# thisparticle/scl_slam

Measured on AMD Instinct MI355X. Metric: loop-closure candidates/sec: (scan, keyframe) pairs taken through full-database ARG-MIN detection per second (every pair aligned exactly and bounded by the f16 matrix-core screening; only the survivors get the f64 distance), batches of 16 scans, 10k-keyframe DB per GPU, higher is better.
Workload: dtype f64 results; f16-operand / f32-accumulate MFMA screening + f64 exact pass on the survivors

## Files before the change

### include/scl_engine.h

```cpp
#ifndef SCL_ENGINE_H
#define SCL_ENGINE_H

#include <stddef.h>
#include <stdint.h>

#ifdef __cplusplus
extern "C" {
#endif

typedef struct scl_engine scl_engine;

typedef enum scl_status {
    SCL_OK               =  0,
    SCL_ERR_INVALID_ARG  = -1,
    SCL_ERR_NO_DEVICE    = -2,
    SCL_ERR_HIP          = -3,
    SCL_ERR_OUT_OF_RANGE = -4,
    SCL_ERR_NOMEM        = -5,
    SCL_ERR_UNSUPPORTED  = -6
} scl_status;

typedef struct scl_config {
    int    num_ring;
    int    num_sector;
// ... 149 lines not shown
                             const scl_icp_params *p, int min_src_points, int min_tgt_points,
                             float T[16], float *fitness, int *converged, int *iterations, int *n_src, int *n_tgt);
int  scl_loop_icp_batch_from_store(scl_engine *e, int robot, int key_cur, const float *pose_cur,
                                   int n_candidates, const int *keys_pre, int search_num, const float *poses_pre, float leaf,
                                   const scl_icp_params *p, int min_src_points, int min_tgt_points,
                                   float *T, float *fitness, int *converged, int *iterations, int *n_src, int *n_tgts);

int  scl_geometric_verification_from_store(scl_engine *e, const void *src, int n_src, int stride_bytes, float src_leaf,
                                           int robot, int key_pre, int search_num, const float *poses_pre, float leaf,
                                           int min_src_points, int min_tgt_points,
                                           int ransac_iterations, double inlier_threshold, double inlier_ratio, uint64_t seed,
                                           float T[16], int *success, int *n_src_filtered, int *n_tgt,
                                           int *n_correspondences, int *n_inliers);

int  scl_geometric_verification_batch(scl_engine *e, const void *src, int n_src,
                                      const void *const *tgts, const int *n_tgts, int n_targets, int stride_bytes,
                                      int ransac_iterations, double inlier_threshold, double inlier_ratio, uint64_t seed,
                                      float *T, int *success, int *n_correspondences, int *n_inliers);
int  scl_geometric_verification_batch_from_store(scl_engine *e, const void *src, int n_src, int stride_bytes, float src_leaf,
                                                 int robot, int n_candidates, const int *keys_pre, int search_num, const float *poses_pre, float leaf,
                                                 int min_src_points, int min_tgt_points,
                                                 int ransac_iterations, double inlier_threshold, double inlier_ratio, uint64_t seed,
                                                 float *T, int *success, int *n_src_filtered, int *n_tgts,
                                                 int *n_correspondences, int *n_inliers);

int  scl_geometric_verification_batch_guess(scl_engine *e, const void *src, int n_src,
                                            const void *const *tgts, const int *n_tgts, int n_targets, int stride_bytes,
                                            const float *guesses,
                                            int ransac_iterations, double inlier_threshold, double inlier_ratio, uint64_t seed,
                                            float *T, float *T_fit, int *success, int *n_correspondences, int *n_inliers);
int  scl_geometric_verification_batch_from_store_guess(scl_engine *e, const void *src, int n_src, int stride_bytes, float src_leaf,
                                                       int robot, int n_candidates, const int *keys_pre, int search_num, const float *poses_pre, float leaf,
                                                       const float *guesses,
                                                       int min_src_points, int min_tgt_points,
                                                       int ransac_iterations, double inlier_threshold, double inlier_ratio, uint64_t seed,
                                                       float *T, float *T_fit, int *success, int *n_src_filtered, int *n_tgts,
                                                       int *n_correspondences, int *n_inliers);

int  scl_icp_align_batch_guess(scl_engine *e, const void *src, int n_src, const void *const *tgts, const int *n_tgts,
                               int n_targets, int stride_bytes, const float *guesses, const scl_icp_params *p,
                               float *T, float *T_icp, float *fitness, int *converged, int *iterations);
int  scl_loop_icp_batch_from_store_guess(scl_engine *e, int robot, int key_cur, const float *pose_cur,
                                         int n_candidates, const int *keys_pre, int search_num, const float *poses_pre, float leaf,
                                         const float *guesses, const scl_icp_params *p, int min_src_points, int min_tgt_points,
                                         float *T, float *T_icp, float *fitness, int *converged, int *iterations, int *n_src, int *n_tgts);
int  scl_icp_align_batch_from_store_guess(scl_engine *e, const void *src, int n_src, int stride_bytes, float src_leaf,
                                          int robot, int n_candidates, const int *keys_pre, int search_num, const float *poses_pre, float leaf,
                                          const float *guesses, const scl_icp_params *p, int min_src_points, int min_tgt_points,
                                          float *T, float *T_icp, float *fitness, int *converged, int *iterations,
                                          int *n_src_filtered, int *n_tgts);

int  scl_registration_eval_batch(scl_engine *e, const void *src, int n_src, const void *const *tgts, const int *n_tgts,
                                 int n_targets, int stride_bytes, const float *transforms, double max_dist,
                                 int *n_valid, int *n_inliers, double *moments);
int  scl_registration_eval_batch_from_store(scl_engine *e, const void *src, int n_src, int stride_bytes, float src_leaf,
                                            int robot, int n_candidates, const int *keys_pre, int search_num, const float *poses_pre, float leaf,
                                            const float *transforms, int min_src_points, int min_tgt_points, double max_dist,
                                            int *n_valid, int *n_inliers, double *moments, int *n_src_filtered, int *n_tgts);
int  scl_loop_eval_batch_from_store(scl_engine *e, int robot, int key_cur, const float *pose_cur,
                                    int n_candidates, const int *keys_pre, int search_num, const float *poses_pre, float leaf,
                                    const float *transforms, int min_src_points, int min_tgt_points, double max_dist,
                                    int *n_valid, int *n_inliers, double *moments, int *n_src, int *n_tgts);
int  scl_registration_information(int n_inliers, const double moments[10], double info[36]);

int  scl_target_normals(scl_engine *e, const void *tgt, int n_tgt, int stride_bytes, double radius, float *normals);
int  scl_registration_eval_plane_batch(scl_engine *e, const void *src, int n_src, const void *const *tgts, const int *n_tgts,
                                       int n_targets, int stride_bytes, const float *transforms, double max_dist, double normal_radius,
                                       int *n_valid, int *n_inliers, int *n_planar, double *sums);
int  scl_registration_eval_plane_batch_from_store(scl_engine *e, const void *src, int n_src, int stride_bytes, float src_leaf,
                                                  int robot, int n_candidates, const int *keys_pre, int search_num, const float *poses_pre, float leaf,
                                                  const float *transforms, int min_src_points, int min_tgt_points, double max_dist, double normal_radius,
                                                  int *n_valid, int *n_inliers, int *n_planar, double *sums, int *n_src_filtered, int *n_tgts);
int  scl_loop_eval_plane_batch_from_store(scl_engine *e, int robot, int key_cur, const float *pose_cur,
                                          int n_candidates, const int *keys_pre, int search_num, const float *poses_pre, float leaf,
                                          const float *transforms, int min_src_points, int min_tgt_points, double max_dist, double normal_radius,
                                          int *n_valid, int *n_inliers, int *n_planar, double *sums, int *n_src, int *n_tgts);
int  scl_registration_information_plane(const double sums[29], double info[36], double grad[6]);

int  scl_profile_enable(scl_engine *e, int on);
int  scl_profile_reset(scl_engine *e);
int  scl_profile_get(scl_engine *e, scl_profile *out);
void scl_debug_icp_tile_stats(unsigned long long out[16], int reset);
int  scl_alignment_stats(scl_engine *e, uint64_t *pairs, uint64_t *fallbacks, int reset);
int  scl_survivor_stats(scl_engine *e, uint64_t *queries, uint64_t *survivors, uint64_t *max_survivors, int reset);
int  scl_device_name(const scl_engine *e, char *buf, int buflen);
int  scl_host_copy_rate(scl_engine *e, size_t bytes, int reps, double *gbytes_per_s);
int  scl_selftest_atanf_blocks(scl_engine *e, int first_block, int n_blocks, uint64_t *checksums);
int  scl_selftest_bin_paths(scl_engine *e, int mode, uint64_t seed, uint64_t n_points, uint64_t *disagreements, uint64_t *sure);

int  scl_selftest_sort_pairs(scl_engine *e, int key_bytes, const void *keys, const uint32_t *values, int n, int bits, const int *segment_offsets,
                             int n_segments, void *keys_out, uint32_t *values_out);
int  scl_selftest_prefix_sum(scl_engine *e, const int32_t *in, int n, int inclusive, int32_t *out);
int  scl_selftest_submaps_batch(scl_engine *e, int robot, int n_jobs, const int *keys, const int *search_nums,
                                const float *poses ,
                                float leaf, void *out, int out_capacity , int *n_out );

#ifdef __cplusplus
}
#endif
#endif
```

### scl_slam_amd/csrc/engine.hip

```cpp
#include "scl_engine.h"

#include <hip/hip_runtime.h>

#include <cfloat>
#include <climits>
#include <chrono>
#include <cmath>
#include <cstdio>
#include <cstdlib>
#include <cstring>
#include <mutex>
#include <new>
#include <string>
#include <atomic>
#include <chrono>
#include <thread>
#include <vector>

#include "db_file.hpp"
#include "engine_internal.hpp"
#include "device_sort.hpp"
#include "plugin_host.hpp"

#ifdef SCL_DIAGNOSTICS
// ... 128 lines not shown
    if ((rc = dev_alloc(e, &nd, tile * nst))) return rc;
    if ((rc = dev_alloc(e, &nv, (size_t)e->S * nst))) return rc;
    if ((rc = dev_alloc(e, &nn, (size_t)e->S * nst))) return rc;
    if ((rc = dev_alloc(e, &nr, (size_t)e->R4 * nst))) return rc;
    if ((rc = dev_alloc(e, &nh, (size_t)e->hstride * nst))) return rc;
    if ((rc = dev_alloc(e, &nk, (size_t)8 * nst))) return rc;
    if ((rc = dev_alloc(e, &nhk, (size_t)e->hkw * nst))) return rc;
    if (hab && (rc = dev_alloc(e, &nha, hab * (size_t)ncap))) return rc;
    if ((rc = dev_alloc(e, &nr4, (size_t)e->RG * ncap))) return rc;
    SCL_HIP(e, hipMemsetAsync(nr4, 0, sizeof(float4) * (size_t)e->RG * ncap, e->stream));
    if (e->n > 0) {
        SCL_HIP(e, hipMemcpyAsync(nd, e->d_desc, sizeof(float4) * tile * e->n, hipMemcpyDeviceToDevice, e->stream));
        SCL_HIP(e, hipMemcpyAsync(nv, e->d_vkey, sizeof(double) * (size_t)e->S * e->n, hipMemcpyDeviceToDevice, e->stream));
        SCL_HIP(e, hipMemcpyAsync(nn, e->d_norm, sizeof(double) * (size_t)e->S * e->n, hipMemcpyDeviceToDevice, e->stream));
        SCL_HIP(e, hipMemcpyAsync(nr, e->d_rkey, sizeof(float) * (size_t)e->R4 * e->n, hipMemcpyDeviceToDevice, e->stream));
        SCL_HIP(e, hipMemcpyAsync(nh, e->d_hdesc, sizeof(uint2) * (size_t)e->hstride * e->n, hipMemcpyDeviceToDevice, e->stream));
        SCL_HIP(e, hipMemcpyAsync(nk, e->d_kmask, sizeof(unsigned int) * (size_t)8 * e->n, hipMemcpyDeviceToDevice, e->stream));
        SCL_HIP(e, hipMemcpyAsync(nhk, e->d_hkey, sizeof(unsigned short) * (size_t)e->hkw * e->n, hipMemcpyDeviceToDevice, e->stream));
        if (hab) SCL_HIP(e, hipMemcpyAsync(nha, e->d_halign, hab * (size_t)e->n, hipMemcpyDeviceToDevice, e->stream));
        SCL_HIP(e, hipMemcpy2DAsync(nr4, sizeof(float4) * ncap, e->d_rkey4, sizeof(float4) * e->cap,
                                    sizeof(float4) * e->n, e->RG, hipMemcpyDeviceToDevice, e->stream));
    }
    if (e->cap > 0) {
        const size_t k = (size_t)e->stage_rows;
        SCL_HIP(e, hipMemcpyAsync(nd + tile * ncap, e->d_desc + tile * e->cap, sizeof(float4) * tile * k, hipMemcpyDeviceToDevice, e->stream));
        SCL_HIP(e, hipMemcpyAsync(nv + (size_t)e->S * ncap, e->d_vkey + (size_t)e->S * e->cap, sizeof(double) * e->S * k, hipMemcpyDeviceToDevice, e->stream));
        SCL_HIP(e, hipMemcpyAsync(nn + (size_t)e->S * ncap, e->d_norm + (size_t)e->S * e->cap, sizeof(double) * e->S * k, hipMemcpyDeviceToDevice, e->stream));
        SCL_HIP(e, hipMemcpyAsync(nr + (size_t)e->R4 * ncap, e->d_rkey + (size_t)e->R4 * e->cap, sizeof(float) * e->R4 * k, hipMemcpyDeviceToDevice, e->stream));
        SCL_HIP(e, hipMemcpyAsync(nh + (size_t)e->hstride * ncap, e->d_hdesc + (size_t)e->hstride * e->cap, sizeof(uint2) * e->hstride * k, hipMemcpyDeviceToDevice, e->stream));
        SCL_HIP(e, hipMemcpyAsync(nk + (size_t)8 * ncap, e->d_kmask + (size_t)8 * e->cap, sizeof(unsigned int) * 8 * k, hipMemcpyDeviceToDevice, e->stream));
        SCL_HIP(e, hipMemcpyAsync(nhk + (size_t)e->hkw * ncap, e->d_hkey + (size_t)e->hkw * e->cap, sizeof(unsigned short) * e->hkw * k, hipMemcpyDeviceToDevice, e->stream));
    }
    SCL_HIP(e, hipStreamSynchronize(e->stream));
    for (hipStream_t s2 : {e->stream_alt, e->stream_surv, e->stream2})
        if (s2) SCL_HIP(e, hipStreamSynchronize(s2));
    dev_free(e->d_desc); dev_free(e->d_vkey); dev_free(e->d_norm); dev_free(e->d_rkey); dev_free(e->d_rkey4);
    dev_free(e->d_hdesc); dev_free(e->d_kmask); dev_free(e->d_hkey); dev_free(e->d_halign);
    e->d_desc = nd; e->d_vkey = nv; e->d_norm = nn; e->d_rkey = nr; e->d_rkey4 = nr4;
    e->d_hdesc = nh; e->d_kmask = nk; e->d_hkey = nhk; e->d_halign = nha;
    e->cap = ncap;
    return SCL_OK;
}

int ensure_vals(scl_engine *e, size_t floats)
{
    if (floats <= e->vals_cap) return SCL_OK;
    dev_free(e->d_vals);
    int rc = dev_alloc(e, &e->d_vals, floats);
    if (rc) { e->vals_cap = 0; return rc; }
    e->vals_cap = floats;
    return SCL_OK;
}

int ensure_points(scl_engine *e, size_t bytes)
{
    if (bytes <= e->points_cap) return SCL_OK;
    dev_free(e->d_points);
    size_t nb = bytes + bytes / 4 + 4096;
    int rc = dev_alloc(e, &e->d_points, nb);
    if (rc) { e->points_cap = 0; return rc; }
    e->points_cap = nb;
    return SCL_OK;
}

int ensure_pairs(scl_engine *e, size_t n)
{
    if (n <= e->pair_cap) return SCL_OK;
    dev_free(e->d_dist); dev_free(e->d_shift); dev_free(e->d_cand); dev_free(e->d_ring_d2);
    dev_free(e->d_approx); dev_free(e->d_surv); dev_free(e->d_starts);
    size_t nn = n + n / 2 + 64;
    int rc;
    e->pair_cap = 0;
    if ((rc = dev_alloc(e, &e->d_approx, nn))) return rc;
    if ((rc = dev_alloc(e, &e->d_starts, nn))) return rc;
    if ((rc = dev_alloc(e, &e->d_surv, nn))) return rc;
    if ((rc = dev_alloc(e, &e->d_ring_d2, nn))) return rc;
    if ((rc = dev_alloc(e, &e->d_dist, nn))) return rc;
    if ((rc = dev_alloc(e, &e->d_shift, nn))) return rc;
    if ((rc = dev_alloc(e, &e->d_cand, nn))) return rc;
    e->pair_cap = nn;
    return SCL_OK;
}

int ensure_sets(scl_engine *e, size_t n)
{
    if (n <= e->set_stride && e->pair_cap >= e->set_stride * scl_engine::kScreenSets) return SCL_OK;
    const size_t stride = n + n / 4 + 64;
    int rc = ensure_pairs(e, stride * scl_engine::kScreenSets);
    if (rc) { e->set_stride = 0; return rc; }
    e->set_stride = stride;
    if (e->smask_cap < stride * scl_engine::kScreenSets) {
        dev_free(e->d_smask); e->d_smask = nullptr; e->smask_cap = 0;
        if ((rc = dev_alloc(e, &e->d_smask, stride * scl_engine::kScreenSets))) { e->set_stride = 0; return rc; }
        e->smask_cap = stride * scl_engine::kScreenSets;
    }
    const size_t need = 2 * stride * sc_screen_scratch_floats(db_view(e), e->SR);
    if (need > e->part_cap) {
        dev_free(e->d_part); e->part_cap = 0;
        if ((rc = dev_alloc(e, &e->d_part, need))) { e->set_stride = 0; return rc; }
        e->part_cap = need;
    }
    return SCL_OK;
}

int ensure_pinned(scl_engine *e, size_t bytes)
{
    if (bytes <= e->pinned_cap) return SCL_OK;
    if (e->h_pinned) { (void)hipHostFree(e->h_pinned); e->h_pinned = nullptr; e->pinned_cap = 0; }
    SCL_HIP(e, hipHostMalloc(&e->h_pinned, bytes, hipHostMallocDefault));
    memset(e->h_pinned, 0, bytes);
    e->pinned_cap = bytes;
    return SCL_OK;
}

int ingest_from_vals(scl_engine *e, int count, int first_slot)
{
    ProfScope ps(e, P_INGEST);
    SCL_HIP(e, launch_ingest(e->d_vals, count, first_slot, e->d_desc, e->d_vkey, e->d_norm, e->d_rkey,
                             e->d_rkey4, e->d_hdesc, e->d_kmask, e->d_hkey, e->hstride, e->cap, e->R, e->S, e->stream, e->d_halign));
    e->db_version++;
    return SCL_OK;
}

int append_meta(scl_engine *e, int8_t robot, int index)
{
    e->robots.push_back(robot);
    e->indexs.push_back(index);
    e->n++;
    return SCL_OK;
}

int ensure_tiles(scl_engine *e, hipStream_t s)
{
    int rc;
    if (!e->d_tiles) {
        if ((rc = dev_alloc(e, &e->d_tiles, (size_t)2 * kMaxScBatch * e->R * e->S))) return rc;
        e->tiles_clean = false;
    }
    if (!e->tiles_clean) {
        SCL_HIP(e, launch_make_sc_tiles_init(e->d_tiles, 2 * kMaxScBatch, e->R, e->S, s));
        e->tiles_clean = true;
    }
    return SCL_OK;
}

int check_cloud(scl_engine *e, const void *points, int n_points, int stride_bytes)
{
    if (n_points < 0 || stride_bytes < 12 || (stride_bytes & 3)) return fail(e, SCL_ERR_INVALID_ARG, "bad point layout");
    if (n_points > 0 && !points) return fail(e, SCL_ERR_INVALID_ARG, "null points");
    return SCL_OK;
}

int group_scatter(scl_engine *e, const unsigned char *const *dptr, const int *n, int count, int stride, hipStream_t s)
{
    int rc;
    if (count < 1 || count > kMaxScBatch) return fail(e, SCL_ERR_INVALID_ARG, "batch of 1..16 scans");
    if ((rc = ensure_tiles(e, s))) return rc;
    if ((rc = ensure_vals(e, (size_t)e->R * e->S * (size_t)kMaxScBatch))) return rc;
    ScanBatch b{};
    b.count = count;
    uint64_t pts = 0;
    for (int i = 0; i < count; ++i) { b.points[i] = dptr[i]; b.n[i] = n[i]; pts += (uint64_t)n[i]; }
    e->tiles_clean = false;
    ProfScope ps(e, P_MAKESC, s);
    const int slice = e->R * e->S > 10000 ? 2 * kScPointsPerWorkgroup : kScPointsPerWorkgroup;
    SCL_HIP(e, launch_make_sc_batch(b, stride, e->R, e->S, e->cfg.lidar_height, e->cfg.max_radius, e->d_tiles,
                                    scl_lab_int("SCL_SC_SLICE", slice), e->num_cu, s));
    e->prof.make_sc_points += e->prof_on ? pts : 0;
// ... 135 lines not shown
const char *scl_status_string(int status)
{
    switch (status) {
    case SCL_OK: return "ok";
    case SCL_ERR_INVALID_ARG: return "invalid argument";
    case SCL_ERR_NO_DEVICE: return "no HIP device";
    case SCL_ERR_HIP: return "HIP runtime error";
    case SCL_ERR_OUT_OF_RANGE: return "index out of range";
    case SCL_ERR_NOMEM: return "out of memory";
    case SCL_ERR_UNSUPPORTED: return "unsupported";
    default: return "unknown status";
    }
}

const char *scl_last_error(const scl_engine *e) { return e ? e->last_error.c_str() : "null engine"; }

int scl_abi_version(void) { return 11; }

int scl_default_config(scl_config *c)
{
    if (!c) return SCL_ERR_INVALID_ARG;
    c->num_ring = 20; c->num_sector = 60; c->num_candidates = 3;
    c->dist_thres = 0.14; c->lidar_height = 1.65; c->max_radius = 80.0;
    c->num_exclude_recent = 100; c->tree_making_period = 10;
    c->search_ratio = 0.1;
    c->knn_exclude_eps = 0.0f;
    c->device = 0;
    c->initial_capacity = 4096;
    return SCL_OK;
}

static void log_env_overrides_once()
{
    static std::atomic<bool> done{false};
    if (done.exchange(true)) return;
    static const char *const names[] = {"SCL_SCREEN", "SCL_SCREEN_FORM", "SCL_SCREEN_V2_MIN", "SCL_RCCL_LIB",
                                        "SCL_SCREEN_VARIANT", "SCL_SCREEN_PROBE", "SCL_SCREEN_TAIL", "SCL_ALIGN_WGS",
                                        "SCL_ALIGN2_WGS", "SCL_ALIGN_FILTER", "SCL_SC_KERNEL", "SCL_SC_WAVES", "SCL_STAMP", "SCL_ABLATE",
                                        "SCL_ICP_REDUCE", "SCL_MATRIX_PLAIN", "SCL_MATRIX_KERNEL", "SCL_MATRIX_KR", "SCL_WIDE_EXACT", "SCL_STREAM_EXACT", "SCL_SMALL_EXACT_OFF",
                                        "SCL_SELF_ALIGN_OFF", "SCL_CAND_EXACT_OFF"};
    constexpr int kProduct = 4;
    int i = 0;
    for (const char *n : names) {
        const char *v = getenv(n);
#ifdef SCL_DIAGNOSTICS
        if (v) fprintf(stderr, "scl_engine (diagnostics build): environment override in effect: %s=%s\n", n, v);
#else
        if (v && i < kProduct) fprintf(stderr, "scl_engine: environment override in effect: %s=%s\n", n, v);
        else if (v) fprintf(stderr, "scl_engine: %s=%s is an experiment's switch: ignored by this build (make EXTRA=-DSCL_DIAGNOSTICS builds them in)\n", n, v);
#endif
        ++i;
    }
    (void)kProduct;
}

int scl_create(const scl_config *cfg, scl_engine **out)
{
    if (!cfg || !out) return SCL_ERR_INVALID_ARG;
    *out = nullptr;
    log_env_overrides_once();
    if (cfg->num_ring < 1 || cfg->num_ring > 256 || cfg->num_sector < 1 || cfg->num_sector > 1024 ||
        cfg->num_candidates < 1 || cfg->num_candidates > kTopkMaxK || cfg->tree_making_period < 1 ||
        cfg->num_exclude_recent < 0 || !(cfg->max_radius > 0.0) || !(cfg->search_ratio >= 0.0))
        return SCL_ERR_INVALID_ARG;
    int ndev = 0;
    if (hipGetDeviceCount(&ndev) != hipSuccess || ndev <= 0) return SCL_ERR_NO_DEVICE;
    if (cfg->device < 0 || cfg->device >= ndev) return SCL_ERR_INVALID_ARG;
    scl_engine *e = new (std::nothrow) scl_engine();
    if (!e) return SCL_ERR_NOMEM;
    e->cfg = *cfg;
    e->R = cfg->num_ring; e->S = cfg->num_sector;
    e->RG = (e->R + 3) / 4; e->R4 = e->RG * 4;
    e->hstride = hdesc_stride(e->RG, e->S);
    e->hkw = hkey_row_halfs(e->S);
    e->SR = (int)std::round(0.5 * cfg->search_ratio * (double)e->S);
    if (e->SR < 0) e->SR = 0;
    e->device = cfg->device;
    int rc = SCL_OK;
    auto bail = [&](int code) { scl_destroy(e); return code; };
    if (hipSetDevice(e->device) != hipSuccess) return bail(SCL_ERR_HIP);
    hipDeviceProp_t prop;
    if (hipGetDeviceProperties(&prop, e->device) == hipSuccess && prop.multiProcessorCount > 0)
        e->num_cu = prop.multiProcessorCount;
    if (hipStreamCreateWithFlags(&e->stream, hipStreamNonBlocking) != hipSuccess) return bail(SCL_ERR_HIP);
    {
        int lo_p = 0, hi_p = 0;
        (void)hipDeviceGetStreamPriorityRange(&lo_p, &hi_p);
        if (hipStreamCreateWithPriority(&e->stream2, hipStreamNonBlocking, hi_p) != hipSuccess) return bail(SCL_ERR_HIP);
    }
    if (hipEventCreateWithFlags(&e->ev_fork, hipEventDisableTiming) != hipSuccess) return bail(SCL_ERR_HIP);
    if (hipEventCreateWithFlags(&e->ev_join, hipEventDisableTiming) != hipSuccess) return bail(SCL_ERR_HIP);
    if (hipHostMalloc((void **)&e->h_out3, 64 * scl_engine::kSlots, hipHostMallocDefault) != hipSuccess) return bail(SCL_ERR_HIP);
    memset(e->h_out3, 0, 64 * scl_engine::kSlots);
    for (int i = 0; i < scl_engine::kSlots; ++i)
        if (hipEventCreateWithFlags(&e->ev_done[i], hipEventDisableTiming) != hipSuccess) return bail(SCL_ERR_HIP);
    if ((rc = ensure_capacity(e, 1))) return bail(rc);
    if ((rc = dev_alloc(e, &e->d_topk_scratch, (size_t)kTopkMaxBlocks * kTopkMaxK + 2))) return bail(rc);
    if (hipMemset(e->d_topk_scratch, 0, sizeof(unsigned long long) * ((size_t)kTopkMaxBlocks * kTopkMaxK + 2)) != hipSuccess) return bail(SCL_ERR_HIP);
    if ((rc = dev_alloc(e, &e->d_topk_idx, (size_t)kTopkMaxK * scl_engine::kScreenSets))) return bail(rc);
    if ((rc = dev_alloc(e, &e->d_topk_d2, (size_t)kTopkMaxK * scl_engine::kScreenSets))) return bail(rc);
    if ((rc = dev_alloc(e, &e->d_out3, (size_t)4))) return bail(rc);
    if ((rc = dev_alloc(e, &e->d_blk_part, (size_t)kTailBlocks * kTailRec * kMaxQueryBatch))) return bail(rc);
    static_assert(kMaxQueryBatch <= 4, "done_counter holds four counters");
    if ((rc = dev_alloc(e, &e->d_done_counter, (size_t)4))) return bail(rc);
    if (hipMemset(e->d_done_counter, 0, 16) != hipSuccess) return bail(SCL_ERR_HIP);
    {
        constexpr int NS = scl_engine::kScreenSets;
        if ((rc = dev_alloc(e, &e->d_nsurv, (size_t)NS))) return bail(rc);
        static_assert(NS <= kTminEpsOffset, "the launch's largest bound sits kTminEpsOffset words behind its t_min word");
        if ((rc = dev_alloc(e, &e->d_tmin, (size_t)NS + kTminEpsOffset))) return bail(rc);
        if (hipMemset(e->d_nsurv, 0, sizeof(int) * NS) != hipSuccess) return bail(SCL_ERR_HIP);
        if (hipMemset(e->d_tmin, 0xff, sizeof(unsigned int) * NS) != hipSuccess) return bail(SCL_ERR_HIP);
        if (hipMemset(e->d_tmin + NS, 0, sizeof(unsigned int) * kTminEpsOffset) != hipSuccess) return bail(SCL_ERR_HIP);
        if ((rc = dev_alloc(e, &e->d_surv_part, (size_t)NS * kSurvivorBlocks * kTailRec))) return bail(rc);
        if ((rc = dev_alloc(e, &e->d_surv_done, (size_t)NS))) return bail(rc);
        if (hipMemset(e->d_surv_done, 0, sizeof(unsigned int) * NS) != hipSuccess) return bail(SCL_ERR_HIP);
        if (hipMalloc(&e->d_surv_args, (size_t)8 * NS * kSurvivorArgBytes) != hipSuccess) return bail(SCL_ERR_NOMEM);
        if (hipHostMalloc(&e->h_surv_args, (size_t)8 * NS * kSurvivorArgBytes, hipHostMallocDefault) != hipSuccess) return bail(SCL_ERR_HIP);
        if (hipHostMalloc((void **)&e->h_stream_out, (size_t)2 * NS * 64, hipHostMallocDefault) != hipSuccess) return bail(SCL_ERR_HIP);
        for (auto &ev : e->ev_chunk) if (hipEventCreateWithFlags(&ev, hipEventDisableTiming) != hipSuccess) return bail(SCL_ERR_HIP);
        for (auto &ev : e->ev_k1) if (hipEventCreateWithFlags(&ev, hipEventDisableTiming) != hipSuccess) return bail(SCL_ERR_HIP);
        for (auto &ev : e->ev_sub0) if (hipEventCreateWithFlags(&ev, hipEventDisableTiming) != hipSuccess) return bail(SCL_ERR_HIP);
        if (hipEventCreateWithFlags(&e->ev_align_gate, hipEventDisableTiming) != hipSuccess) return bail(SCL_ERR_HIP);
        {
            int lo_p = 0, hi_p = 0;
            (void)hipDeviceGetStreamPriorityRange(&lo_p, &hi_p);
            const bool wide_grid = e->S == 180 && e->RG == 20;
            if (hipStreamCreateWithPriority(&e->stream_surv, hipStreamNonBlocking, wide_grid ? hi_p : lo_p) != hipSuccess) return bail(SCL_ERR_HIP);
            if (hipStreamCreateWithPriority(&e->stream_queue_place, hipStreamNonBlocking, lo_p) != hipSuccess) return bail(SCL_ERR_HIP);
        }
    }
    if (hipStreamCreateWithFlags(&e->stream_alt, hipStreamNonBlocking) != hipSuccess) return bail(SCL_ERR_HIP);
    if (hipEventCreateWithFlags(&e->ev_db, hipEventDisableTiming) != hipSuccess) return bail(SCL_ERR_HIP);
    if ((rc = dev_alloc(e, &e->d_align_fallbacks, (size_t)1))) return bail(rc);
    if (hipMemset(e->d_align_fallbacks, 0, sizeof(unsigned long long)) != hipSuccess) return bail(SCL_ERR_HIP);
    if ((rc = dev_alloc(e, &e->d_surv_stats, (size_t)3))) return bail(rc);
    if (hipMemset(e->d_surv_stats, 0, 3 * sizeof(unsigned long long)) != hipSuccess) return bail(SCL_ERR_HIP);
    if ((rc = ensure_pairs(e, 1024))) return bail(rc);
    e->screen = sc_screen_supported(db_view(e), e->SR) && cfg->num_candidates <= kTailTopMaxK;
    if ((rc = ensure_pinned(e, 1 << 16))) return bail(rc);
    if ((rc = ensure_vals(e, (size_t)e->R * e->S))) return bail(rc);
    *out = e;
    return SCL_OK;
}

int scl_destroy(scl_engine *e)
{
#ifdef SCL_DIAGNOSTICS
    if (e && !e->front && scl_lab_int("SCL_INGEST_STAMPS", 0)) { (void)hipSetDevice(e->device); scl::ingest_stamps_print(); scl::cand_stamps_print(); }
#endif
    if (!e) return SCL_OK;
    if (e->front) return front_destroy(e);
    (void)hipSetDevice(e->device);
    if (e->stream) (void)hipStreamSynchronize(e->stream);
    for (auto &p : e->pending) { (void)hipEventDestroy(p.start); (void)hipEventDestroy(p.stop); }
    for (auto ev : e->event_pool) (void)hipEventDestroy(ev);
    icp_workspace_free(&e->icp_ws);
    icp_workspace_free(&e->vox_ws);
    for (void *slab : e->kf_slabs) (void)hipFree(slab);
    for (int i = 0; i < scl_engine::kIcpBatch; ++i) icp_workspace_free(&e->icp_batch_ws[i]);
    for (int i = 0; i < scl_engine::kIcpLanes; ++i) icp_workspace_free(&e->vox_lane_ws[i]);
    icp_workspace_free(&e->icp_batch_ctl);
    for (int i = 0; i < scl_engine::kIcpLanes; ++i) {
        if (e->ev_lane[i]) (void)hipEventDestroy(e->ev_lane[i]);
        icp_workspace_free(&e->icp_lane_ws[i]);
        if (e->icp_lane_stream[i]) (void)hipStreamDestroy(e->icp_lane_stream[i]);
    }
    dev_free(e->d_desc); dev_free(e->d_vkey); dev_free(e->d_norm); dev_free(e->d_rkey); dev_free(e->d_rkey4);
    dev_free(e->d_hdesc); dev_free(e->d_kmask); dev_free(e->d_hkey); dev_free(e->d_halign);
    dev_free(e->d_vals); dev_free(e->d_points); dev_free(e->d_tiles);
    for (int b = 0; b < 3; ++b) {
        dev_free(e->d_pbuf[b]);
        for (int c = 0; c < scl_engine::kCopyStreams; ++c) if (e->ev_copied[c][b]) (void)hipEventDestroy(e->ev_copied[c][b]);
        if (e->ev_consumed[b]) (void)hipEventDestroy(e->ev_consumed[b]);
    }
    if (e->stream_copy) { (void)hipStreamSynchronize(e->stream_copy); (void)hipStreamDestroy(e->stream_copy); }
    for (hipStream_t cs : e->stream_copy_x) if (cs) { (void)hipStreamSynchronize(cs); (void)hipStreamDestroy(cs); }
    for (void *hp : e->host_allocs) (void)hipHostFree(hp);
    dev_free(e->d_dist); dev_free(e->d_shift); dev_free(e->d_cand); dev_free(e->d_ring_d2);
    dev_free(e->d_approx); dev_free(e->d_starts); dev_free(e->d_surv); dev_free(e->d_nsurv); dev_free(e->d_tmin); dev_free(e->d_part);
    dev_free(e->d_align_fallbacks);
    dev_free(e->d_smask);
    if (e->d_mat_dist) (void)hipFree(e->d_mat_dist);
    if (e->d_mat_shift) (void)hipFree(e->d_mat_shift);
    if (e->d_rank_key) (void)hipFree(e->d_rank_key);
    if (e->d_rank_pos) (void)hipFree(e->d_rank_pos);
    if (e->d_rank_out) (void)hipFree(e->d_rank_out);
    if (e->h_rank_out) (void)hipHostFree(e->h_rank_out);
    dev_free(e->d_meta_robot); dev_free(e->d_meta_index);
    if (e->h_mat) (void)hipHostFree(e->h_mat);
    for (auto &ev : e->ev_mat_k) if (ev) (void)hipEventDestroy(ev);
    for (auto &ev : e->ev_mat_c) if (ev) (void)hipEventDestroy(ev);
    dev_free(e->d_surv_stats);
    dev_free(e->d_surv_part); dev_free(e->d_surv_done);
    if (e->d_surv_args) (void)hipFree(e->d_surv_args);
    if (e->h_surv_args) (void)hipHostFree(e->h_surv_args);
    if (e->h_stream_out) (void)hipHostFree(e->h_stream_out);
    for (auto ev : e->ev_chunk) if (ev) (void)hipEventDestroy(ev);
    if (e->stream_surv) { (void)hipStreamSynchronize(e->stream_surv); (void)hipStreamDestroy(e->stream_surv); }
    if (e->stream_queue_place) (void)hipStreamDestroy(e->stream_queue_place);
    for (auto ev : e->ev_k1) if (ev) (void)hipEventDestroy(ev);
    for (auto ev : e->ev_sub0) if (ev) (void)hipEventDestroy(ev);
    if (e->ev_align_gate) (void)hipEventDestroy(e->ev_align_gate);
    dev_free(e->d_topk_scratch); dev_free(e->d_topk_idx); dev_free(e->d_topk_d2); dev_free(e->d_out3);
    dev_free(e->d_blk_part); dev_free(e->d_done_counter);
    if (e->ev_db) (void)hipEventDestroy(e->ev_db);
    if (e->stream_alt) { (void)hipStreamSynchronize(e->stream_alt); (void)hipStreamDestroy(e->stream_alt); }
    if (e->h_pinned) (void)hipHostFree(e->h_pinned);
    if (e->h_out3) (void)hipHostFree(e->h_out3);
    if (e->ev_call) (void)hipEventDestroy(e->ev_call);
    for (int i = 0; i < scl_engine::kSlots; ++i) if (e->ev_done[i]) (void)hipEventDestroy(e->ev_done[i]);
    if (e->ev_fork) (void)hipEventDestroy(e->ev_fork);
    if (e->ev_join) (void)hipEventDestroy(e->ev_join);
    if (e->stream2) { (void)hipStreamSynchronize(e->stream2); (void)hipStreamDestroy(e->stream2); }
    if (e->stream) (void)hipStreamDestroy(e->stream);
    delete e;
    return SCL_OK;
}


int scl_make_and_save(scl_engine *e, const void *points, int n_points, int stride_bytes,
                      int8_t robot, int index, float *out_values)
{
    if (!e) return SCL_ERR_INVALID_ARG;
    if (e->front) return front_make_and_save(e, points, n_points, stride_bytes, robot, index, out_values, false, 0.f, nullptr);
    std::lock_guard<std::mutex> lk(e->mu);
    (void)hipSetDevice(e->device);
    int rc;
    if ((rc = ensure_capacity(e, e->n + 1))) return rc;
    if ((rc = scatter_host_cloud(e, points, n_points, stride_bytes))) return rc;
    if ((rc = group_ingest(e, 1, e->n, e->stream))) return rc;
    if (out_values)
        SCL_HIP(e, hipMemcpyAsync(out_values, e->d_vals, sizeof(float) * (size_t)e->R * e->S,
                                  hipMemcpyDeviceToHost, e->stream));
    if ((rc = sync_short(e))) return rc;
    return append_meta(e, robot, index);
}

int scl_make_and_save_filtered(scl_engine *e, const void *points, int n_points, int stride_bytes, float leaf,
                               int8_t robot, int index, float *out_values, int *n_filtered)
{
    if (!e) return SCL_ERR_INVALID_ARG;
    if (e->front) return front_make_and_save(e, points, n_points, stride_bytes, robot, index, out_values, true, leaf, n_filtered);
    std::lock_guard<std::mutex> lk(e->mu);
    (void)hipSetDevice(e->device);
    int rc;
    if ((rc = check_cloud(e, points, n_points, stride_bytes))) return rc;
    if ((rc = ensure_capacity(e, e->n + 1))) return rc;
    std::string err;
    const void *d_cloud = nullptr;
    int m = 0;
    if ((rc = voxel_grid_to_device(&e->vox_ws, e->stream, points, n_points, stride_bytes, leaf, &d_cloud, &m, &err))) { e->last_error = err; return rc; }
    const unsigned char *dp = static_cast<const unsigned char *>(d_cloud);
    if ((rc = group_scatter(e, &dp, &m, 1, stride_bytes, e->stream))) return rc;
    if ((rc = group_ingest(e, 1, e->n, e->stream))) return rc;
    if (out_values)
        SCL_HIP(e, hipMemcpyAsync(out_values, e->d_vals, sizeof(float) * (size_t)e->R * e->S,
                                  hipMemcpyDeviceToHost, e->stream));
    if ((rc = sync(e))) return rc;
    if (n_filtered) *n_filtered = m;
    return append_meta(e, robot, index);
}

// ... 516 lines not shown

int scl_sc_search_range(scl_engine *e, const int *queries, const int *lo, const int *hi, int n_queries, int k,
                        int *cand_ids, int *cand_shifts, double *cand_dists, int *n_found)
{
    if (!e || n_queries < 0 || k < 1 || k > SCL_SC_SEARCH_MAX || (n_queries > 0 && (!queries || !lo || !hi || !cand_ids))) return SCL_ERR_INVALID_ARG;
    if (n_queries == 0) return SCL_OK;
    if (e->front) return front_sc_search_range(e, queries, lo, hi, n_queries, k, cand_ids, cand_shifts, cand_dists, n_found);
    std::lock_guard<std::mutex> pk(e->pass_mu);
    std::lock_guard<std::mutex> lk(e->mu);
    (void)hipSetDevice(e->device);
    return sc_search_locked(e, queries, lo, hi, n_queries, k, cand_ids, cand_shifts, cand_dists, n_found);
}

int scl_sc_search(scl_engine *e, const int *curs, int count, int k, int *cand_ids, int *cand_shifts, double *cand_dists, int *n_found)
{
    if (!e || count < 0 || k < 1 || k > SCL_SC_SEARCH_MAX || (count > 0 && (!curs || !cand_ids))) return SCL_ERR_INVALID_ARG;
    if (count == 0) return SCL_OK;
    std::vector<int> lo((size_t)count, 0), hi((size_t)count, 0);
    for (int i = 0; i < count; ++i) {
        if (curs[i] < 0) return SCL_ERR_OUT_OF_RANGE;
        const int h = curs[i] - e->cfg.num_exclude_recent;
        hi[(size_t)i] = h > 0 ? h : 0;
    }
    return scl_sc_search_range(e, curs, lo.data(), hi.data(), count, k, cand_ids, cand_shifts, cand_dists, n_found);
}

namespace {

int sc_search_robot(scl_engine *e, const int *curs, int count, bool inter, int robot_pre, int k,
                    int *cand_ids, int *cand_shifts, double *cand_dists, int *n_found)
{
    std::lock_guard<std::mutex> pk(e->pass_mu);
    std::lock_guard<std::mutex> lk(e->mu);
    (void)hipSetDevice(e->device);
    for (int i = 0; i < count; ++i)
        if (curs[i] < 0 || curs[i] >= e->n) return fail(e, SCL_ERR_OUT_OF_RANGE, "query keyframe out of range");
    std::vector<ScRankRule> rules((size_t)count);
    for (int i = 0; i < count; ++i) {
        const int r = e->robots[(size_t)curs[i]], x = e->indexs[(size_t)curs[i]];
        if (inter && robot_pre != SCL_SC_ANY_OTHER_ROBOT && robot_pre == r) return fail(e, SCL_ERR_INVALID_ARG, "robot_pre is the query's own robot: that is scl_sc_search_intra's set");
        rules[(size_t)i] = inter ? sc_inter_rule(r, robot_pre) : sc_intra_rule(r, x, e->cfg.num_exclude_recent);
    }
    const std::vector<int> lo((size_t)count, 0), hi((size_t)count, e->n);
    return sc_search_locked(e, curs, lo.data(), hi.data(), count, k, cand_ids, cand_shifts, cand_dists, n_found, rules.data());
}

}

int scl_sc_search_intra(scl_engine *e, const int *curs, int count, int k, int *cand_ids, int *cand_shifts, double *cand_dists, int *n_found)
{
    if (!e || count < 0 || k < 1 || k > SCL_SC_SEARCH_MAX || (count > 0 && (!curs || !cand_ids))) return SCL_ERR_INVALID_ARG;
    if (count == 0) return SCL_OK;
    if (e->front) return front_sc_search_intra(e, curs, count, k, cand_ids, cand_shifts, cand_dists, n_found);
    return sc_search_robot(e, curs, count, false, 0, k, cand_ids, cand_shifts, cand_dists, n_found);
}

int scl_sc_search_inter(scl_engine *e, const int *curs, int count, int robot_pre, int k, int *cand_ids, int *cand_shifts, double *cand_dists,
                        int *n_found)
{
    if (!e || count < 0 || k < 1 || k > SCL_SC_SEARCH_MAX || (count > 0 && (!curs || !cand_ids))) return SCL_ERR_INVALID_ARG;
    if (robot_pre < SCL_SC_ANY_OTHER_ROBOT || robot_pre > 127) return SCL_ERR_INVALID_ARG;
    if (count == 0) return SCL_OK;
    if (e->front) return front_sc_search_inter(e, curs, count, robot_pre, k, cand_ids, cand_shifts, cand_dists, n_found);
    return sc_search_robot(e, curs, count, true, robot_pre, k, cand_ids, cand_shifts, cand_dists, n_found);
}

namespace {

int submit_full_many_locked(scl_engine *e, const int *queries, const int *los, const int *his, int nq, int *tickets);

struct ScreenGroup { const int *qslot, *lo, *n; int nq, set0; int part_half = 0; bool masks = false; bool keys_later = false; };
int launch_screen_group(scl_engine *e, const ScreenGroup &cur, int phases = kScreenAlign | kScreenProducts,
                        const ScreenGroup *next = nullptr, hipStream_t stream = nullptr)
{
    if (!stream) stream = e->stream;
    auto fill = [&](ScreenBatch &sb, const ScreenGroup &g) {
        sb.nq = g.nq;
        for (int j = 0; j < g.nq; ++j) { sb.slot[j] = g.qslot[j]; sb.base[j] = g.lo[j]; sb.n[j] = g.n[j]; sb.buf[j] = g.set0 + j; }
        sb.pair_stride = e->set_stride;
        sb.approx = e->d_approx; sb.starts = e->d_starts; sb.align_fallbacks = e->d_align_fallbacks; sb.ring_d2 = e->d_ring_d2;
        sb.survivors = nullptr; sb.n_surv = nullptr; sb.t_min = e->d_tmin;
        sb.smask = (g.masks || sc_screen_is_wide(db_view(e), e->SR)) ? e->d_smask : nullptr;
        sb.part = e->d_part + (g.part_half ? e->part_cap / 2 : 0);
        sb.no_ring_metric = g.keys_later;
        sb.k = e->cfg.num_candidates; sb.exclude_eps = e->cfg.knn_exclude_eps; sb.topk_idx = e->d_topk_idx; sb.topk_d2 = e->d_topk_d2;
    };
    ScreenBatch sb{}, nx{};
    fill(sb, cur);
    const bool has_next = next && next->nq > 0;
    if (has_next) fill(nx, *next);
    if (phases & kScreenAlign) for (int j = 0; j < cur.nq; ++j) e->align_pairs += (uint64_t)cur.n[j];
    if (has_next) for (int j = 0; j < next->nq; ++j) e->align_pairs += (uint64_t)next->n[j];
    if ((phases & kScreenAlign) && (phases & kScreenProducts) && has_next) {
        SCL_HIP(e, launch_sc_screen_batch(db_view(e), sb, e->SR, sc_align_filter_enabled(), e->num_cu, stream, kScreenAlign, nullptr));
        phases = kScreenProducts;
    }
    ProfScope ps(e, P_SC, stream);
    SCL_HIP(e, launch_sc_screen_batch(db_view(e), sb, e->SR, sc_align_filter_enabled(), e->num_cu, stream, phases, has_next ? &nx : nullptr));
    if (ps.active()) { for (int j = 0; j < cur.nq; ++j) e->prof.sc_distance_pairs += (uint64_t)cur.n[j]; }
    return SCL_OK;
}

unsigned survivor_arg_region(scl_engine *e) { return e->surv_arg_tick++ & 7u; }
int launch_survivor_pass(scl_engine *e, const int *qslot, const int *lo, const int *n, int nq, int set0, double *const *out3, hipStream_t stream = nullptr,
                         int phases = kSurvivorArgs | kSurvivorKernel, int region_in = -1, bool ring_from_keys = false)
{
    if (!stream) stream = e->stream;
    SurvivorPass sp{};
    sp.nq = nq; sp.ring_from_keys = ring_from_keys ? 1 : 0;
    for (int j = 0; j < nq; ++j) { sp.slot[j] = qslot[j]; sp.base[j] = lo[j]; sp.n[j] = n[j]; sp.buf[j] = set0 + j; sp.out3[j] = out3[j]; }
    sp.pair_stride = e->set_stride;
    sp.approx = e->d_approx; sp.survivors = e->d_surv; sp.t_min = e->d_tmin; sp.out_dist = e->d_dist; sp.out_shift = e->d_shift;
    sp.blk_part = e->d_surv_part; sp.done_counter = e->d_surv_done; sp.surv_stats = e->d_surv_stats;
    sp.ring_d2 = e->d_ring_d2; sp.k = e->cfg.num_candidates; sp.exclude_eps = e->cfg.knn_exclude_eps; sp.topk_idx = e->d_topk_idx; sp.topk_d2 = e->d_topk_d2;
    const size_t region = (size_t)(region_in >= 0 ? (unsigned)region_in : survivor_arg_region(e)) * scl_engine::kScreenSets * kSurvivorArgBytes;
    sp.d_args = static_cast<char *>(e->d_surv_args) + region; sp.h_args = static_cast<char *>(e->h_surv_args) + region;
    if (!(phases & kSurvivorKernel)) {
        SCL_HIP(e, launch_sc_distance_survivors(db_view(e), sp, e->SR, e->num_cu, stream, phases));
        return SCL_OK;
    }
    ProfScope ps(e, P_ARGMIN, stream);
    SCL_HIP(e, launch_sc_distance_survivors(db_view(e), sp, e->SR, e->num_cu, stream, phases));
    return SCL_OK;
}

int launch_small_exact_chunk(scl_engine *e, const int *qslot, const int *lo, const int *n, int nq, int set0, double *const *out3, hipStream_t stream,
                             int phases, int region_in)
{
    static_assert(sizeof(SmallExactQuery) <= kSurvivorArgBytes && kMaxSmallExactQueries <= scl_engine::kScreenSets, "argument regions");
    if (nq < 1 || nq > kMaxSmallExactQueries) return fail(e, SCL_ERR_INVALID_ARG, "exact pass: too many scans for one launch");
    const size_t region = (size_t)(region_in >= 0 ? (unsigned)region_in : survivor_arg_region(e)) * scl_engine::kScreenSets * kSurvivorArgBytes;
    SmallExactQuery *h = reinterpret_cast<SmallExactQuery *>(static_cast<char *>(e->h_surv_args) + region);
    SmallExactQuery *d = reinterpret_cast<SmallExactQuery *>(static_cast<char *>(e->d_surv_args) + region);
    const bool wide_masks = sc_screen_is_wide(db_view(e), e->SR) && e->d_smask;
    if (phases & kSurvivorArgs) {
        for (int j = 0; j < nq; ++j) {
            const size_t set = (size_t)(set0 + j), off = set * e->set_stride;
            SmallExactQuery &sq = h[j];
            sq.qslot = qslot[j]; sq.base = lo[j]; sq.n = n[j];
            sq.approx = e->d_approx + off; sq.starts = e->d_starts + off; sq.smask = wide_masks ? e->d_smask + off : nullptr; sq.ring_d2 = e->d_ring_d2 + off;
            sq.t_min = e->d_tmin + set; sq.list = e->d_surv + off; sq.out3 = out3[j];
            sq.topk_idx = e->d_topk_idx + set * kTailTopMaxK; sq.topk_d2 = e->d_topk_d2 + set * kTailTopMaxK;
        }
        SCL_HIP(e, hipMemcpyAsync(d, h, sizeof(SmallExactQuery) * (size_t)nq, hipMemcpyHostToDevice, stream));
    }
    if (!(phases & kSurvivorKernel)) return SCL_OK;
    SmallExactArgs sa{};
    sa.nq = nq; sa.k = e->cfg.num_candidates; sa.exclude_eps = e->cfg.knn_exclude_eps; sa.two_eps = 2.0f * sc_screen_eps(); sa.surv_stats = e->d_surv_stats;
    sa.q_dev = d;
    sa.every_shift = wide_masks ? 0 : 1;
    ProfScope ps(e, P_ARGMIN, stream);
    SCL_HIP(e, launch_sc_small_exact(db_view(e), e->SR, sa, stream));
    return SCL_OK;
}

int launch_survivor_pass_wide(scl_engine *e, const int *qslot, const int *lo, const int *n, int nq, int set0, double *const *out3, hipStream_t stream, hipEvent_t first_done = nullptr)
{
    ProfScope ps(e, P_ARGMIN, stream);
    for (int g = 0; g < nq; g += kWideExactBatch) {
        const int w = nq - g < kWideExactBatch ? nq - g : kWideExactBatch;
        ScreenBatch sb{};
        sb.nq = w;
        for (int j = 0; j < w; ++j) { sb.slot[j] = qslot[g + j]; sb.base[j] = lo[g + j]; sb.n[j] = n[g + j]; sb.buf[j] = set0 + g + j; }
        sb.pair_stride = e->set_stride;
        sb.approx = e->d_approx; sb.starts = e->d_starts; sb.align_fallbacks = e->d_align_fallbacks; sb.ring_d2 = e->d_ring_d2;
        sb.survivors = e->d_surv; sb.n_surv = e->d_nsurv; sb.t_min = e->d_tmin; sb.surv_stats = e->d_surv_stats;
// ... 1017 lines not shown

int scl_screen_distances(scl_engine *e, int query, int lo, int hi, float *approx, int *survivors, int *n_survivors, float *eps)
{
    if (!e || !approx) return SCL_ERR_INVALID_ARG;
    if (e->front) return fail(e, SCL_ERR_UNSUPPORTED, "screen_distances: call it on a one-GPU engine");
    std::lock_guard<std::mutex> pk(e->pass_mu);
    std::lock_guard<std::mutex> lk(e->mu);
    (void)hipSetDevice(e->device);
    if (eps) *eps = sc_screen_eps();
    if (!e->screen) return fail(e, SCL_ERR_UNSUPPORTED, "no screening pass for this grid (64x120 and 80x180 at search ratio 0.1 only)");
    int qslot;
    if (query >= 0) { if (query >= e->n) return fail(e, SCL_ERR_OUT_OF_RANGE, "query slot out of range"); qslot = query; }
    else { const int j = -1 - query; if (j >= e->stage_rows || !e->staged[j]) return fail(e, SCL_ERR_INVALID_ARG, "no staged query"); qslot = e->cap + j; }
    if (lo < 0) lo = 0;
    if (hi > e->n) hi = e->n;
    const int n = hi - lo;
    if (n_survivors) *n_survivors = 0;
    if (n <= 0) return SCL_OK;
    int rc;
    if ((rc = ensure_pairs(e, (size_t)n))) return rc;
    {
        const size_t per_pair = sc_screen_scratch_floats(db_view(e), e->SR) / (size_t)sc_screen_max_batch(db_view(e), e->SR);
        if ((size_t)n * per_pair > e->part_cap) {
            dev_free(e->d_part); e->part_cap = 0;
            if ((rc = dev_alloc(e, &e->d_part, (size_t)n * per_pair + 1024))) return rc;
            e->part_cap = (size_t)n * per_pair + 1024;
        }
    }
    ScreenBatch sb{};
    sb.part = e->d_part;
    sb.nq = 1; sb.slot[0] = qslot; sb.base[0] = lo; sb.n[0] = n; sb.pair_stride = (size_t)n;
    sb.approx = e->d_approx; sb.starts = e->d_starts; sb.align_fallbacks = e->d_align_fallbacks; sb.ring_d2 = e->d_ring_d2; sb.survivors = e->d_surv; sb.n_surv = e->d_nsurv; sb.t_min = e->d_tmin;
    sb.k = e->cfg.num_candidates; sb.exclude_eps = e->cfg.knn_exclude_eps; sb.topk_idx = e->d_topk_idx; sb.topk_d2 = e->d_topk_d2;
    SCL_HIP(e, launch_sc_screen_batch(db_view(e), sb, e->SR, sc_align_filter_enabled(), e->num_cu, e->stream));
    SCL_HIP(e, launch_sc_select_batch(sb, e->stream));
    SCL_HIP(e, hipMemcpyAsync(approx, e->d_approx, sizeof(float) * (size_t)n, hipMemcpyDeviceToHost, e->stream));
    int ns = 0;
    SCL_HIP(e, hipMemcpyAsync(&ns, e->d_nsurv, sizeof(int), hipMemcpyDeviceToHost, e->stream));
    if ((rc = sync(e))) return rc;
    if (n_survivors) *n_survivors = ns;
    if (survivors && ns > 0) {
        SCL_HIP(e, hipMemcpyAsync(survivors, e->d_surv, sizeof(int) * (size_t)ns, hipMemcpyDeviceToHost, e->stream));
        if ((rc = sync(e))) return rc;
    }
    return SCL_OK;
}

int scl_screen_distances_many(scl_engine *e, const int *queries, int n_queries, int lo, int hi, float *approx, float *eps)
{
    if (!e || !queries || !approx || n_queries < 1 || n_queries > kMaxScreenBatch) return SCL_ERR_INVALID_ARG;
    if (e->front) return fail(e, SCL_ERR_UNSUPPORTED, "screen_distances_many: call it on a one-GPU engine");
    std::lock_guard<std::mutex> pk(e->pass_mu);
    std::lock_guard<std::mutex> lk(e->mu);
    (void)hipSetDevice(e->device);
    if (eps) *eps = sc_screen_eps();
    if (!e->screen) return fail(e, SCL_ERR_UNSUPPORTED, "no screening pass for this grid (64x120 and 80x180 at search ratio 0.1 only)");
    if (n_queries > sc_screen_max_batch(db_view(e), e->SR)) return fail(e, SCL_ERR_INVALID_ARG, "more scans than a screening launch takes");
    if (lo < 0) lo = 0;
    if (hi > e->n) hi = e->n;
    const int n = hi - lo;
    if (n <= 0) return SCL_OK;
    int rc;
    if ((rc = ensure_pairs(e, (size_t)n * (size_t)n_queries))) return rc;
    {
        const size_t per_pair = sc_screen_scratch_floats(db_view(e), e->SR) / (size_t)sc_screen_max_batch(db_view(e), e->SR);
        const size_t want = (size_t)n * (size_t)n_queries * per_pair + 1024;
        if (want > e->part_cap) {
            dev_free(e->d_part); e->part_cap = 0;
            if ((rc = dev_alloc(e, &e->d_part, want))) return rc;
            e->part_cap = want;
        }
    }
    ScreenBatch sb{};
    sb.part = e->d_part;
    sb.nq = n_queries; sb.pair_stride = (size_t)n;
    for (int i = 0; i < n_queries; ++i) {
        const int q = queries[i];
        if (q >= 0) { if (q >= e->n) return fail(e, SCL_ERR_OUT_OF_RANGE, "query slot out of range"); sb.slot[i] = q; }
        else { const int j = -1 - q; if (j >= e->stage_rows || !e->staged[j]) return fail(e, SCL_ERR_INVALID_ARG, "no staged query"); sb.slot[i] = e->cap + j; }
        sb.base[i] = lo; sb.n[i] = n; sb.buf[i] = i;
    }
    sb.approx = e->d_approx; sb.starts = e->d_starts; sb.align_fallbacks = e->d_align_fallbacks; sb.ring_d2 = e->d_ring_d2; sb.survivors = e->d_surv; sb.n_surv = e->d_nsurv; sb.t_min = e->d_tmin;
    sb.k = e->cfg.num_candidates; sb.exclude_eps = e->cfg.knn_exclude_eps; sb.topk_idx = e->d_topk_idx; sb.topk_d2 = e->d_topk_d2;
    SCL_HIP(e, launch_sc_screen_batch(db_view(e), sb, e->SR, sc_align_filter_enabled(), e->num_cu, e->stream));
    SCL_HIP(e, hipMemsetAsync(e->d_tmin, 0xff, sizeof(unsigned int) * (size_t)n_queries, e->stream));
    SCL_HIP(e, hipMemsetAsync(e->d_tmin + kTminEpsOffset, 0, sizeof(unsigned int) * (size_t)n_queries, e->stream));
    SCL_HIP(e, hipMemcpyAsync(approx, e->d_approx, sizeof(float) * (size_t)n * (size_t)n_queries, hipMemcpyDeviceToHost, e->stream));
    return sync(e);
}

int scl_get_last_topk(scl_engine *e, int k, int *idx, float *d2)
{
    if (!e || !idx || !d2 || k < 1 || k > kTopkMaxK) return SCL_ERR_INVALID_ARG;
    if (e->front) return front_get_last_topk(e, k, idx, d2);
    std::lock_guard<std::mutex> pk(e->pass_mu);
    std::lock_guard<std::mutex> lk(e->mu);
    (void)hipSetDevice(e->device);
    if (e->last_pass_empty) {
        for (int i = 0; i < k; ++i) { idx[i] = -1; d2[i] = FLT_MAX; }
        return SCL_OK;
    }
    SCL_HIP(e, hipMemcpyAsync(idx, e->d_topk_idx, sizeof(int) * k, hipMemcpyDeviceToHost, e->stream));
    SCL_HIP(e, hipMemcpyAsync(d2, e->d_topk_d2, sizeof(float) * k, hipMemcpyDeviceToHost, e->stream));
    return sync(e);
}

int scl_detect_full(scl_engine *e, int cur, int *loop_id, int *nn_idx, int *shift, double *dist)
{
    if (!e || !loop_id || !nn_idx || !shift || !dist) return SCL_ERR_INVALID_ARG;
    *loop_id = -1;
    if (cur < 0) return SCL_ERR_OUT_OF_RANGE;
    const int hi = cur - e->cfg.num_exclude_recent;
    int rc = scl_detect_full_range(e, cur, 0, hi, nn_idx, shift, dist);
    if (rc) return rc;
    if (*nn_idx >= 0 && *dist < e->cfg.dist_thres) *loop_id = *nn_idx;
    return SCL_OK;
}


int scl_get_descriptors(const scl_engine *ce, int first, int count, float *values)
{
    scl_engine *e = const_cast<scl_engine *>(ce);
    if (!e || !values || first < 0 || count < 0) return SCL_ERR_INVALID_ARG;
    const size_t cells = (size_t)e->R * e->S;
    if (e->front) {
        for (int i = 0; i < count; ++i) { const int rc = scl_get_descriptor(e, first + i, values + (size_t)i * cells); if (rc) return rc; }
        return SCL_OK;
    }
    std::lock_guard<std::mutex> lk(e->mu);
    (void)hipSetDevice(e->device);
    if (first + count > e->n) return fail(e, SCL_ERR_OUT_OF_RANGE, "get_descriptors: range exceeds the database");
    const int chunk = 512;
    int rc;
    if ((rc = ensure_vals(e, cells * (size_t)(count < chunk ? (count > 0 ? count : 1) : chunk)))) return rc;
    for (int done = 0; done < count; done += chunk) {
        const int c = count - done < chunk ? count - done : chunk;
        for (int i = 0; i < c; ++i)
            SCL_HIP(e, launch_untile(e->d_desc + (size_t)(first + done + i) * e->RG * e->S, e->R, e->S, e->d_vals + (size_t)i * cells, e->stream));
        SCL_HIP(e, hipMemcpyAsync(values + (size_t)done * cells, e->d_vals, sizeof(float) * cells * (size_t)c, hipMemcpyDeviceToHost, e->stream));
        if ((rc = sync(e))) return rc;
    }
    return SCL_OK;
}

int scl_find_key(const scl_engine *e, int8_t robot, int index, int *key)
{
    if (!e || !key) return SCL_ERR_INVALID_ARG;
    *key = -1;
    const int n = scl_get_size(e, -1);
    if (n < 0) return n;
    for (int k = n - 1; k >= 0; --k) {
        int8_t r = 0; int idx = 0;
        const int rc = scl_get_index(e, k, &r, &idx);
        if (rc) return rc;
        if (r == robot && idx == index) { *key = k; break; }
    }
    return SCL_OK;
}

int scl_db_dump_file(scl_engine *e, const char *path)
{
    if (!e || !path) return SCL_ERR_INVALID_ARG;
    const int n = scl_get_size(e, -1);
    if (n < 0) return n;
    FILE *f = std::fopen(path, "wb");
    if (!f) return fail(e, SCL_ERR_INVALID_ARG, "db_dump: cannot open the file for writing");
// ... 1268 lines not shown
                                      int *n_valid, int *n_inliers, int *n_planar, double *sums)
{
    const EvalPlane pl = {normal_radius, n_planar, sums};
    return eval_batch_host(e, src, n_src, tgts, n_tgts, n_targets, stride_bytes, transforms, max_dist, n_valid, n_inliers, nullptr, &pl);
}

int scl_registration_eval_plane_batch_from_store(scl_engine *e, const void *src, int n_src, int stride_bytes, float src_leaf,
                                                 int robot, int n_candidates, const int *keys_pre, int search_num, const float *poses_pre, float leaf,
                                                 const float *transforms, int min_src_points, int min_tgt_points, double max_dist, double normal_radius,
                                                 int *n_valid, int *n_inliers, int *n_planar, double *sums, int *n_src_filtered, int *n_tgts)
{
    const EvalPlane pl = {normal_radius, n_planar, sums};
    return eval_batch_store(e, true, src, n_src, stride_bytes, src_leaf, robot, 0, nullptr, n_candidates, keys_pre, search_num, poses_pre, leaf,
                            transforms, min_src_points, min_tgt_points, max_dist, n_valid, n_inliers, nullptr, n_src_filtered, n_tgts, &pl);
}

int scl_loop_eval_plane_batch_from_store(scl_engine *e, int robot, int key_cur, const float *pose_cur,
                                         int n_candidates, const int *keys_pre, int search_num, const float *poses_pre, float leaf,
                                         const float *transforms, int min_src_points, int min_tgt_points, double max_dist, double normal_radius,
                                         int *n_valid, int *n_inliers, int *n_planar, double *sums, int *n_src, int *n_tgts)
{
    const EvalPlane pl = {normal_radius, n_planar, sums};
    return eval_batch_store(e, false, nullptr, 0, 0, 0.f, robot, key_cur, pose_cur, n_candidates, keys_pre, search_num, poses_pre, leaf,
                            transforms, min_src_points, min_tgt_points, max_dist, n_valid, n_inliers, nullptr, n_src, n_tgts, &pl);
}

int scl_registration_information_plane(const double sums[29], double info[36], double grad[6])
{
    if (!sums || !info) return SCL_ERR_INVALID_ARG;
    int t = 0;
    for (int a = 0; a < 6; ++a)
        for (int b = a; b < 6; ++b) { info[6 * a + b] = sums[t]; info[6 * b + a] = sums[t]; ++t; }
    if (grad) for (int a = 0; a < 6; ++a) grad[a] = sums[21 + a];
    return SCL_OK;
}


int scl_profile_enable(scl_engine *e, int on)
{
    if (!e) return SCL_ERR_INVALID_ARG;
    if (e->front) return front_profile_enable(e, on);
    std::lock_guard<std::mutex> lk(e->mu);
    e->prof_on = on < 0 ? 0 : (on > 3 ? 1 : on);
    e->prof_tick = 0;
    return SCL_OK;
}

int scl_profile_reset(scl_engine *e)
{
    if (!e) return SCL_ERR_INVALID_ARG;
    if (e->front) return front_profile_reset(e);
    std::lock_guard<std::mutex> lk(e->mu);
    std::memset(&e->prof, 0, sizeof e->prof);
    return SCL_OK;
}

int scl_profile_get(scl_engine *e, scl_profile *out)
{
    if (!e || !out) return SCL_ERR_INVALID_ARG;
    if (e->front) return front_profile_get(e, out);
    std::lock_guard<std::mutex> lk(e->mu);
    *out = e->prof;
    return SCL_OK;
}

int scl_alignment_stats(scl_engine *e, uint64_t *pairs, uint64_t *fallbacks, int reset)
{
    if (!e) return SCL_ERR_INVALID_ARG;
    if (e->front) return front_alignment_stats(e, pairs, fallbacks, reset);
    std::lock_guard<std::mutex> lk(e->mu);
    (void)hipSetDevice(e->device);
    unsigned long long f = 0;
    SCL_HIP(e, hipStreamSynchronize(e->stream));
    SCL_HIP(e, hipMemcpy(&f, e->d_align_fallbacks, sizeof f, hipMemcpyDeviceToHost));
    if (pairs) *pairs = e->align_pairs;
    if (fallbacks) *fallbacks = (uint64_t)f;
    if (reset) {
        SCL_HIP(e, hipMemset(e->d_align_fallbacks, 0, sizeof f));
        e->align_pairs = 0;
    }
    return SCL_OK;
}

int scl_survivor_stats(scl_engine *e, uint64_t *queries, uint64_t *survivors, uint64_t *max_survivors, int reset)
{
    if (!e) return SCL_ERR_INVALID_ARG;
    if (e->front) return front_survivor_stats(e, queries, survivors, max_survivors, reset);
    std::lock_guard<std::mutex> lk(e->mu);
    (void)hipSetDevice(e->device);
    unsigned long long s[3] = {0, 0, 0};
    SCL_HIP(e, hipStreamSynchronize(e->stream));
    if (e->stream_surv) SCL_HIP(e, hipStreamSynchronize(e->stream_surv));
    SCL_HIP(e, hipMemcpy(s, e->d_surv_stats, sizeof s, hipMemcpyDeviceToHost));
    if (survivors) *survivors = (uint64_t)s[0];
    if (max_survivors) *max_survivors = (uint64_t)s[1];
    if (queries) *queries = (uint64_t)s[2];
    if (reset) SCL_HIP(e, hipMemset(e->d_surv_stats, 0, sizeof s));
    return SCL_OK;
}

int scl_device_name(const scl_engine *e, char *buf, int buflen)
{
    if (!e || !buf || buflen <= 0) return SCL_ERR_INVALID_ARG;
    if (e->front) e = front_primary(e);
    hipDeviceProp_t prop;
    if (hipGetDeviceProperties(&prop, e->device) != hipSuccess) return SCL_ERR_HIP;
    std::snprintf(buf, (size_t)buflen, "%s (%s, %d CUs)", prop.name, prop.gcnArchName, prop.multiProcessorCount);
    return SCL_OK;
}

}

namespace scl {

int eng_stage_from_peer(scl_engine *dst, int j, scl_engine *src, int src_slot, int count)
{
    if (!dst || !src || count < 1 || j < 0 || j + count > dst->stage_rows) return SCL_ERR_INVALID_ARG;
    std::lock_guard<std::mutex> lk(dst->mu);
    if (src_slot < 0 || src_slot + count > src->n) return fail(dst, SCL_ERR_OUT_OF_RANGE, "stage_from_peer: source slot out of range");
    (void)hipSetDevice(dst->device);
    const size_t tile = (size_t)dst->RG * dst->S, S = (size_t)dst->S, R4 = (size_t)dst->R4, m = (size_t)count;
    const size_t d = (size_t)dst->cap + (size_t)j, s = (size_t)src_slot;
    if (dst->hstride != src->hstride || dst->hkw != src->hkw) return fail(dst, SCL_ERR_INVALID_ARG, "stage_from_peer: the shards' layouts differ");
    SCL_HIP(dst, hipMemcpyPeerAsync(dst->d_desc + d * tile, dst->device, src->d_desc + s * tile, src->device, sizeof(float4) * tile * m, dst->stream));
    SCL_HIP(dst, hipMemcpyPeerAsync(dst->d_vkey + d * S, dst->device, src->d_vkey + s * S, src->device, sizeof(double) * S * m, dst->stream));
    SCL_HIP(dst, hipMemcpyPeerAsync(dst->d_norm + d * S, dst->device, src->d_norm + s * S, src->device, sizeof(double) * S * m, dst->stream));
    SCL_HIP(dst, hipMemcpyPeerAsync(dst->d_rkey + d * R4, dst->device, src->d_rkey + s * R4, src->device, sizeof(float) * R4 * m, dst->stream));
    SCL_HIP(dst, hipMemcpyPeerAsync(dst->d_hdesc + d * dst->hstride, dst->device, src->d_hdesc + s * src->hstride, src->device, sizeof(uint2) * src->hstride * m, dst->stream));
    SCL_HIP(dst, hipMemcpyPeerAsync(dst->d_kmask + d * 8, dst->device, src->d_kmask + s * 8, src->device, sizeof(unsigned int) * 8 * m, dst->stream));
    SCL_HIP(dst, hipMemcpyPeerAsync(dst->d_hkey + d * dst->hkw, dst->device, src->d_hkey + s * src->hkw, src->device, sizeof(unsigned short) * src->hkw * m, dst->stream));
    for (int i = 0; i < count; ++i) dst->staged[j + i] = true;
    return SCL_OK;
}

int eng_set_stage_rows(scl_engine *e, int rows)
{
    if (!e || rows < scl_engine::kStage) return SCL_ERR_INVALID_ARG;
    std::lock_guard<std::mutex> lk(e->mu);
    if (e->n > 0) return fail(e, SCL_ERR_INVALID_ARG, "stage rows are fixed once a keyframe is stored");
    (void)hipSetDevice(e->device);
    const int old_cap = e->cap;
    e->stage_rows = rows;
    e->staged.assign((size_t)rows, 0);
    e->cap = 0;
    return ensure_capacity(e, old_cap > 0 ? old_cap : 1);
}

int eng_stage_values(scl_engine *e, int j, const float *values)
{
    if (!e || !values || j < 0 || j >= e->stage_rows) return SCL_ERR_INVALID_ARG;
    std::lock_guard<std::mutex> lk(e->mu);
    (void)hipSetDevice(e->device);
    int rc;
    const size_t cells = (size_t)e->R * e->S;
    if ((rc = ensure_vals(e, cells))) return rc;
    SCL_HIP(e, hipMemcpyAsync(e->d_vals, values, sizeof(float) * cells, hipMemcpyHostToDevice, e->stream));
    {
        ProfScope ps(e, P_INGEST);
        SCL_HIP(e, launch_ingest(e->d_vals, 1, e->cap + j, e->d_desc, e->d_vkey, e->d_norm, e->d_rkey, nullptr, e->d_hdesc, e->d_kmask, e->d_hkey, e->hstride,
                                 e->cap, e->R, e->S, e->stream));
    }
    if ((rc = sync(e))) return rc;
    e->staged[j] = true;
    return SCL_OK;
}

// ... 78 lines not shown
```

### scl_slam_amd/csrc/engine_internal.hpp

```cpp
#pragma once

#include "scl_engine.h"

#include <hip/hip_runtime.h>

#include <climits>
#include <mutex>
#include <string>
#include <vector>

#include "icp.hpp"
#include "kernels.hpp"

namespace scl {

enum ProfKind { P_SC = 0, P_TOPK, P_ARGMIN, P_MAKESC, P_INGEST, P_ICPNN, P_ICPRED, P_COUNT };

struct PendingEvent { hipEvent_t start, stop; int kind; int launches = 1; };

struct ShardedFront;

}

struct scl_engine {
    scl_config cfg;
    scl::ShardedFront *front = nullptr;
    int R = 0, S = 0, RG = 0, R4 = 0, SR = 0;
    int device = 0, num_cu = 256;
    hipStream_t stream = nullptr;
    hipStream_t stream2 = nullptr;
    hipEvent_t ev_fork = nullptr, ev_join = nullptr;
    double *h_out3 = nullptr;
    static constexpr int kSlots = 8;
    hipEvent_t ev_done[kSlots] = {nullptr};
    hipEvent_t ev_call = nullptr;
    int slot_lo[kSlots] = {0}; bool slot_busy[kSlots] = {false}; bool slot_empty[kSlots] = {false};
    unsigned int pinned_seq = 0;
    unsigned int slot_seq[kSlots] = {0}; unsigned int out_seq = 0;
    int slot_ev[kSlots] = {0};
    unsigned next_slot = 0;
    mutable std::mutex mu;
    mutable std::mutex pass_mu;
    mutable std::string last_error;

    int n = 0, cap = 0;
    float4 *d_desc = nullptr; double *d_vkey = nullptr; double *d_norm = nullptr;
    float *d_rkey = nullptr; float4 *d_rkey4 = nullptr;
    uint2 *d_hdesc = nullptr; unsigned int *d_kmask = nullptr; int hstride = 0;
    unsigned char *d_halign = nullptr;
    unsigned short *d_hkey = nullptr; int hkw = 0;
    std::vector<int8_t> robots;
    std::vector<int> indexs;

    static constexpr int kStage = 76;
    int stage_rows = kStage;
    std::vector<unsigned char> staged = std::vector<unsigned char>(kStage, 0);

    float *d_vals = nullptr; size_t vals_cap = 0;
    unsigned char *d_points = nullptr; size_t points_cap = 0;
    int *d_tiles = nullptr; bool tiles_clean = false;
    unsigned char *d_pbuf[3] = {nullptr, nullptr, nullptr}; size_t pbuf_cap = 0;
    static constexpr int kCopyStreams = 4;
    hipStream_t stream_copy = nullptr;
    hipStream_t stream_copy_x[kCopyStreams - 1] = {nullptr, nullptr, nullptr};
    hipEvent_t ev_copied[kCopyStreams][3] = {}, ev_consumed[3] = {nullptr, nullptr, nullptr};
    std::vector<void *> host_allocs;
    double *d_dist = nullptr; int *d_shift = nullptr; int *d_cand = nullptr; float *d_ring_d2 = nullptr; size_t pair_cap = 0;
#ifndef SCL_SCREEN_SETS
#define SCL_SCREEN_SETS 256
#endif
    static constexpr int kScreenSets = SCL_SCREEN_SETS;
    float *d_approx = nullptr; int *d_starts = nullptr; int *d_surv = nullptr;
    unsigned int *d_smask = nullptr; size_t smask_cap = 0;
    float *d_part = nullptr; size_t part_cap = 0;
    int *d_nsurv = nullptr; unsigned int *d_tmin = nullptr;
    unsigned long long *d_align_fallbacks = nullptr; uint64_t align_pairs = 0;
    unsigned long long *d_surv_stats = nullptr;
    size_t set_stride = 0;
    unsigned long long *d_surv_part = nullptr; unsigned int *d_surv_done = nullptr;
    void *d_surv_args = nullptr; void *h_surv_args = nullptr; unsigned surv_arg_tick = 0;
    double *h_stream_out = nullptr;
    hipEvent_t ev_chunk[2] = {nullptr, nullptr};
    bool exact_heavy = false;
    hipEvent_t ev_sub0[2] = {nullptr, nullptr};
    hipStream_t stream_surv = nullptr;
    hipEvent_t ev_k1[2] = {nullptr, nullptr};
    hipEvent_t ev_align_gate = nullptr;
    hipStream_t stream_queue_place = nullptr;
    bool screen = false;
    bool in_single_fallback = false;
    unsigned long long *d_topk_scratch = nullptr; int *d_topk_idx = nullptr; float *d_topk_d2 = nullptr;
    double *d_out3 = nullptr;
    unsigned long long *d_blk_part = nullptr; unsigned int *d_done_counter = nullptr;
    hipStream_t stream_alt = nullptr;
    hipEvent_t ev_db = nullptr;
    uint64_t db_version = 0, alt_seen_version = 0;
    bool last_pass_empty = false;
    void *h_pinned = nullptr; size_t pinned_cap = 0;
    double *d_mat_dist = nullptr; int *d_mat_shift = nullptr; void *h_mat = nullptr; size_t mat_cap = 0;
    hipEvent_t ev_mat_k[2] = {nullptr, nullptr}, ev_mat_c[2] = {nullptr, nullptr};
    unsigned long long *d_rank_key = nullptr; unsigned int *d_rank_pos = nullptr; size_t rank_part_cap = 0;
    void *d_rank_out = nullptr; void *h_rank_out = nullptr; size_t rank_out_cap = 0;
    signed char *d_meta_robot = nullptr; int *d_meta_index = nullptr; int meta_n = 0, meta_cap = 0;

    int tree_counter = 0, tree_n = 0;

    int prof_on = 0;
    unsigned prof_tick = 0;
    scl_profile prof{};
    std::vector<scl::PendingEvent> pending;
    std::vector<hipEvent_t> event_pool;

    scl::IcpWorkspace icp_ws;
    scl::IcpWorkspace vox_ws;
    static constexpr int kIcpLanes = 8;
    scl::IcpWorkspace icp_lane_ws[kIcpLanes];
    scl::IcpWorkspace vox_lane_ws[kIcpLanes];
    static constexpr int kIcpBatch = 32;
    scl::IcpWorkspace icp_batch_ws[kIcpBatch];
    scl::IcpWorkspace icp_batch_ctl;
    hipEvent_t ev_lane[kIcpLanes] = {nullptr};
    hipStream_t icp_lane_stream[kIcpLanes] = {nullptr};

    struct StoredCloud { unsigned char *d = nullptr; int n = -1; size_t cap_bytes = 0; };
    std::vector<std::vector<StoredCloud>> kf;
    std::vector<void *> kf_slabs;
    size_t kf_slab_used = 0, kf_slab_cap = 0;
    int kf_stride = 0;
};


namespace scl {

int eng_set_stage_rows(scl_engine *e, int rows);
int eng_stage_from_peer(scl_engine *dst, int j, scl_engine *src, int src_slot, int count = 1);
int eng_stage_values(scl_engine *e, int j, const float *values);
int eng_topk_enqueue(scl_engine *e, int query, int lo, int hi, int k, float eps, bool want_dist, bool *have_dist);
int eng_topk_finish(scl_engine *e, int k, bool have_dist, int *idx, float *d2, double *dist, int *shift, int *found);
int eng_sync_streams(scl_engine *e);
bool eng_would_regrow(const scl_engine *e, int count);
int eng_truncate(scl_engine *e, int n_keep);
int eng_sc_search_ruled(scl_engine *e, const int *queries, const int *lo, const int *hi, const ScRankRule *rules, int n_queries, int k,
                        int *cand_ids, int *cand_shifts, double *cand_dists, int *n_found);
const double *eng_ticket_record(const scl_engine *e, int ticket, int *slot_lo, bool *empty);
hipStream_t eng_stream(const scl_engine *e);
int eng_release_ticket(scl_engine *e, int ticket);

inline ScRankRule sc_intra_rule(int r, int x, int num_exclude_recent)
{
    const long long b = (long long)x - (long long)num_exclude_recent;
    if (b > (long long)INT_MAX) return {r, kScRuleActive, 0};
    return {r, kScRuleActive | kScRuleIndex, b < (long long)INT_MIN ? INT_MIN : (int)b};
}

inline ScRankRule sc_inter_rule(int r, int robot_pre)
{
// ... 39 lines not shown
```

### scl_slam_amd/csrc/kernels.hpp

```cpp
#pragma once

#include <hip/hip_runtime.h>
#include <stdint.h>

#include <stdlib.h>

namespace scl {

#ifdef SCL_DIAGNOSTICS
inline int scl_lab_int(const char *name, int dflt) { const char *e = getenv(name); return e ? atoi(e) : dflt; }
inline bool scl_lab_is(const char *name, const char *value) { const char *e = getenv(name); if (!e) return false; while (*value) if (*e++ != *value++) return false; return true; }
#else
constexpr int scl_lab_int(const char *, int dflt) { return dflt; }
constexpr bool scl_lab_is(const char *, const char *) { return false; }
#endif

constexpr double kBigDist = 10000000.0;
constexpr int kTminEpsOffset = 256;
constexpr int hdesc_sector(int RG) { return ((RG * 8 + 63) / 64) * 8; }
constexpr int hkey_halfs(int S) { return ((S + 31) / 32) * 32; }
constexpr int hkey_store_halfs(int S) { return hkey_halfs(S) + 8; }
constexpr int hkey_row_halfs(int S) { return 2 * hkey_halfs(S) + 8; }
constexpr int halign_P(int S) { return S % 8 == 0 ? 8 : (S % 4 == 0 ? 4 : 0); }
constexpr int halign_CP(int S) { return ((S + 8 + 31) / 32) * 32; }
// ... 38 lines not shown
struct FullTail {
    unsigned long long *blk_part; unsigned int *done_counter; double *out3; int *topk_idx; float *topk_d2;
    int k; float exclude_eps;
};
constexpr int kMaxQueryBatch = 4;
struct QueryBatch {
    int nq;
    int slot[kMaxQueryBatch], base[kMaxQueryBatch], n[kMaxQueryBatch];
    double *out3[kMaxQueryBatch];
    size_t pair_stride;
};
hipError_t launch_sc_distance_batch(const struct DbView &db, const QueryBatch &qb, int SR, double *out_dist, int *out_shift,
                                    float *out_ring_d2, const FullTail &tail, int num_cu, hipStream_t stream);
hipError_t launch_sc_distance_matrix(const struct DbView &db, const int *slots, int nq, int base, int n, int SR,
                                     double *out_dist, int *out_shift, size_t row_stride, int num_cu, hipStream_t stream);
constexpr int kMaxMaskedQueries = 16;
struct MaskedQuery {
    int qslot, slot_base, n; const int *n_dev; const int *cand; const int *starts; const unsigned int *smask;
    double *out_dist; int *out_shift;
};
struct MaskedArgs { const float4 *desc; const double *norm; int nq, parts, spread; MaskedQuery q[kMaxMaskedQueries]; };
bool sc_matrix_supported(const struct DbView &db, int SR);
hipError_t launch_sc_matrix(const struct DbView &db, int SR, const int *qslots, int nq, int lo, int n, const int *starts, const unsigned int *smask,
                            size_t set_stride, double *out_dist, int *out_shift, size_t row_stride, int kr, hipStream_t stream);
constexpr int kScRankMaxK = 32;
constexpr int kScRuleActive = 1, kScRuleNotEqual = 2, kScRuleIndex = 4;
struct ScRankRecord { double dist; int id; int shift; };
struct ScRankRule { int robot, flags, bound; };
struct ScRankArgs {
    const double *dist; const int *shift; unsigned long long row_stride;
    int rows, n, base, k, tiles;
    int plo[16], phi[16];
    const signed char *meta_robot; const int *meta_index;
    ScRankRule rule[16];
    unsigned long long *part_key; unsigned int *part_pos;
    ScRankRecord *out;
};
size_t sc_rank_part_entries(int rows, int n, int k);
hipError_t launch_sc_rank(const ScRankArgs &args, hipStream_t stream);
struct SmallExactQuery {
    int qslot, base, n;
    const float *approx; const int *starts; const unsigned int *smask; const float *ring_d2; unsigned int *t_min;
    int *list; double *out3; int *topk_idx; float *topk_d2;
};
struct SmallExactArgs {
    const float4 *desc; const double *norm; const double *vkey;
    int nq, k; float exclude_eps, two_eps; unsigned long long *surv_stats;
    int every_shift;
    unsigned int seq;
    const SmallExactQuery *q_dev;
    SmallExactQuery q[kMaxQueryBatch];
};
constexpr int kMaxSmallExactQueries = 128;
struct CandExactArgs {
    const float4 *desc; const double *norm; const double *vkey; const float4 *q_desc; const double *q_norm; const double *q_vkey;
    int k; const int *cand_idx; const float *cand_d2; char *out;
    const unsigned long long *lists; int n_lists;
    int *cand_idx_out; float *cand_d2_out;
    unsigned int seq;
};
constexpr size_t cand_seq_offset(int k) { return (((size_t)k * (sizeof(int) * 2 + sizeof(float) + sizeof(double))) + 15) / 16 * 16; }
bool sc_cand_exact_supported(const struct DbView &db, int SR);
hipError_t launch_sc_cand_exact(const struct DbView &db, const struct QueryView &q, int SR, int k, const int *cand_idx, const float *cand_d2, void *pinned_out, hipStream_t stream,
                                unsigned int seq = 0, const unsigned long long *lists = nullptr, int n_lists = 0, int *cand_idx_out = nullptr, float *cand_d2_out = nullptr);
constexpr int kCandMergeMaxKeys = 1024;
bool sc_small_exact_supported(const struct DbView &db, int SR);
hipError_t launch_sc_small_exact(const struct DbView &db, int SR, const SmallExactArgs &args, hipStream_t stream);
bool sc_masked_supported(const struct DbView &db, int SR);
hipError_t launch_sc_masked(const struct DbView &db, int SR, const MaskedQuery *queries, int nq, int parts, hipStream_t stream, bool spread = false);
constexpr int kWideExactBatch = 16;
constexpr int kMaxScreenBatch = 16;
struct ScreenBatch {
    int nq;
    int slot[kMaxScreenBatch], base[kMaxScreenBatch], n[kMaxScreenBatch];
    int buf[kMaxScreenBatch];
    size_t pair_stride;
    float *approx; float *ring_d2; int *survivors; int *n_surv; unsigned int *t_min;
    int *starts;
    unsigned long long *align_fallbacks;
    unsigned long long *surv_stats;
    unsigned int *smask;
    int k; float exclude_eps; int *topk_idx; float *topk_d2;
    float *part;
    bool no_ring_metric;
};
bool sc_screen_supported(const struct DbView &db, int SR);
bool sc_screen_is_wide(const struct DbView &db, int SR);
float sc_screen_eps();
int sc_screen_max_batch(const struct DbView &db, int SR);
size_t sc_screen_scratch_floats(const struct DbView &db, int SR);
constexpr int kScreenAlign = 1, kScreenProducts = 2;
hipError_t launch_sc_screen_batch(const struct DbView &db, const ScreenBatch &sb, int SR, int align_filter, int num_cu, hipStream_t stream,
                                  int phases = kScreenAlign | kScreenProducts, const ScreenBatch *next = nullptr);
hipError_t launch_sc_select_batch(const ScreenBatch &sb, hipStream_t stream);
constexpr int kSurvivorBlocks = 2;
constexpr int kSurvivorArgBytes = 384;
constexpr int kMaxSurvivorQueries = 128;
struct SurvivorPass {
    int nq;
    int slot[kMaxSurvivorQueries], base[kMaxSurvivorQueries], n[kMaxSurvivorQueries], buf[kMaxSurvivorQueries];
    double *out3[kMaxSurvivorQueries];
    size_t pair_stride;
    const float *approx; int *survivors; unsigned int *t_min; double *out_dist; int *out_shift;
    const float *ring_d2; int k; float exclude_eps; int *topk_idx; float *topk_d2;
    unsigned long long *blk_part; unsigned int *done_counter;
    unsigned long long *surv_stats;
    void *d_args; void *h_args;
    int ring_from_keys;
};
constexpr int kSurvivorArgs = 1, kSurvivorKernel = 2;
hipError_t launch_sc_distance_survivors(const struct DbView &db, const SurvivorPass &sp, int SR, int num_cu, hipStream_t stream,
                                        int phases = kSurvivorArgs | kSurvivorKernel);
hipError_t launch_sc_distance_survivors_wide(const struct DbView &db, int nq, const int *query_slot, const int *slot_base, int SR,
                                             const int *const *survivors, const int *const *n_surv, double *const *out_dist, int *const *out_shift,
                                             double *const *out3, int num_cu, hipStream_t stream,
                                             const int *const *starts = nullptr, const unsigned int *const *smask = nullptr);
int sc_align_filter_enabled();

hipError_t launch_sc_distance(const DbView &db, const QueryView &q, const int *cand, int slot_base,
                              int n, int SR, double *out_dist, int *out_shift, int num_cu,
                              hipStream_t stream, float *out_ring_d2 = nullptr, bool *ring_fused = nullptr,
                              const FullTail *tail = nullptr);

bool sc_distance_fuses_ring(const DbView &db, int SR);
hipError_t launch_argmin(const double *dist, const int *shift, int n, double *out3, hipStream_t stream);
hipError_t launch_full_epilogue(const double *dist, const int *shift, const float *ring_d2, int n, int slot_base,
                                int k, float exclude_eps, double *out3, int *topk_idx, float *topk_d2,
                                hipStream_t stream);

constexpr int kTopkMaxBlocks = 256;
constexpr int kTopkMaxK = 64;
static_assert(kTopkMaxK == kTailTopMaxK, "top-k sets share one size");
hipError_t launch_topk_pack(const int *idx, const float *d2, const double *dist, const int *shift, int k, bool have_dist, void *pinned_out, hipStream_t stream);
hipError_t launch_ringkey_lists(const DbView &db, const float *qkey, int lo, int hi, int k, float exclude_eps,
                                unsigned long long *scratch, int *n_lists, hipStream_t stream);
hipError_t launch_topk_merge(const unsigned long long *scratch, int n_lists, int k, int *out_idx, float *out_d2, void *pinned_out, hipStream_t stream);
hipError_t launch_ringkey_topk(const DbView &db, const float *qkey, int lo, int hi, int k,
                               float exclude_eps, unsigned long long *scratch,
                               int *out_idx, float *out_d2, hipStream_t stream);

hipError_t launch_ingest(const float *values, int count, int first_slot,
                         float4 *desc, double *vkey, double *norm, float *rkey, float4 *rkey4,
                         uint2 *hdesc, unsigned int *kmask, unsigned short *hkey, int hstride,
                         int cap, int R, int S, hipStream_t stream, unsigned char *halign = nullptr,
                         int *tiles = nullptr, float *vals_out = nullptr);
hipError_t launch_untile(const float4 *desc_slot, int R, int S, float *values, hipStream_t stream);

constexpr int kMaxScBatch = 16;
constexpr int kScPointsPerWorkgroup = 4096;
struct ScanBatch {
    const unsigned char *points[kMaxScBatch];
    int n[kMaxScBatch];
    int first_wg[kMaxScBatch + 1];
    int count;
};
struct IngestArgs {
    const float *values; int first_slot; float4 *desc; double *vkey; double *norm; float *rkey; float4 *rkey4; uint2 *hdesc; unsigned int *kmask;
    unsigned short *hkey; int hstride, cap, R, S; unsigned char *halign; int *tiles; float *vals_out;
};
hipError_t launch_front_fused(ScanBatch b, int stride_bytes, double lidar_height, double max_radius, int *gtiles, int points_per_wg,
                              const IngestArgs &ia, int n_ingest, hipStream_t stream);
hipError_t launch_make_sc_tiles_init(int *tiles, int count, int R, int S, hipStream_t stream);
hipError_t launch_make_sc_finalize(int *tiles, int count, int R, int S, float *values, hipStream_t stream);
hipError_t launch_make_sc_batch(ScanBatch b, int stride_bytes, int R, int S, double lidar_height, double max_radius,
                                int *tiles, int points_per_wg, int num_cu, hipStream_t stream);
hipError_t launch_atanf_block_checksums(int first_block, int n_blocks, unsigned long long *d_out, hipStream_t stream);
hipError_t launch_bin_paths_selftest(int mode, unsigned long long seed, unsigned long long n, int R, int S, double max_radius, unsigned long long *d_out2, hipStream_t stream);

}
```

### scl_slam_amd/csrc/sc_screen.hip

```cpp
#include <atomic>
#include <type_traits>

#include "align_exact.hpp"
#include "device_common.hpp"
#include "kernels.hpp"

namespace scl {

namespace {

typedef _Float16 h4 __attribute__((ext_vector_type(4)));
typedef _Float16 h8 __attribute__((ext_vector_type(8)));
typedef float f4v __attribute__((ext_vector_type(4)));
typedef float f2 __attribute__((ext_vector_type(2)));
typedef unsigned int u32x4 __attribute__((ext_vector_type(4)));
typedef u32x4 __attribute__((aligned(8))) u32x4_a8;

struct ScreenArgs {
    const double *vkey;
    const uint2 *hdesc; const unsigned int *kmask;
    const double *q_vkey; const float *q_rkey;
    const uint2 *q_hdesc; const unsigned int *q_kmask;
    const _Float16 *hkey; const _Float16 *q_hkey; int hkw;
    const float4 *rkey4; int rk_cap;
// ... 230 lines not shown
#pragma unroll
                    for (int t = 0; t < MT; ++t) acc[t] = __builtin_amdgcn_mfma_f32_16x16x4f32(qa[16 * (b + t) + e], b4[e], acc[t], 0, 0, 0);
                }
            }
            kn2 += __shfl_xor(kn2, 16, kWave);
            kn2 += __shfl_xor(kn2, 32, kWave);
            float w1, w2;
            int b1;
            top2(acc, w1, w2, b1);
            const float nsum = sqrtf(qn2) + sqrtf(kn2);
            const float eps = 4.07e-6f * sqrtf(qn2) * sqrtf(kn2) + 1e-12f * (qn2 + kn2);
            const bool sane = (qn2 < 3.0e38f) && (kn2 < 3.0e38f) && (nsum * nsum < 0.9e14f);
            if (!uniq && sane && (w2 < w1 - 4.0f * eps)) { uniq = true; a1 = b1; }
            amb = __builtin_amdgcn_ballot_w64(mine && !uniq);
        }
        if (mine && uniq) a.starts[c_base + lane] = wrapS(a1 - SR, S);
#ifdef SCL_DIAGNOSTICS
        if (a.align_filter == 3) { amb = 0; if (mine) a.starts[c_base + lane] = 0; }
#endif
        if (amb && lane == 0 && a.fallbacks) atomicAdd(a.fallbacks, (unsigned long long)__popcll(amb));
        while (amb) {
            const int n = __ffsll((long long)amb) - 1;
            amb &= amb - 1;
            int al;
            if constexpr (S / 2 <= kWave) {
                const int ll = lane < L ? lane : L - 1;
                const double2 vk = *reinterpret_cast<const double2 *>(a.vkey + (size_t)(first_slot + n) * S + 2 * ll);
                al = align_keyframe_exact<S>(vk, lane, vk2, vq);
            } else {
                constexpr int SPL = (S + kWave - 1) / kWave, LA = S / SPL;
                const int ll = lane < LA ? lane : LA - 1;
                double vk[SPL];
#pragma unroll
                for (int u = 0; u < SPL; ++u) vk[u] = a.vkey[(size_t)(first_slot + n) * S + SPL * ll + u];
                al = align_keyframe_wide<S>(vk, lane, vk2, vq);
            }
            if (lane == 0) a.starts[c_base + n] = wrapS(al - SR, S);
        }
        if (mine && !ab.skip_d2) {
            const int slot = first_slot + lane;
            float result = 0.0f;
#pragma unroll
            for (int r = 0; r < RG; ++r) {
                const float4 bk = a.rkey4[(size_t)r * a.rk_cap + slot];
                const float4 qk = *reinterpret_cast<const float4 *>(a.q_rkey + 4 * r);
                const float d0 = qk.x - bk.x, d1 = qk.y - bk.y, d2 = qk.z - bk.z, d3 = qk.w - bk.w;
                const float grp = d0 * d0 + d1 * d1 + d2 * d2 + d3 * d3;
                result += grp;
            }
            a.out_d2[c_base + lane] = result;
        }
    }
}

constexpr int kAlignUndecided = -1;
constexpr float kAlignSplitEps = 6.0e-6f;
#ifndef SCL_A2_OCC_WIDE
#define SCL_A2_OCC_WIDE 2
#endif
#ifndef SCL_A2_OCC
#define SCL_A2_OCC 2
#endif
#ifndef SCL_A2_PROBE
#define SCL_A2_PROBE 0
#endif

template <int S>
struct Align2Cfg {
    static constexpr int P = halign_P(S), CP = halign_CP(S);
    static constexpr int ROWS = P ? S / P : 0;
    static constexpr int NTAU = (ROWS + 15) / 16;
    static constexpr int NT = P * NTAU;
    static constexpr int SK = hkey_halfs(S), KS = SK / 32;
    static constexpr int TSTEP = 16 * P / 32;
    static constexpr int ND = KS + TSTEP * (NTAU - 1);
    static constexpr int IMG = halign_img_bytes(S);
    static constexpr int NLD = (IMG + kWave * 16 - 1) / (kWave * 16);
    static constexpr int LDS_WAVE = 2 * IMG > (2 * S + 2) * 8 ? 2 * IMG : ((2 * S + 2) * 8 + 15) / 16 * 16;
    static constexpr int OCC = KS <= 4 ? SCL_A2_OCC : SCL_A2_OCC_WIDE;
};

template <int S, int W>
__device__ __forceinline__ void sc_align2_role(const ScreenBatchArgs &ab, const unsigned char *halign, int u_lo, int u_n,
                                               const int wave_global, const int waves_total, unsigned char *smem_wave)
{
    using C = Align2Cfg<S>;
    constexpr int P = C::P, CP = C::CP, KS = C::KS, NTAU = C::NTAU, NT = C::NT, ND = C::ND, IMG = C::IMG, SK = C::SK, NLD = C::NLD;
    static_assert(P == 4 || P == 8, "alignment image");
    static_assert(S % P == 0 && (16 * P) % 32 == 0 && CP >= S + 8 && IMG % 16 == 0 && S <= 256 && NLD >= 1 && NLD <= 2, "tiling of the shifts");
    constexpr int SR = (W - 1) / 2;
    constexpr int HAB = halign_bytes(S);
    const int lane = threadIdx.x & (kWave - 1);
    const int c16 = lane & 15, j4 = lane >> 4;
    const int cq = c16 < ab.nq ? c16 : 0;
    const ScreenQuery sq = ab.q[cq];
    const bool q_live = c16 < ab.nq;
    int *starts_q = ab.starts + (size_t)sq.buf * (size_t)ab.pair_stride;
    const _Float16 *qk = reinterpret_cast<const _Float16 *>(ab.hkey) + (size_t)sq.slot * (size_t)ab.hkw;
    h8 bq[KS];
#pragma unroll
    for (int kk = 0; kk < KS; ++kk) bq[kk] = *reinterpret_cast<const h8 *>(qk + 32 * kk + 8 * j4);
    const float qnorm = *reinterpret_cast<const float *>(qk + SK);
    const float qerr = *reinterpret_cast<const float *>(qk + SK + 2);
    unsigned int offs[ND];
    {
        int base0 = (8 * j4 - P * c16) % S; base0 = base0 < 0 ? base0 + S : base0;
#pragma unroll
        for (int d = 0; d < ND; ++d) {
            int x = (base0 + 32 * (d - C::TSTEP * (NTAU - 1))) % S; x = x < 0 ? x + S : x;
            offs[d] = (unsigned int)(2 * x);
        }
    }
    const bool use_filter = ab.align_filter != 0;
    const float kNegInf = __int_as_float(0xff800000);
    unsigned long long open_pairs = 0;
    auto frag = [&](const unsigned char *ap) -> h8 {
        if constexpr (P == 8) return *reinterpret_cast<const h8 *>(ap);
        else {
            const uint2 a0 = *reinterpret_cast<const uint2 *>(ap), a1 = *reinterpret_cast<const uint2 *>(ap + 8);
            const u32x4 aw = {a0.x, a0.y, a1.x, a1.y};
            return __builtin_bit_cast(h8, aw);
        }
    };
    const unsigned int loff0 = (unsigned int)lane * 16u, loff1 = (unsigned int)(kWave + lane) * 16u;
    const bool ld1 = NLD > 1 && loff1 < (unsigned int)IMG;
    uint4 pre0 = make_uint4(0, 0, 0, 0), pre1 = make_uint4(0, 0, 0, 0);
    float knorm_pre = 0.f, kerr_pre = 0.f;
    auto image_of = [&](int idx) { idx = idx < u_n ? idx : u_n - 1; return halign + (size_t)(u_lo + idx) * (size_t)HAB; };
    if (wave_global < u_n) {
        const unsigned char *g = image_of(wave_global);
        pre0 = *reinterpret_cast<const uint4 *>(g + 16 + loff0);
        if (NLD > 1) pre1 = *reinterpret_cast<const uint4 *>(g + 16 + (ld1 ? loff1 : 0u));
        knorm_pre = *reinterpret_cast<const float *>(g);
        kerr_pre = *reinterpret_cast<const float *>(g + 4);
    }
    for (int idx = wave_global; idx < u_n; idx += waves_total) {
        wave_fence();
        *reinterpret_cast<uint4 *>(smem_wave + loff0) = pre0;
        if (ld1) *reinterpret_cast<uint4 *>(smem_wave + loff1) = pre1;
        const float knorm = knorm_pre, kerr = kerr_pre;
        wave_fence();
        const unsigned char *g_cur = image_of(idx);
        {
            const unsigned char *g = image_of(idx + waves_total);
            pre0 = *reinterpret_cast<const uint4 *>(g + 16 + loff0);
            if (NLD > 1) pre1 = *reinterpret_cast<const uint4 *>(g + 16 + (ld1 ? loff1 : 0u));
            knorm_pre = *reinterpret_cast<const float *>(g);
            kerr_pre = *reinterpret_cast<const float *>(g + 4);
        }
        float hi[2] = {kNegInf, kNegInf}, lo[2] = {kNegInf, kNegInf};
        h8 af[2][KS];
#pragma unroll
        for (int kk = 0; kk < KS; ++kk) af[0][kk] = frag(smem_wave + offs[kk + C::TSTEP * (NTAU - 1)]);
#pragma unroll
        for (int t = 0; t < NT; ++t) {
            const int rho = t / NTAU, tau = t - rho * NTAU;
            if (t + 1 < NT) {
                const int rn = (t + 1) / NTAU, tn = (t + 1) - rn * NTAU;
#pragma unroll
                for (int kk = 0; kk < KS; ++kk) af[(t + 1) & 1][kk] = frag(smem_wave + rn * (CP * 2) + offs[kk + C::TSTEP * (NTAU - 1 - tn)]);
            }
            f4v acc = {0.f, 0.f, 0.f, 0.f};
#pragma unroll
            for (int kk = 0; kk < KS; ++kk) acc = __builtin_amdgcn_mfma_f32_16x16x32_f16(af[t & 1][kk], bq[kk], acc, 0, 0, 0);
            const int ch = t & 1;
#pragma unroll
            for (int i = 0; i < 4; i += 2) {
                const int sg0 = 16 * tau + 4 * j4 + i, sg1 = sg0 + 1;
                const float x = sg0 < C::ROWS ? __uint_as_float((__float_as_uint(acc[i]) & ~255u) | (unsigned int)(P * sg0 + rho)) : kNegInf;
                const float y = sg1 < C::ROWS ? __uint_as_float((__float_as_uint(acc[i + 1]) & ~255u) | (unsigned int)(P * sg1 + rho)) : kNegInf;
                lo[ch] = fmaxf(lo[ch], __builtin_amdgcn_fmed3f(hi[ch], x, y));
                hi[ch] = fmaxf(fmaxf(hi[ch], x), y);
            }
        }
        auto merge = [](float &h, float &l, float oh, float ol) { l = fmaxf(fmaxf(l, ol), fminf(h, oh)); h = fmaxf(h, oh); };
        merge(hi[0], lo[0], hi[1], lo[1]);
#pragma unroll
        for (int off = 16; off <= 32; off <<= 1) merge(hi[0], lo[0], __shfl_xor(hi[0], off, kWave), __shfl_xor(lo[0], off, kWave));
        const float v1 = hi[0], v2 = lo[0] + 7.0e-5f;
        int a1 = (int)(__float_as_uint(hi[0]) & 255u);
        const bool in_range = qnorm >= 1e-30f && qnorm <= 4.0e6f && knorm >= 1e-30f && knorm <= 4.0e6f &&
                              qnorm <= 1.0e4f * knorm && knorm <= 1.0e4f * qnorm;
        const float lead = (qerr > 0.f && kerr > 0.f) ? fminf(kAlign16Margin, 2.0f * (qerr + kerr + qerr * kerr) * 1.0001f + 1.6e-5f) : kAlign16Margin;
        bool uniq = use_filter && in_range && (v1 == v1) && (v2 < v1 - lead);
        const int ci = u_lo + idx - sq.base;
        const bool mine = q_live && ci >= 0 && ci < sq.n;
        unsigned long long amb = __builtin_amdgcn_ballot_w64(mine && !uniq) & 0xffffull;
        if (SCL_A2_PROBE != 1 && use_filter && amb) {
            const uint4 l0 = *reinterpret_cast<const uint4 *>(g_cur + 16 + IMG + loff0);
            uint4 l1 = make_uint4(0, 0, 0, 0);
            if (NLD > 1) l1 = *reinterpret_cast<const uint4 *>(g_cur + 16 + IMG + (ld1 ? loff1 : 0u));
            *reinterpret_cast<uint4 *>(smem_wave + IMG + loff0) = l0;
            if (ld1) *reinterpret_cast<uint4 *>(smem_wave + IMG + loff1) = l1;
            h8 bql[KS];
#pragma unroll
            for (int kk = 0; kk < KS; ++kk) bql[kk] = *reinterpret_cast<const h8 *>(qk + SK + 8 + 32 * kk + 8 * j4);
            wave_fence();
            float h2 = kNegInf, l2 = kNegInf;
            int g2 = 0;
#pragma unroll
            for (int t = 0; t < NT; ++t) {
                const int rho = t / NTAU, tau = t - rho * NTAU;
                const f4v zero = {0.f, 0.f, 0.f, 0.f};
                f4v hh = zero, xx = zero;
#pragma unroll
                for (int kk = 0; kk < KS; ++kk) {
                    const unsigned char *ap = smem_wave + rho * (CP * 2) + offs[kk + C::TSTEP * (NTAU - 1 - tau)];
                    const h8 ah = frag(ap), al = frag(ap + IMG);
                    const f4v one = __builtin_amdgcn_mfma_f32_16x16x32_f16(ah, bq[kk], zero, 0, 0, 0);
                    hh = kk == 0 ? one : hh + one;
                    xx = __builtin_amdgcn_mfma_f32_16x16x32_f16(ah, bql[kk], xx, 0, 0, 0);
                    xx = __builtin_amdgcn_mfma_f32_16x16x32_f16(al, bq[kk], xx, 0, 0, 0);
                }
#pragma unroll
                for (int i = 0; i < 4; ++i) {
                    const int sg = 16 * tau + 4 * j4 + i;
                    const float c = sg < C::ROWS ? __builtin_fmaf(xx[i], 0x1p-11f, hh[i]) : kNegInf;
                    l2 = fmaxf(l2, fminf(c, h2));
                    g2 = c > h2 ? P * sg + rho : g2;
                    h2 = fmaxf(h2, c);
                }
            }
#pragma unroll
            for (int off = 16; off <= 32; off <<= 1) {
                const float oh = __shfl_xor(h2, off, kWave), ol = __shfl_xor(l2, off, kWave);
                const int og = __shfl_xor(g2, off, kWave);
                l2 = fmaxf(fmaxf(l2, ol), fminf(h2, oh));
                g2 = oh > h2 ? og : g2;
                h2 = fmaxf(h2, oh);
            }
            if (!uniq && in_range && (h2 == h2) && (l2 < h2 - 2.0f * kAlignSplitEps)) { uniq = true; a1 = g2; }
            amb = __builtin_amdgcn_ballot_w64(mine && !uniq) & 0xffffull;
        }
        if (mine && j4 == 0 && uniq) starts_q[ci] = wrapS(a1 - SR, S);
        if (SCL_A2_PROBE == 1 && mine && j4 == 0 && !uniq) starts_q[ci] = kAlignUndecided;
        open_pairs += (unsigned long long)__popcll(amb);
        while (SCL_A2_PROBE != 1 && amb) {
            const int qn = __ffsll((long long)amb) - 1;
            amb &= amb - 1;
            const ScreenQuery oq = ab.q[qn];
            const double *vq = ab.vkey + (size_t)oq.slot * S;
            const double *vkp = ab.vkey + (size_t)(u_lo + idx) * S;
            double *vk2 = reinterpret_cast<double *>(smem_wave);
            int al;
            if constexpr (S / 2 <= kWave) {
                constexpr int L = S >> 1;
                const int ll = lane < L ? lane : L - 1;
                const double2 vk = *reinterpret_cast<const double2 *>(vkp + 2 * ll);
                al = align_keyframe_exact<S>(vk, lane, vk2, vq);
            } else {
                constexpr int SPL = (S + kWave - 1) / kWave, LA = S / SPL;
                const int ll = lane < LA ? lane : LA - 1;
                double vk[SPL];
#pragma unroll
                for (int u = 0; u < SPL; ++u) vk[u] = vkp[SPL * ll + u];
                al = align_keyframe_wide<S>(vk, lane, vk2, vq);
            }
            if (lane == 0) (ab.starts + (size_t)oq.buf * (size_t)ab.pair_stride)[u_lo + idx - oq.base] = wrapS(al - SR, S);
        }
    }
    if (lane == 0 && open_pairs && ab.fallbacks) atomicAdd(ab.fallbacks, open_pairs);
}

template <int RG, int S, int W>
__global__ __launch_bounds__(kScreenWaves * kWave, Align2Cfg<S>::OCC) void sc_align2_kernel(ScreenBatchArgs ab, const unsigned char *halign, int u_lo, int u_n)
{
    extern __shared__ __attribute__((aligned(16))) unsigned char smem_align2[];
    const int wave = __builtin_amdgcn_readfirstlane((int)(threadIdx.x >> 6));
    sc_align2_role<S, W>(ab, halign, u_lo, u_n, (int)blockIdx.x * kScreenWaves + wave, (int)gridDim.x * kScreenWaves,
                         smem_align2 + (size_t)wave * Align2Cfg<S>::LDS_WAVE);
}


template <int S>
__device__ __forceinline__ void rotate_mask(const unsigned long long (&m)[(S + 63) / 64], int s, unsigned long long (&out)[(S + 63) / 64])
{
    constexpr int NW = (S + 63) / 64;
    auto shr = [&](int k, unsigned long long (&o)[NW]) {
        const int w = k >> 6, b = k & 63;
#pragma unroll
        for (int i = 0; i < NW; ++i) {
            const unsigned long long lo = i + w < NW ? m[i + w] : 0ull, hi = i + w + 1 < NW ? m[i + w + 1] : 0ull;
            o[i] = b ? (lo >> b) | (hi << (64 - b)) : lo;
        }
    };
    auto shl = [&](int k, unsigned long long (&o)[NW]) {
        const int w = k >> 6, b = k & 63;
#pragma unroll
        for (int i = 0; i < NW; ++i) {
            const unsigned long long hi = i - w >= 0 && i - w < NW ? m[i - w] : 0ull, lo = i - w - 1 >= 0 && i - w - 1 < NW ? m[i - w - 1] : 0ull;
            o[i] = b ? (hi << b) | (lo >> (64 - b)) : hi;
        }
    };
    unsigned long long r1[NW], r2[NW];
    shr(s, r1);
    shl(S - s, r2);
#pragma unroll
    for (int i = 0; i < NW; ++i) {
        unsigned long long v = r1[i] | r2[i];
        const int top = S - 64 * i;
        if (top < 64) v &= top > 0 ? ((1ull << (top & 63)) - 1ull) : 0ull;
        out[i] = v;
    }
}

template <int RGH, int S, int W, int D, int PROBE>
__device__ __forceinline__ void sc_screen_role(const ScreenBatchArgs &ab, const int qi, const int bid, unsigned char *smem_raw)
{
    constexpr int NWV = kScreenWaves;
    constexpr int MT = (W + 15) / 16;
    constexpr int QSX = S + 16 * MT;
    constexpr int SB = RGH * 8;
    constexpr int KH = SB / 64;
    constexpr int QST = SB + 32;
    constexpr int HS = hdesc_stride_rgh(RGH, S);
    constexpr int SPW = S / NWV;
    constexpr int NST = SPW * KH;
    constexpr int NW64 = (S + 63) / 64;
    constexpr int MW = (NW64 + 1) / 2;
    static_assert(S % NWV == 0 && SB % 64 == 0 && NST % D == 0 && W <= 32 && S <= 224, "tiling");

    const int nbk = ab.nb;
    const ScreenArgs a = screen_args_of(ab, qi);
    const int lane = threadIdx.x & (kWave - 1);
    const int wave = __builtin_amdgcn_readfirstlane((int)(threadIdx.x >> 6));

    unsigned char *Qs = smem_raw;
    uint4 *rotq = reinterpret_cast<uint4 *>(Qs + (size_t)QSX * QST);
    unsigned char *tile = reinterpret_cast<unsigned char *>(rotq + S * MW) + (size_t)wave * (kGroup * kTileStride);
    f4v *part = reinterpret_cast<f4v *>(reinterpret_cast<unsigned char *>(rotq + S * MW) + (size_t)NWV * (kGroup * kTileStride));

    for (int idx = threadIdx.x; idx < QSX * (SB / 16); idx += blockDim.x) {
        const int cx = idx / (SB / 16), ch = idx - cx * (SB / 16);
        const int c = cx < S ? cx : cx - S;
        *reinterpret_cast<uint4 *>(Qs + (size_t)cx * QST + ch * 16) =
            *reinterpret_cast<const uint4 *>(reinterpret_cast<const unsigned char *>(a.q_hdesc) + (size_t)c * SB + ch * 16);
    }
    const bool q_bad = a.q_kmask[7] != 0;
    const float q_err = __uint_as_float(a.q_kmask[6]);
    {
        unsigned long long qm[NW64];
#pragma unroll
        for (int i = 0; i < NW64; ++i) qm[i] = (unsigned long long)a.q_kmask[2 * i] | ((unsigned long long)(2 * i + 1 < 7 ? a.q_kmask[2 * i + 1] : 0u) << 32);
        for (int sft = threadIdx.x; sft < S; sft += blockDim.x) {
            unsigned long long rr[NW64];
            rotate_mask<S>(qm, sft, rr);
#pragma unroll
            for (int i = 0; i < MW; ++i) {
                const unsigned long long lo = rr[2 * i], hi = 2 * i + 1 < NW64 ? rr[2 * i + 1] : 0ull;
                rotq[sft * MW + i] = make_uint4((unsigned int)lo, (unsigned int)(lo >> 32), (unsigned int)hi, (unsigned int)(hi >> 32));
            }
        }
    }

// ... 294 lines not shown

}

bool sc_screen_supported(const DbView &db, int SR)
{
    static const bool off = [] { const char *e = getenv("SCL_SCREEN"); return e && e[0] == '0'; }();
    if (off) return false;
    return (db.RG == 16 && db.R == 64 && db.S == 120 && SR == 6) || sc_screen_is_wide(db, SR);
}

bool sc_screen_is_wide(const DbView &db, int SR) { return db.RG == 20 && db.R == 80 && db.S == 180 && SR == 9; }

float sc_screen_eps() { return kScreenEps; }

hipError_t launch_sc_select_batch(const ScreenBatch &sb, hipStream_t stream)
{
    if (sb.nq < 1 || sb.nq > kMaxScreenBatch) return hipErrorInvalidValue;
    SelectBatchArgs sel{};
    for (int i = 0; i < sb.nq; ++i) {
        SelectArgs &s = sel.q[i];
        s.approx = sb.approx + (size_t)sb.buf[i] * sb.pair_stride; s.d2 = sb.ring_d2 + (size_t)sb.buf[i] * sb.pair_stride;
        s.n = sb.n[i]; s.slot_base = sb.base[i]; s.t_min = sb.t_min + sb.buf[i];
        s.survivors = sb.survivors ? sb.survivors + (size_t)sb.buf[i] * sb.pair_stride : nullptr; s.n_surv = sb.n_surv ? sb.n_surv + sb.buf[i] : nullptr;
        s.surv_stats = sb.surv_stats;
        s.k = sb.k; s.exclude_eps = sb.exclude_eps; s.topk_idx = sb.topk_idx + sb.buf[i] * kTailTopMaxK; s.topk_d2 = sb.topk_d2 + sb.buf[i] * kTailTopMaxK;
    }
    hipLaunchKernelGGL(sc_select_kernel, dim3(sb.nq), dim3(1024), 0, stream, sel);
    return hipGetLastError();
}

#ifndef S2_FRAG_SHIFT
#define S2_FRAG_SHIFT 1
#endif
#ifndef S2NBUF_A
#define S2NBUF_A 9
#endif
#ifndef S2NBUF_B
#define S2NBUF_B 6
#endif
#ifndef S2RS_A
#define S2RS_A 10
#endif
#ifndef S2RS_B
#define S2RS_B 9
#endif
#ifndef S2WV_B
#define S2WV_B 16
#endif
#ifndef S2WV_A
#define S2WV_A 16
#endif
#ifdef S2_STAMP
__device__ unsigned long long g_s2_stamps[4 * 64];
#endif
template <int RG, int S, int W> struct S2Cfg;
template <> struct S2Cfg<16, 120, 13> { static constexpr int NP = 2, NPASS = 1, STEPS = 4, SPK = 1, PS = 13, NQ = 16, RS = S2RS_A, WV = S2WV_A, NBUF = S2NBUF_A; };
#ifdef S2_WIDE_THIRDS
template <> struct S2Cfg<20, 180, 19> { static constexpr int NP = 3, NPASS = 2, STEPS = 4, SPK = 1, PS = 13, NQ = 12, RS = 9, WV = S2WV_B, NBUF = S2NBUF_B; };
#else
#ifndef S2_WIDE_PS
#define S2_WIDE_PS 12
#endif
template <> struct S2Cfg<20, 180, 19> { static constexpr int NP = 5, NPASS = 2, STEPS = 2, SPK = 2, PS = S2_WIDE_PS, NQ = 16, RS = 9, WV = S2WV_B, NBUF = S2NBUF_B; };
#endif
constexpr int kS2PassRows = 13;

constexpr int s2_quad(int S, int SECT, int SPK) { return SPK == 2 ? (S + SECT - 1) * 256 : ((((S + SECT - 1) * 256 / 16) % 4 == 2) ? (S + SECT - 1) * 256 : (S + SECT - 1) * 256 + 32); }
template <int RG, int S, int W> constexpr size_t s2_lds()
{
    using C = S2Cfg<RG, S, W>;
    return (size_t)(C::NQ / (4 * C::SPK)) * s2_quad(S, C::STEPS * C::SPK, C::SPK);
}
template <int RG, int S, int W> constexpr bool s2_group_used(int p, int g4) { return 4 * g4 < kS2PassRows && W - 1 - S2Cfg<RG, S, W>::PS * p - 4 * g4 >= 0; }
template <int RG, int S, int W> constexpr int s2_pass_f4(int p) { int n = 0; for (int g = 0; g < 4; ++g) n += s2_group_used<RG, S, W>(p, g) ? 1 : 0; return n; }
template <int RG, int S, int W> constexpr int s2_pass_off(int p) { int o = 0; for (int q = 0; q < p; ++q) o += s2_pass_f4<RG, S, W>(q); return o; }
template <int RG, int S, int W> constexpr int s2_part_f4() { return s2_pass_off<RG, S, W>(S2Cfg<RG, S, W>::NPASS); }
template <int RG, int S, int W> constexpr int s2_part_floats() { return S2Cfg<RG, S, W>::NP * s2_part_f4<RG, S, W>() * 4; }

struct Screen2Args {
    ScreenBatchArgs prod;
    float *part;
    int u_lo, u_n;
    int nwg;
};

template <int RG, int S, int W>
__global__ __launch_bounds__((S2Cfg<RG, S, W>::WV * kWave), 1) void sc_screen2_kernel(Screen2Args fa)
{
    using C = S2Cfg<RG, S, W>;
    constexpr int WVP = C::WV;
    constexpr int NP = C::NP, NPASS = C::NPASS, STEPS = C::STEPS, NQ = C::NQ, SPK = C::SPK, PS = C::PS;
    constexpr bool AOFF = PS != kS2PassRows;
    constexpr int NB = AOFF ? 1 : NPASS;
    constexpr int LAG = AOFF ? PS / 4 : 0;
    constexpr int RGH = hdesc_rgh(RG);
    constexpr int SB = RGH * 8;
    constexpr int HS = hdesc_stride(RG, S);
    constexpr int SECT = STEPS * SPK;
    constexpr int NIT = S / SECT;
    constexpr int ROWS = S + SECT - 1;
    constexpr int QUAD = s2_quad(S, SECT, SPK);
    constexpr int SPR = 4 * SPK, SCB = 64 / SPK;
    static_assert(SB >= SCB * NP && SB == 64 * ((NP * SCB + 63) / 64) && S % SECT == 0 && SECT == 4 && kS2PassRows + SPK * (STEPS - 1) <= 16 && W <= PS * (NPASS - 1) + kS2PassRows && (!AOFF || (NPASS == 2 && PS == 12))
                  && NQ % SPR == 0 && NQ <= kMaxScreenBatch && (SPK == 1 || SPK == 2), "second form");
    static_assert(SPK == 2 ? QUAD % 256 == 0 : (QUAD / 16) % 4 == 2, "bank slots of the image's blocks");
    extern __shared__ __attribute__((aligned(16))) unsigned char smem2[];
    const ScreenBatchArgs &ab = fa.prod;
    const int lane = threadIdx.x & (kWave - 1);
    const int wave = __builtin_amdgcn_readfirstlane((int)(threadIdx.x >> 6));
    const int b = (int)blockIdx.x, xcd = b & 7, jx = b >> 3;
    const int part = jx % NP;
    const int gi = (jx / NP) * 8 + xcd;
    const int waves_part = (fa.nwg / NP) * WVP;
    const int gw = gi * WVP + wave;

#ifdef S2_STAMP
#define S2_STAMP_AT(slot) do { if ((wave == 0 || wave == 5) && (b == 0 || b == 37) && lane == 0) g_s2_stamps[((b ? 2 : 0) + (wave ? 1 : 0)) * 64 + (slot)] = __builtin_amdgcn_s_memtime(); } while (0)
#else
#define S2_STAMP_AT(slot) do { } while (0)
#endif
    S2_STAMP_AT(32);
    const int c16 = lane & 15, j4 = lane >> 4;
    const int cq = c16 < NQ ? c16 : c16 - 12;
    const ScreenQuery sq = ab.q[cq];
    const int *starts_q = ab.starts + (size_t)sq.buf * (size_t)ab.pair_stride;
    const bool q_live = c16 < ab.nq && c16 < NQ;
    const int lsec = c16 + (SPK == 2 ? (j4 >> 1) : 0);
    const unsigned int a_lane = (unsigned int)(hdesc2_offset(RG, S) * 8 + (((SPK == 2 ? part * 2 + (j4 & 1) : part * 4 + j4)) * (S + 16) + lsec) * 16);
    const unsigned char *hd = reinterpret_cast<const unsigned char *>(ab.hdesc);
    auto kf_base = [&](int k) -> const unsigned char * {
        int idx = gw + k * waves_part;
        idx = idx < fa.u_n ? idx : fa.u_n - 1;
        idx = idx < 0 ? 0 : idx;
        return hd + (size_t)(fa.u_lo + idx) * (size_t)(HS * 8);
    };
    auto first_shift = [&](int k) -> int {
        int idx = gw + k * waves_part;
        idx = idx < fa.u_n ? idx : fa.u_n - 1;
        const int ci = fa.u_lo + idx - sq.base;
        const bool ok = ci >= 0 && ci < sq.n;
        return starts_q[ok ? ci : 0];
    };
    const int nk = gw < fa.u_n ? (fa.u_n - gw + waves_part - 1) / waves_part : 0;
    const unsigned int q_lds = (unsigned int)((cq / SPR) * QUAD + (cq % SPR) * SCB + (SPK == 2 ? (j4 & 1) * 16 + (j4 >> 1) * 256 : j4 * 16));
    const int up16 = ((lane + 16) & 63) * 4;
    constexpr int NGR = (NIT + 3) / 4;
    constexpr int NL = ((NIT - 1) % 4 == 0) ? NGR : NGR + 1;
    constexpr int NBUF = C::NBUF;
    static_assert(NL % NBUF == 0 && NBUF >= 3, "fragment buffers");
    auto load_off = [&](int g) -> unsigned int { const int sct = 16 * g + lsec; return a_lane + (unsigned int)((sct < S ? sct : (sct - S < S ? sct - S : 0)) - lsec) * 16u; };
    u32x4 F[NBUF];
    const unsigned char *base_cur = kf_base(0), *base_nxt = kf_base(1);
    int b_cur = 0, b_nxt = 0;
    {
        constexpr int PPS = 4 / SPK;
        constexpr int NWV = WVP, NPIECE = ROWS * PPS, BATCH = 8;
        constexpr int NBATCH = (NPIECE + BATCH * kWave - 1) / (BATCH * kWave);
        static_assert(NBATCH <= 2 && NQ <= 2 * NWV, "staging turns");
        uint4 pc0, pc1, pc2, pc3, pc4, pc5, pc6, pc7;
        unsigned int ds0, ds1, ds2, ds3, ds4, ds5, ds6, ds7;
#define S2_STAGE_RQ(BASE, r, PC, DS)                                                                                                            \
        {                                                                                                                                       \
            const int idx0 = (BASE) + (r) * kWave + lane;                                                                                       \
            const int idx = idx0 < NPIECE ? idx0 : NPIECE - 1;                                                                                  \
            const int sx = idx / PPS, ch = idx % PPS;                                                                                           \
            const int sct = sx < S ? sx : sx - S;                                                                                               \
            PC = *reinterpret_cast<const uint4 *>(sbase + (unsigned int)(sct * SB + ch * 16));                                                  \
            DS = dbase + (unsigned int)(sx * 256 + ch * 16);                                                                                    \
        }
#define S2_STAGE_ST(BASE, r, PC, DS) if ((BASE) + (r) * kWave + lane < NPIECE) *reinterpret_cast<uint4 *>(smem2 + DS) = PC;
#define S2_STAGE_REQUEST(BASE) S2_STAGE_RQ(BASE, 0, pc0, ds0) S2_STAGE_RQ(BASE, 1, pc1, ds1) S2_STAGE_RQ(BASE, 2, pc2, ds2) S2_STAGE_RQ(BASE, 3, pc3, ds3) \
                               S2_STAGE_RQ(BASE, 4, pc4, ds4) S2_STAGE_RQ(BASE, 5, pc5, ds5) S2_STAGE_RQ(BASE, 6, pc6, ds6) S2_STAGE_RQ(BASE, 7, pc7, ds7)
#define S2_STAGE_STORE(BASE) S2_STAGE_ST(BASE, 0, pc0, ds0) S2_STAGE_ST(BASE, 1, pc1, ds1) S2_STAGE_ST(BASE, 2, pc2, ds2) S2_STAGE_ST(BASE, 3, pc3, ds3) \
                             S2_STAGE_ST(BASE, 4, pc4, ds4) S2_STAGE_ST(BASE, 5, pc5, ds5) S2_STAGE_ST(BASE, 6, pc6, ds6) S2_STAGE_ST(BASE, 7, pc7, ds7)
        if (wave + NWV < NQ) {
            const int q2 = wave + NWV;
            const unsigned char *sbase = reinterpret_cast<const unsigned char *>(ab.hdesc + (size_t)ab.q[q2].slot * HS) + part * SCB;
            const unsigned int dbase = (unsigned int)((q2 / SPR) * QUAD + (q2 % SPR) * SCB);
            if constexpr (NBATCH == 2) { S2_STAGE_REQUEST(0) S2_STAGE_STORE(0) }
            S2_STAGE_REQUEST((NBATCH - 1) * BATCH * kWave)
            S2_STAGE_STORE((NBATCH - 1) * BATCH * kWave)
        }
        const int q1 = wave < NQ ? wave : NQ - 1;
        const unsigned char *sbase = reinterpret_cast<const unsigned char *>(ab.hdesc + (size_t)ab.q[q1].slot * HS) + part * SCB;
        const unsigned int dbase = (unsigned int)((q1 / SPR) * QUAD + (q1 % SPR) * SCB);
        if constexpr (NBATCH == 2) { S2_STAGE_REQUEST(0) S2_STAGE_STORE(0) }
        S2_STAGE_REQUEST((NBATCH - 1) * BATCH * kWave)
        S2_STAMP_AT(61);
        __builtin_amdgcn_sched_barrier(0);
        constexpr int NPRE = NBUF - 1 < 4 ? NBUF - 1 : 4;
#pragma unroll
        for (int j = 0; j < NPRE; ++j) F[j] = *reinterpret_cast<const u32x4 *>(base_cur + load_off(j));
        b_cur = first_shift(0); b_nxt = first_shift(1);
        __builtin_amdgcn_sched_barrier(0);
        S2_STAMP_AT(62);
        if (wave < NQ) { S2_STAGE_STORE((NBATCH - 1) * BATCH * kWave) }
        S2_STAMP_AT(63);
        __builtin_amdgcn_sched_barrier(0);
#pragma unroll
        for (int j = NPRE; j < NBUF - 1; ++j) F[j] = *reinterpret_cast<const u32x4 *>(base_cur + load_off(j));
    }
    __syncthreads();
    S2_STAMP_AT(33);
    if (gw >= fa.u_n) return;
    const unsigned char *preB[NB], *postB[NB];
    int wrapB[NB];
    auto scan_bases = [&](const int first) {
#pragma unroll
        for (int p = 0; p < NB; ++p) {
            int c0 = first + (W - 1) - PS * (AOFF ? 1 : p);
            c0 = c0 >= S ? c0 - S : c0;
            preB[p] = smem2 + (q_lds + (unsigned int)c0 * 256u);
            postB[p] = preB[p] - S * 256;
            wrapB[p] = (S - c0 + SECT - 1) / SECT;
        }
    };
    auto readB = [&](h8 (&dst)[NB][STEPS], const int it) {
#pragma unroll
        for (int p = 0; p < NB; ++p) {
            const unsigned char *qp = (it < wrapB[p] ? preB[p] : postB[p]) + it * SECT * 256;
#pragma unroll
            for (int u = 0; u < STEPS; ++u) dst[p][u] = *reinterpret_cast<const h8 *>(qp + 256 * SPK * u);
        }
    };
    h8 bfr[2][NB][STEPS];
    scan_bases(b_cur);
    readB(bfr[0], 0);
    for (int k = 0; k < nk; ++k) {
        f4v acc[NPASS][STEPS];
#pragma unroll
        for (int p = 0; p < NPASS; ++p)
#pragma unroll
            for (int u = 0; u < STEPS; ++u) acc[p][u] = f4v{0.f, 0.f, 0.f, 0.f};
        if (k < 6) S2_STAMP_AT(34 + 3 * k);
        auto fragment_of = [&](const int it2) -> u32x4 {
            const int g = it2 >> 2, o = it2 & 3;
            u32x4 fr = F[g % NBUF];
            if (o != 0) {
                const u32x4 f0 = F[g % NBUF], f1 = F[(g + 1) % NBUF];
#pragma unroll
                for (int d = 0; d < 4; ++d) {
                    int t = o == 1 ? __builtin_amdgcn_update_dpp(0, (int)f1[d], 0x11C, 0xf, 0xf, true)
                          : o == 2 ? __builtin_amdgcn_update_dpp(0, (int)f1[d], 0x118, 0xf, 0xf, true)
                                   : __builtin_amdgcn_update_dpp(0, (int)f1[d], 0x114, 0xf, 0xf, true);
                    t = o == 1 ? __builtin_amdgcn_update_dpp(t, (int)f0[d], 0x104, 0xf, 0xf, false)
                      : o == 2 ? __builtin_amdgcn_update_dpp(t, (int)f0[d], 0x108, 0xf, 0xf, false)
                               : __builtin_amdgcn_update_dpp(t, (int)f0[d], 0x10C, 0xf, 0xf, false);
                    fr[d] = (unsigned int)t;
                }
            }
            return fr;
        };
        u32x4 fr_cur = F[0];
        u32x4 fr_h1 = fr_cur, fr_h2 = fr_cur, fr_h3 = fr_cur;
#pragma unroll
        for (int it = 0; it < NIT; ++it) {
            const int g = it >> 2, o = it & 3;
#ifdef S2_STAMP
            if (k == 1 && (wave == 0 || wave == 5) && (b == 0 || b == 37) && lane == 0)
                g_s2_stamps[((b ? 2 : 0) + (wave ? 1 : 0)) * 64 + it] = __builtin_amdgcn_s_memtime();
#endif
            if (o == 0) {
                const int j = g + NBUF - 1;
                constexpr int kLastLanes = SPK == 2 ? 16 : 4 * (NIT - 1) + 16 - 16 * (NL - 1);
                if (j == NL - 1 && kLastLanes < 16) { if (c16 < kLastLanes) F[j % NBUF] = *reinterpret_cast<const u32x4 *>(base_cur + load_off(j)); }
                else if (j < NL) F[j % NBUF] = *reinterpret_cast<const u32x4 *>(base_cur + load_off(j));
                else if (j - NL < NBUF - 1) F[j % NBUF] = *reinterpret_cast<const u32x4 *>(base_nxt + load_off(j - NL));
            }
            if (it + 1 < NIT) readB(bfr[(it + 1) & 1], it + 1);
#ifndef S2_NO_READ_PIN
            __builtin_amdgcn_sched_barrier(0);
#endif
            u32x4 fr_nxt = fr_cur;
            if (it + 1 < NIT) fr_nxt = fragment_of(it + 1);
            const h8 af = __builtin_bit_cast(h8, fr_cur);
            const int nmm = (AOFF && it < LAG) ? STEPS : STEPS * NPASS;
            if constexpr (AOFF) {
                const h8 ah = __builtin_bit_cast(h8, fr_h3);
#pragma unroll
                for (int u = 0; u < STEPS; ++u) {
                    acc[1][u] = __builtin_amdgcn_mfma_f32_16x16x32_f16(af, bfr[it & 1][0][u], acc[1][u], 0, 0, 0);
                    if (it >= LAG) acc[0][u] = __builtin_amdgcn_mfma_f32_16x16x32_f16(ah, bfr[it & 1][0][u], acc[0][u], 0, 0, 0);
                }
            } else {
#pragma unroll
                for (int u = 0; u < STEPS; ++u)
#pragma unroll
                    for (int p = 0; p < NPASS; ++p)
                        acc[p][u] = __builtin_amdgcn_mfma_f32_16x16x32_f16(af, bfr[it & 1][p][u], acc[p][u], 0, 0, 0);
            }
#ifndef S2_NO_INTERLEAVE
            if (it + 1 < NIT && ((it + 1) & 3) != 0) {
                if (nmm == STEPS * NPASS) {
#pragma unroll
                    for (int x = 0; x < STEPS * NPASS; ++x) {
                        __builtin_amdgcn_sched_group_barrier(0x008, 1, 0);
                        __builtin_amdgcn_sched_group_barrier(0x002, 8 / (STEPS * NPASS), 0);
                    }
                } else {
#pragma unroll
                    for (int x = 0; x < STEPS; ++x) {
                        __builtin_amdgcn_sched_group_barrier(0x008, 1, 0);
                        __builtin_amdgcn_sched_group_barrier(0x002, 8 / STEPS, 0);
                    }
                }
            }
#endif
#ifndef S2_NO_ITER_BARRIER
            __builtin_amdgcn_sched_barrier(0);
#endif
            if constexpr (AOFF) { fr_h3 = fr_h2; fr_h2 = fr_h1; fr_h1 = fr_cur; }
            fr_cur = fr_nxt;
        }
        if constexpr (AOFF) {
            h8 bx[LAG][NB][STEPS];
#pragma unroll
            for (int x = 0; x < LAG; ++x) readB(bx[x], x);
#pragma unroll
            for (int x = 0; x < LAG; ++x) {
                const h8 ah = __builtin_bit_cast(h8, x == 0 ? fr_h3 : (x == 1 ? fr_h2 : fr_h1));
#pragma unroll
                for (int u = 0; u < STEPS; ++u) acc[0][u] = __builtin_amdgcn_mfma_f32_16x16x32_f16(ah, bx[x][0][u], acc[0][u], 0, 0, 0);
            }
        }
        if (k < 6) S2_STAMP_AT(35 + 3 * k);
#pragma unroll
        for (int j = NGR + NBUF - 1 - NL; j < NBUF - 1; ++j)
            if (j >= 0) F[j % NBUF] = *reinterpret_cast<const u32x4 *>(base_nxt + load_off(j));
        static_assert(NIT >= 2, "");
        scan_bases(b_nxt);
        if constexpr (((NIT - 1) & 1) == 0) __builtin_amdgcn_sched_barrier(0);
        readB(bfr[0], 0);
        {
            const int idx = gw + k * waves_part;
            const int ci = fa.u_lo + idx - sq.base;
            const bool ok = q_live && ci >= 0 && ci < sq.n;
#pragma unroll
            for (int p = 0; p < NPASS; ++p) {
                f4v sum = acc[p][0];
#pragma unroll
                for (int u = 1; u < STEPS; ++u) {
                    constexpr int kMaxSh = SPK * (STEPS - 1);
                    const int sh = SPK * u;
                    float nx[4];
#pragma unroll
                    for (int e2 = 0; e2 < kMaxSh; ++e2)
                        if (e2 < sh) nx[e2] = __int_as_float(__builtin_amdgcn_ds_bpermute(up16, __float_as_int(acc[p][u][e2])));
#pragma unroll
                    for (int i = 0; i < 4; ++i) sum[i] += (i + sh <= 3) ? acc[p][u][(i + sh) & 3] : nx[(i + sh - 4) & 3];
                }
                if (ok && j4 < s2_pass_f4<RG, S, W>(p))
                    *reinterpret_cast<f4v *>(fa.part + (((size_t)c16 * (size_t)ab.pair_stride + (size_t)ci) * NP + part) * (s2_part_f4<RG, S, W>() * 4) + (s2_pass_off<RG, S, W>(p) + j4) * 4) = sum;
            }
        }
        base_cur = base_nxt; base_nxt = kf_base(k + 2);
        b_cur = b_nxt; b_nxt = first_shift(k + 2);
        if (k < 6) S2_STAMP_AT(36 + 3 * k);
    }
    S2_STAMP_AT(60);
}

template <int S>
__device__ __forceinline__ void build_rotq(const unsigned int *q_kmask, uint4 *rotq, int tid, int nthreads)
{
    constexpr int NW64 = (S + 63) / 64, MW = (NW64 + 1) / 2;
    unsigned long long qm[NW64];
#pragma unroll
    for (int i = 0; i < NW64; ++i) qm[i] = (unsigned long long)q_kmask[2 * i] | ((unsigned long long)(2 * i + 1 < 7 ? q_kmask[2 * i + 1] : 0u) << 32);
    for (int sft = tid; sft < S; sft += nthreads) {
        unsigned long long rr[NW64];
        rotate_mask<S>(qm, sft, rr);
#pragma unroll
        for (int i = 0; i < MW; ++i) {
            const unsigned long long lo = rr[2 * i], hi = 2 * i + 1 < NW64 ? rr[2 * i + 1] : 0ull;
            rotq[sft * MW + i] = make_uint4((unsigned int)lo, (unsigned int)(lo >> 32), (unsigned int)hi, (unsigned int)(hi >> 32));
        }
    }
}

template <int RG, int S, int W, bool D2 = true>
struct FinishLoads {
    static constexpr int NPA = S2Cfg<RG, S, W>::NP <= 3 ? S2Cfg<RG, S, W>::NP : 3;
    static constexpr int PF4 = s2_part_f4<RG, S, W>();
    static constexpr int NPF = NPA * PF4;
    static constexpr int MW = (((S + 63) / 64) + 1) / 2;
    static constexpr bool kRingUpFront = NPF * 4 + RG * 4 <= 100;
    uint4 km[MW]; unsigned int kflag; float kerr; int b_raw; f4v pv[NPF]; const f4v *rest; float4 bk[(D2 && kRingUpFront) ? RG : 1];
};
template <int RG, int S, int W, bool D2 = true>
__device__ __forceinline__ FinishLoads<RG, S, W, D2> sc_screen2_finish_request(const Screen2Args &fa, const ScreenArgs &a, const int qi, const int ci)
{
    using L = FinishLoads<RG, S, W, D2>;
    const ScreenBatchArgs &ab = fa.prod;
    L l;
    if constexpr (D2 && L::kRingUpFront) {
        const int slot = a.slot_base + ci;
#pragma unroll
        for (int r = 0; r < RG; ++r) l.bk[r] = a.rkey4[(size_t)r * a.rk_cap + slot];
    }
    const unsigned int *kp = a.kmask + (size_t)(a.slot_base + ci) * 8;
#pragma unroll
    for (int i = 0; i < L::MW; ++i) l.km[i] = *reinterpret_cast<const uint4 *>(kp + 4 * i);
    {
        const uint2 ef = *reinterpret_cast<const uint2 *>(kp + 6);
        l.kerr = __uint_as_float(ef.x); l.kflag = ef.y;
    }
    l.b_raw = a.starts[ci];
    const f4v *pp = reinterpret_cast<const f4v *>(fa.part + ((size_t)qi * (size_t)ab.pair_stride + (size_t)ci) * (size_t)s2_part_floats<RG, S, W>());
#pragma unroll
    for (int i = 0; i < L::NPF; ++i) l.pv[i] = pp[i];
    l.rest = pp + L::NPF;
    return l;
}
template <int RG, int S, int W, bool MASKS = true, bool D2 = true>
__device__ __forceinline__ float sc_screen2_finish_compute(const ScreenArgs &a, const int ci, const uint4 *rotq, const float4 *qkey, const bool q_bad, const float q_err, FinishLoads<RG, S, W, D2> &l, float &pair_eps)
{
    using C = S2Cfg<RG, S, W>;
    using L = FinishLoads<RG, S, W, D2>;
    constexpr int NP = C::NP, NPASS = C::NPASS, MW = L::MW, PS = C::PS;
    const float kInf = __int_as_float(0x7f800000);
    if (MW == 2) { l.km[MW - 1].z = 0u; l.km[MW - 1].w = 0u; }
    const bool b_open = l.b_raw < 0;
    const int b0 = b_open ? 0 : l.b_raw;
    float dmin = kInf;
    float dsh[W];
    const bool want_mask = MASKS && a.out_smask != nullptr;
    const float e_pair = (q_err + l.kerr) * 1.002f;
    const bool e_ok = e_pair >= 0.0f && e_pair < 1.0f;
    float hi_min = kInf;
    int ne_min = 0x7fffffff;
    float dlo[MASKS ? W : 1];
#pragma unroll
    for (int t = 0; t < W; ++t) { dsh[t] = kInf; if (MASKS) dlo[MASKS ? t : 0] = kInf; }
    constexpr int NPA = L::NPA;
    f4v psum[NPASS][4];
#pragma unroll
    for (int p = 0; p < NPASS; ++p)
#pragma unroll
// ... 59 lines not shown
        for (int t = 0; t < W; ++t) m |= ((exact_only || dlo[MASKS ? t : 0] <= hi_min) ? 1u : 0u) << t;
        a.out_smask[ci] = b_open ? 0u : m;
    }
    if constexpr (D2) {
        const int slot = a.slot_base + ci;
        float result = 0.0f;
#pragma unroll
        for (int r = 0; r < RG; ++r) {
            float4 bk;
            if constexpr (L::kRingUpFront) bk = l.bk[r]; else bk = a.rkey4[(size_t)r * a.rk_cap + slot];
            const float4 qk = qkey[r];
            const float d0 = qk.x - bk.x, d1 = qk.y - bk.y, d2 = qk.z - bk.z, d3 = qk.w - bk.w;
            const float grp = d0 * d0 + d1 * d1 + d2 * d2 + d3 * d3;
            result += grp;
        }
        a.out_d2[ci] = result;
    }
    return exact_only ? kInf : dmin;
}
template <int RG, int S, int W, bool MASKS = true, bool D2 = true>
__device__ __forceinline__ void sc_screen2_finish_body(const Screen2Args &fa, const int qi, const int chunk)
{
    constexpr int NW64 = (S + 63) / 64, MW = (NW64 + 1) / 2;
    const ScreenBatchArgs &ab = fa.prod;
    const ScreenArgs a = screen_args_of(ab, qi);
    __shared__ uint4 rotq[S * MW];
    __shared__ float wmin[4], wmax[4];
    __shared__ float4 qkey[D2 ? RG : 1];
    const int ci = (int)(chunk * blockDim.x + threadIdx.x);
    const bool live = ci < a.n;
    float4 qk_mine = make_float4(0.0f, 0.0f, 0.0f, 0.0f);
    if constexpr (D2) { if (threadIdx.x < RG) qk_mine = reinterpret_cast<const float4 *>(a.q_rkey)[threadIdx.x]; }
    FinishLoads<RG, S, W, D2> ld = sc_screen2_finish_request<RG, S, W, D2>(fa, a, qi, live ? ci : 0);
    build_rotq<S>(a.q_kmask, rotq, (int)threadIdx.x, (int)blockDim.x);
    const bool q_bad = a.q_kmask[7] != 0;
    if constexpr (D2) { if (threadIdx.x < RG) qkey[threadIdx.x] = qk_mine; }
    __syncthreads();
#pragma unroll
    for (int i = 0; i < FinishLoads<RG, S, W, D2>::NPF; ++i) asm("" : "+v"(ld.pv[i]));
    const float kInf = __int_as_float(0x7f800000);
    float contrib = kInf, peps = 0.0f;
    if (live) contrib = sc_screen2_finish_compute<RG, S, W, MASKS, D2>(a, ci, rotq, qkey, q_bad, __uint_as_float(a.q_kmask[6]), ld, peps);
    contrib = -wave_max_f32_dpp(-contrib);
    peps = wave_max_f32_dpp(peps);
    if ((threadIdx.x & 63) == 0) { wmin[threadIdx.x >> 6] = contrib; wmax[threadIdx.x >> 6] = peps; }
    __syncthreads();
    if (threadIdx.x == 0) {
        const float m = fminf(fminf(wmin[0], wmin[1]), fminf(wmin[2], wmin[3]));
        if (m < kInf) atomicMin(a.t_min, float_to_ordered_u(m));
        const float pe = fmaxf(fmaxf(wmax[0], wmax[1]), fmaxf(wmax[2], wmax[3]));
        if (pe > 0.0f) atomicMax(a.t_min + kTminEpsOffset, __float_as_uint(pe));
    }
}

__device__ __forceinline__ bool finish_block_of(const int fb, const int nq, const int chunks, int &qi, int &chunk)
{
    const int x = fb & 7, s = fb >> 3, g = s / nq;
    chunk = 8 * g + x; qi = s - g * nq;
    return chunk < chunks;
}
static int finish_blocks(int chunks, int nq) { return 8 * ((chunks + 7) / 8) * nq; }

template <int RG, int S, int W>
__global__ __launch_bounds__(256) void sc_screen2_finish_kernel(Screen2Args fa, int chunks)
{
    int qi, chunk;
    if (!finish_block_of((int)blockIdx.x, fa.prod.nq, chunks, qi, chunk)) return;
    sc_screen2_finish_body<RG, S, W>(fa, qi, chunk);
}

template <int RG, int S, int W>
__global__ __launch_bounds__(kScreenWaves * kWave, 2) void sc_screen2_tail_kernel(Screen2Args fa, ScreenBatchArgs nb, int align_blocks, int chunks)
{
    extern __shared__ __attribute__((aligned(16))) unsigned char smem_tail[];
    const int b = (int)blockIdx.x;
    if (b < align_blocks) { sc_align_role<RG, S, W>(nb, b, smem_tail); return; }
    int qi, chunk;
    if (!finish_block_of(b - align_blocks, fa.prod.nq, chunks, qi, chunk)) return;
    sc_screen2_finish_body<RG, S, W>(fa, qi, chunk);
}

template <int RG, int S, int W, bool MASKS = true, bool D2 = true>
__global__ __launch_bounds__(kScreenWaves * kWave, Align2Cfg<S>::OCC) void sc_screen2_tail2_kernel(Screen2Args fa, ScreenBatchArgs nb, const unsigned char *halign, int u_lo, int u_n,
                                                                                     int align_blocks, int chunks)
{
    extern __shared__ __attribute__((aligned(16))) unsigned char smem_tail2[];
#ifdef SCL_TAIL_FINISH_FIRST
    const int fblocks = (int)gridDim.x - align_blocks;
    const int b = (int)blockIdx.x < fblocks ? (int)blockIdx.x + align_blocks : (int)blockIdx.x - fblocks;
#else
    const int b = (int)blockIdx.x;
#endif
    if (b < align_blocks) {
        const int wave = __builtin_amdgcn_readfirstlane((int)(threadIdx.x >> 6));
        sc_align2_role<S, W>(nb, halign, u_lo, u_n, b * kScreenWaves + wave, align_blocks * kScreenWaves, smem_tail2 + (size_t)wave * Align2Cfg<S>::LDS_WAVE);
        return;
    }
    int qi, chunk;
    if (!finish_block_of(b - align_blocks, fa.prod.nq, chunks, qi, chunk)) return;
    sc_screen2_finish_body<RG, S, W, MASKS, D2>(fa, qi, chunk);
}

static bool screen_second_form()
{
    static const int form = [] { const char *e = getenv("SCL_SCREEN_FORM"); return e ? atoi(e) : 2; }();
    return form != 1;
}
static int screen_v2_min_env()
{
    static const int v = [] { const char *e = getenv("SCL_SCREEN_V2_MIN"); return e ? atoi(e) : 0; }();
    return v;
}
int sc_screen_max_batch(const DbView &db, int SR)
{
    return (sc_screen_is_wide(db, SR) && screen_second_form()) ? S2Cfg<20, 180, 19>::NQ : kMaxScreenBatch;
}
size_t sc_screen_scratch_floats(const DbView &db, int SR)
{
    return sc_screen_is_wide(db, SR) ? (size_t)S2Cfg<20, 180, 19>::NQ * s2_part_floats<20, 180, 19>() : (size_t)S2Cfg<16, 120, 13>::NQ * s2_part_floats<16, 120, 13>();
}

static int fill_screen_args(const DbView &db, const ScreenBatch &sb, int align_filter, ScreenBatchArgs *ab)
{
    ab->vkey = db.vkey; ab->rkey = db.rkey; ab->hdesc = db.hdesc; ab->kmask = db.kmask; ab->rkey4 = db.rkey4; ab->hkey = db.hkey; ab->hkw = hkey_row_halfs(db.S);
    ab->starts = sb.starts; ab->approx = sb.approx; ab->ring_d2 = sb.ring_d2; ab->t_min = sb.t_min; ab->fallbacks = sb.align_fallbacks; ab->smask = sb.smask;
    ab->pair_stride = (unsigned long long)sb.pair_stride;
    ab->S = db.S; ab->R4 = 4 * db.RG; ab->hstride = db.hstride; ab->rk_cap = db.cap; ab->align_filter = align_filter;
    ab->nq = sb.nq;
    int nmax = 0;
    for (int i = 0; i < sb.nq; ++i) {
        if (sb.n[i] <= 0) return -1;
        ab->q[i] = ScreenQuery{sb.slot[i], sb.base[i], sb.n[i], sb.buf[i]};
        nmax = sb.n[i] > nmax ? sb.n[i] : nmax;
    }
    for (int i = sb.nq; i < kMaxScreenBatch; ++i) ab->q[i] = ab->q[0];
    return nmax;
}

template <int RG, int S, int W, int OCC0, int OCC1>
static hipError_t launch_screen_grid(const DbView &db, const ScreenBatch &sb, int align_filter, int num_cu, hipStream_t stream, int phases,
                                     const ScreenBatch *next)
{
    constexpr int RGH = hdesc_rgh(RG);
    ScreenBatchArgs ab{};
    const int nmax = fill_screen_args(db, sb, align_filter, &ab);
    if (nmax < 0) return hipErrorInvalidValue;
    const int ngroups = (nmax + kGroup - 1) / kGroup;
    static_assert(halign_bytes(S) > 0, "alignment image");
    if (db.hstride != hdesc_stride(RG, S) || !sb.starts || !db.halign) return hipErrorInvalidValue;
    static std::atomic<bool> attr_set_dev[64];
    int dev_ = 0; (void)hipGetDevice(&dev_);
    std::atomic<bool> &attr_set = attr_set_dev[dev_ & 63];
    static const int variant = scl_lab_int("SCL_SCREEN_VARIANT", 0);
    void (*kern)(ScreenFusedArgs) = sc_screen_kernel<RG, S, W, 15, OCC0>;
#ifdef SCL_DIAGNOSTICS
    if (variant == 1) kern = sc_screen_kernel<RG, S, W, 15, OCC1>;
    if (variant == 2) kern = sc_screen_kernel<RG, S, W, 5, OCC0>;
    static const int probe = scl_lab_int("SCL_SCREEN_PROBE", 0);
    if (probe == 2) kern = sc_screen_kernel<RG, S, W, 15, OCC0, 2>;
#else
    const int probe = 0;
#endif
    constexpr int MTA = (S + 15) / 16, MT = (W + 15) / 16, QSX = S + 16 * MT, MW = ((S + 63) / 64 + 1) / 2;
    const size_t lds0 = (size_t)S * 8 + (size_t)(32 * MTA) * 4 + (size_t)2 * (16 * MTA + hkey_halfs(S) + 8) * 2 +
                        (size_t)kScreenWaves * ((2 * S + 2) * 8);
    const size_t lds1 = (size_t)QSX * (RGH * 8 + 32) + (size_t)S * MW * 16 + (size_t)kScreenWaves * kGroup * kTileStride +
                        (size_t)(2 * kScreenWaves * MT) * kWave * 16;
    if (!attr_set.load(std::memory_order_acquire)) {
        hipError_t e = hipFuncSetAttribute((const void *)sc_screen_kernel<RG, S, W, 15, OCC0>, hipFuncAttributeMaxDynamicSharedMemorySize, 128 * 1024);
        if (e == hipSuccess) e = hipFuncSetAttribute((const void *)sc_align_kernel<RG, S, W>, hipFuncAttributeMaxDynamicSharedMemorySize, 128 * 1024);
        if (e != hipSuccess) return e;
#ifdef SCL_DIAGNOSTICS
        (void)hipFuncSetAttribute((const void *)sc_screen_kernel<RG, S, W, 15, OCC1>, hipFuncAttributeMaxDynamicSharedMemorySize, 128 * 1024);
        (void)hipFuncSetAttribute((const void *)sc_screen_kernel<RG, S, W, 5, OCC0>, hipFuncAttributeMaxDynamicSharedMemorySize, 128 * 1024);
        (void)hipFuncSetAttribute((const void *)sc_screen_kernel<RG, S, W, 15, OCC0, 2>, hipFuncAttributeMaxDynamicSharedMemorySize, 128 * 1024);
#endif
        attr_set.store(true, std::memory_order_release);
    }
    auto align_blocks = [&](int groups, int nq, bool beside_products) {
        int b = (groups + kScreenWaves - 1) / kScreenWaves;
        static const int cap_env = scl_lab_int("SCL_ALIGN_WGS", 0);
        int cap = cap_env > 0 ? cap_env : (beside_products ? 2 * num_cu / (nq > 0 ? nq : 1) : num_cu);
        if (cap < 1) cap = 1;
        return b > cap ? cap : b;
    };
    const int v2_min = screen_v2_min_env() > 0 ? screen_v2_min_env() : (S <= 128 ? 4 : 2);
    auto second_form_for = [&](const ScreenBatch &b) {
        return screen_second_form() && b.part && probe == 0 && variant == 0 && b.nq >= v2_min && b.nq <= S2Cfg<RG, S, W>::NQ;
    };
    const bool use_v2 = second_form_for(sb);
    const bool next_v2 = next && second_form_for(*next);
    ab.skip_d2 = use_v2 ? 1 : 0;
    constexpr size_t lds_a2 = (size_t)kScreenWaves * Align2Cfg<S>::LDS_WAVE;
    auto union_of = [](const ScreenBatch &b, int *lo_out, int *n_out) {
        int lo = b.base[0], hi = b.base[0] + b.n[0];
        for (int i = 1; i < b.nq; ++i) { lo = b.base[i] < lo ? b.base[i] : lo; hi = b.base[i] + b.n[i] > hi ? b.base[i] + b.n[i] : hi; }
        *lo_out = lo; *n_out = hi - lo;
    };
    auto align2_blocks = [&](int u_n) {
        static const int env = scl_lab_int("SCL_ALIGN2_WGS", 0);
        int b = (u_n + kScreenWaves * 3 - 1) / (kScreenWaves * 3);
        const int cap = env > 0 ? env : 2 * num_cu;
        b = b > cap ? cap : b;
        return b < 1 ? 1 : b;
    };
    const bool self_align = (phases & kScreenAlign) && (phases & kScreenProducts) && !use_v2 && probe == 0 && !scl_lab_int("SCL_SELF_ALIGN_OFF", 0);
    if ((phases & kScreenAlign) && probe != 3 && !self_align) {
        if (use_v2) {
            int ulo, un;
            union_of(sb, &ulo, &un);
            hipLaunchKernelGGL((sc_align2_kernel<RG, S, W>), dim3(align2_blocks(un)), dim3(kScreenWaves * kWave), lds_a2, stream, ab, db.halign, ulo, un);
        } else {
            ab.nb = align_blocks(ngroups, sb.nq, false);
            hipLaunchKernelGGL((sc_align_kernel<RG, S, W>), dim3(ab.nb * sb.nq), dim3(kScreenWaves * kWave), lds0, stream, ab);
        }
        hipError_t e = hipGetLastError();
        if (e != hipSuccess) return e;
    }
    if (probe == 4 || !(phases & kScreenProducts)) return hipSuccess;
    if (use_v2) {
        static std::atomic<bool> attr2_dev[64];
        std::atomic<bool> &attr2 = attr2_dev[dev_ & 63];
        if (!attr2.load(std::memory_order_acquire)) {
            hipError_t e = hipFuncSetAttribute((const void *)sc_screen2_kernel<RG, S, W>, hipFuncAttributeMaxDynamicSharedMemorySize, (int)(s2_lds<RG, S, W>()));
            if (e != hipSuccess) return e;
            attr2.store(true, std::memory_order_release);
        }
        Screen2Args f2{};
        f2.prod = ab; f2.part = sb.part;
        union_of(sb, &f2.u_lo, &f2.u_n);
        constexpr int WGU = 8 * S2Cfg<RG, S, W>::NP;
        int nwg = (num_cu / WGU) * WGU;
        if (nwg < WGU) nwg = WGU;
        f2.nwg = nwg;
        hipError_t e = hipSuccess;
        hipLaunchKernelGGL((sc_screen2_kernel<RG, S, W>), dim3(nwg), dim3(S2Cfg<RG, S, W>::WV * kWave), (s2_lds<RG, S, W>()), stream, f2);
        if ((e = hipGetLastError()) != hipSuccess) return e;
        const int chunks = (nmax + 255) / 256;
        const dim3 fgrid(finish_blocks(chunks, sb.nq)), ablock(kScreenWaves * kWave);
        if (!next) {
            hipLaunchKernelGGL((sc_screen2_finish_kernel<RG, S, W>), fgrid, dim3(256), 0, stream, f2, chunks);
            return hipGetLastError();
        }
        if (next->nq < 1 || next->nq > kMaxScreenBatch) return hipErrorInvalidValue;
        ScreenBatchArgs nb{};
        const int nmax2 = fill_screen_args(db, *next, align_filter, &nb);
        if (nmax2 < 0) return hipErrorInvalidValue;
        nb.skip_d2 = next_v2 ? 1 : 0;
        int ulo = 0, un = 0, ablocks;
        if (next_v2) {
            union_of(*next, &ulo, &un);
            ablocks = align2_blocks(un);
        } else {
            const int ng2 = (nmax2 + kGroup - 1) / kGroup;
            int per_q = 3 * num_cu / next->nq;
            per_q = per_q < 1 ? 1 : per_q;
            nb.nb = (ng2 + kScreenWaves - 1) / kScreenWaves;
            nb.nb = nb.nb > per_q ? per_q : nb.nb;
            ablocks = nb.nb * next->nq;
        }
        static const int tail_env = scl_lab_int("SCL_SCREEN_TAIL", 1);
        if (tail_env) {
            const dim3 tgrid(ablocks + finish_blocks(chunks, sb.nq));
            const bool d2 = !sb.no_ring_metric;
            if (!next_v2) hipLaunchKernelGGL((sc_screen2_tail_kernel<RG, S, W>), tgrid, ablock, lds0, stream, f2, nb, ablocks, chunks);
            else if (sb.smask && d2) hipLaunchKernelGGL((sc_screen2_tail2_kernel<RG, S, W, true, true>), tgrid, ablock, lds_a2, stream, f2, nb, db.halign, ulo, un, ablocks, chunks);
            else if (sb.smask) hipLaunchKernelGGL((sc_screen2_tail2_kernel<RG, S, W, true, false>), tgrid, ablock, lds_a2, stream, f2, nb, db.halign, ulo, un, ablocks, chunks);
            else if (d2) hipLaunchKernelGGL((sc_screen2_tail2_kernel<RG, S, W, false, true>), tgrid, ablock, lds_a2, stream, f2, nb, db.halign, ulo, un, ablocks, chunks);
            else hipLaunchKernelGGL((sc_screen2_tail2_kernel<RG, S, W, false, false>), tgrid, ablock, lds_a2, stream, f2, nb, db.halign, ulo, un, ablocks, chunks);
            return hipGetLastError();
        }
        hipLaunchKernelGGL((sc_screen2_finish_kernel<RG, S, W>), fgrid, dim3(256), 0, stream, f2, chunks);
        if ((e = hipGetLastError()) != hipSuccess) return e;
        if (next_v2) hipLaunchKernelGGL((sc_align2_kernel<RG, S, W>), dim3(ablocks), ablock, lds_a2, stream, nb, db.halign, ulo, un);
        else hipLaunchKernelGGL((sc_align_kernel<RG, S, W>), dim3(ablocks), ablock, lds0, stream, nb);
        return hipGetLastError();
    }
    ScreenFusedArgs fa{};
    fa.prod = ab;
    int blocks = num_cu * 2;
    if (blocks > ngroups) blocks = ngroups;
    if (blocks > kScreenMaxBlocks) blocks = kScreenMaxBlocks;
    fa.prod.nb = blocks;
    fa.prod.self_align = self_align ? 1 : 0;
    int extra = 0;
    if (next && probe != 3) {
        if (next->nq < 1 || next->nq > kMaxScreenBatch) return hipErrorInvalidValue;
        const int nmax2 = fill_screen_args(db, *next, align_filter, &fa.next);
        if (nmax2 < 0) return hipErrorInvalidValue;
        fa.next.skip_d2 = next_v2 ? 1 : 0;
        fa.next.nb = align_blocks((nmax2 + kGroup - 1) / kGroup, next->nq, true);
        extra = fa.next.nb * next->nq;
#ifdef SCL_DIAGNOSTICS
        if (probe == 5 || probe == 6) fa.next.align_filter = probe == 5 ? 2 : 3;
#endif
    }
    const size_t lds = (extra || self_align) && lds0 > lds1 ? lds0 : lds1;
    fa.align_blocks = extra;
    const int patterned = fused_patterned_blocks(sb.nq, blocks, extra);
    const int slots = 8 * ((blocks + 7) >> 3);
    const int grid = patterned + (extra > slots ? extra - slots : 0);
    hipLaunchKernelGGL(kern, dim3(grid), dim3(kScreenWaves * kWave), lds, stream, fa);
    return hipGetLastError();
}

hipError_t launch_sc_screen_batch(const DbView &db, const ScreenBatch &sb, int SR, int align_filter, int num_cu, hipStream_t stream, int phases,
                                  const ScreenBatch *next)
{
    if (sb.nq < 1 || sb.nq > kMaxScreenBatch || !sc_screen_supported(db, SR)) return hipErrorInvalidValue;
    if (sc_screen_is_wide(db, SR)) return launch_screen_grid<20, 180, 19, 2, 2>(db, sb, align_filter, num_cu, stream, phases, next);
    return launch_screen_grid<16, 120, 13, 2, 3>(db, sb, align_filter, num_cu, stream, phases, next);
}

}

#ifdef S2_STAMP
extern "C" int scl_debug_s2_stamps(unsigned long long *out)
{
    return (int)hipMemcpyFromSymbol(out, HIP_SYMBOL(scl::g_s2_stamps), sizeof(unsigned long long) * 4 * 64);
}
#endif
```

### scl_slam_amd/engine.py

```python
import ctypes
import os
from ctypes import POINTER, byref, c_char_p, c_double, c_float, c_int, c_int8, c_uint64, c_void_p

import numpy as np

from ._native import load_library

QUERY_STAGED = -1


class SclConfig(ctypes.Structure):
    _fields_ = [
        ("num_ring", c_int), ("num_sector", c_int), ("num_candidates", c_int),
        ("dist_thres", c_double), ("lidar_height", c_double), ("max_radius", c_double),
        ("num_exclude_recent", c_int), ("tree_making_period", c_int),
        ("search_ratio", c_double), ("knn_exclude_eps", c_float),
        ("device", c_int), ("initial_capacity", c_int),
    ]


class IcpParams(ctypes.Structure):
    _fields_ = [
        ("max_iterations", c_int), ("max_correspondence_dist", c_double),
        ("transformation_epsilon", c_double), ("euclidean_fitness_epsilon", c_double),
# ... 962 lines not shown
        self._check(self._lib.scl_target_normals(self._h, a.ctypes.data_as(c_void_p), n, stride, radius, _ptr(out, c_float)), "scl_target_normals")
        return out[:n]

    def registration_eval_plane_batch(self, src, tgts, transforms, max_dist, normal_radius):
        s, ns, stride = _cloud(src)
        arrs, ptrs, counts, m, stride_t = self._cloud_list(tgts)
        if m and stride != stride_t:
            raise ValueError("source and targets must share a record layout")
        Tm = _f32(np.asarray(transforms)).reshape(m, 16)
        k = max(m, 1)
        nv = np.zeros(k, np.int32); ni = np.zeros(k, np.int32); npl = np.zeros(k, np.int32); su = np.zeros((k, 29), np.float64)
        self._check(self._lib.scl_registration_eval_plane_batch(self._h, s.ctypes.data_as(c_void_p), ns, ptrs, _ptr(counts, c_int), m, stride,
                                                                _ptr(Tm, c_float), max_dist, normal_radius, _ptr(nv, c_int), _ptr(ni, c_int),
                                                                _ptr(npl, c_int), _ptr(su, c_double)),
                    "scl_registration_eval_plane_batch")
        return RegistrationPlaneEval(ns, nv[:m], ni[:m], npl[:m], su[:m])

    def registration_eval_plane_batch_from_store(self, src, src_leaf, robot, keys_pre, search_num, poses_pre, leaf, transforms, max_dist,
                                                 normal_radius, min_src_points=300, min_tgt_points=1000):
        a, n, stride = _cloud(src)
        keys = np.ascontiguousarray(keys_pre, dtype=np.int32); m = keys.size
        Tp = _f32(np.asarray(poses_pre)).reshape(m, 2 * search_num + 1, 16)
        Tm = _f32(np.asarray(transforms)).reshape(m, 16)
        k = max(m, 1)
        nv = np.zeros(k, np.int32); ni = np.zeros(k, np.int32); npl = np.zeros(k, np.int32); su = np.zeros((k, 29), np.float64)
        ns = c_int(); nt = np.zeros(k, np.int32)
        self._check(self._lib.scl_registration_eval_plane_batch_from_store(
            self._h, a.ctypes.data_as(c_void_p), n, stride, src_leaf, robot, m, _ptr(keys, c_int), search_num, _ptr(Tp, c_float), leaf,
            _ptr(Tm, c_float), min_src_points, min_tgt_points, max_dist, normal_radius, _ptr(nv, c_int), _ptr(ni, c_int), _ptr(npl, c_int),
            _ptr(su, c_double), byref(ns), _ptr(nt, c_int)), "scl_registration_eval_plane_batch_from_store")
        return RegistrationPlaneEval(ns.value, nv[:m], ni[:m], npl[:m], su[:m], nt[:m])

    def loop_eval_plane_batch_from_store(self, robot, key_cur, pose_cur, keys_pre, search_num, poses_pre, leaf, transforms, max_dist,
                                         normal_radius, min_src_points=300, min_tgt_points=1000):
        keys = np.ascontiguousarray(keys_pre, dtype=np.int32); m = keys.size
        Tc = _f32(np.asarray(pose_cur)).reshape(16)
        Tp = _f32(np.asarray(poses_pre)).reshape(m, 2 * search_num + 1, 16)
        Tm = _f32(np.asarray(transforms)).reshape(m, 16)
        k = max(m, 1)
        nv = np.zeros(k, np.int32); ni = np.zeros(k, np.int32); npl = np.zeros(k, np.int32); su = np.zeros((k, 29), np.float64)
        ns = c_int(); nt = np.zeros(k, np.int32)
        self._check(self._lib.scl_loop_eval_plane_batch_from_store(
            self._h, robot, key_cur, _ptr(Tc, c_float), m, _ptr(keys, c_int), search_num, _ptr(Tp, c_float), leaf, _ptr(Tm, c_float),
            min_src_points, min_tgt_points, max_dist, normal_radius, _ptr(nv, c_int), _ptr(ni, c_int), _ptr(npl, c_int), _ptr(su, c_double),
            byref(ns), _ptr(nt, c_int)), "scl_loop_eval_plane_batch_from_store")
        return RegistrationPlaneEval(ns.value, nv[:m], ni[:m], npl[:m], su[:m], nt[:m])

    @staticmethod
    def registration_information_plane(sums):
        lib = load_library(); _bind(lib)
        su = np.ascontiguousarray(sums, dtype=np.float64).reshape(29)
        info = np.empty(36, np.float64); grad = np.empty(6, np.float64)
        rc = lib.scl_registration_information_plane(_ptr(su, c_double), _ptr(info, c_double), _ptr(grad, c_double))
        if rc != 0:
            raise SclError(rc, "scl_registration_information_plane")
        return info.reshape(6, 6), grad

    @staticmethod
    def loop_guess_from_shift(shift, num_sector, pose_cur, pose_pre):
        lib = load_library(); _bind(lib)
        pc = _f32(np.asarray(pose_cur)).reshape(6); pp = _f32(np.asarray(pose_pre)).reshape(6)
        G = np.empty(16, np.float32)
        rc = lib.scl_loop_guess_from_shift(int(shift), int(num_sector), _ptr(pc, c_float), _ptr(pp, c_float), _ptr(G, c_float))
        if rc != 0:
            raise SclError(rc, "scl_loop_guess_from_shift")
        return G.reshape(4, 4)

    def profile_enable(self, on=True):
        self._check(self._lib.scl_profile_enable(self._h, int(on)), "scl_profile_enable")

    def profile_reset(self):
        self._check(self._lib.scl_profile_reset(self._h), "scl_profile_reset")

    def profile(self):
        p = SclProfile()
        self._check(self._lib.scl_profile_get(self._h, byref(p)), "scl_profile_get")
        return {name: getattr(p, name) for name, _ in SclProfile._fields_}

    def alignment_stats(self, reset=False):
        a, b = c_uint64(0), c_uint64(0)
        self._check(self._lib.scl_alignment_stats(self._h, byref(a), byref(b), int(bool(reset))), "scl_alignment_stats")
        return int(a.value), int(b.value)

    def survivor_stats(self, reset=False):
        q, s, m = c_uint64(0), c_uint64(0), c_uint64(0)
        self._check(self._lib.scl_survivor_stats(self._h, byref(q), byref(s), byref(m), int(bool(reset))), "scl_survivor_stats")
        return int(q.value), int(s.value), int(m.value)

    def device_name(self):
        buf = ctypes.create_string_buffer(256)
        self._check(self._lib.scl_device_name(self._h, buf, 256), "scl_device_name")
        return buf.value.decode()


class ScanContextDescriptor:

    def __init__(self, numRing=20, numSector=60, numCandidates=3, distThres=0.14, lidarHeight=1.65,
                 maxRadius=80.0, numExcludeRecent=100, treeMakingPeriod=10, searchRatio=0.1, **engine_kw):
        self.engine = ScanContextEngine(numRing, numSector, numCandidates, distThres, lidarHeight, maxRadius,
                                        numExcludeRecent, treeMakingPeriod, searchRatio, **engine_kw)

    def makeAndSaveDescriptorAndKey(self, scan, robot, index):
        return self.engine.make_and_save(scan, robot, index)

    def saveDescriptorAndKey(self, descriptorMat, robot, index):
        self.engine.save_from_wire(descriptorMat, robot, index)

    def detectIntraLoopClosureID(self, currentPtr):
        lid, shift, _ = self.engine.detect_intra(currentPtr)
        return lid, shift

    def detectInterLoopClosureID(self, currentPtr):
        lid, yaw, _ = self.engine.detect_inter(currentPtr)
        return lid, yaw

    def getIndex(self, key):
        return self.engine.get_index(key)

    def getSize(self, idIn=-1):
        return self.engine.get_size(idIn)
```

Measured before the change: 2.549 billion.

## Prebuild screen LDS images and shift table during the align2 pass

Adds extra prep blocks to the align2 (and tail2) launches that copy query descriptor pieces into a pre-laid-out LDS image in global memory. The align pass also writes per-keyframe start shifts into a compact 16-wide table. The screen2 kernel gets a PREP variant that stages LDS linearly from that image and reads shifts from the compact table through buffer loads. This is meant to remove scattered staging and gather costs from the screen kernel, at the cost of extra memory, ownership tracking across two slots, and more blocks in the align launch.

```diff
diff --git a/include/scl_engine.h b/include/scl_engine.h
--- a/include/scl_engine.h
+++ b/include/scl_engine.h
@@ -255,6 +255,7 @@
 int  scl_profile_get(scl_engine *e, scl_profile *out);
 void scl_debug_icp_tile_stats(unsigned long long out[16], int reset);
 int  scl_alignment_stats(scl_engine *e, uint64_t *pairs, uint64_t *fallbacks, int reset);
+int  scl_screen_prepared_launches(scl_engine *e, uint64_t *launches, int reset);
 int  scl_survivor_stats(scl_engine *e, uint64_t *queries, uint64_t *survivors, uint64_t *max_survivors, int reset);
 int  scl_device_name(const scl_engine *e, char *buf, int buflen);
 int  scl_host_copy_rate(scl_engine *e, size_t bytes, int reps, double *gbytes_per_s);
diff --git a/scl_slam_amd/csrc/engine.hip b/scl_slam_amd/csrc/engine.hip
--- a/scl_slam_amd/csrc/engine.hip
+++ b/scl_slam_amd/csrc/engine.hip
@@ -234,8 +234,25 @@
     return SCL_OK;
 }
 
+int ensure_prep(scl_engine *e)
+{
+    if (!e->prep_on || (e->d_prep && e->prep_km_cap >= e->cap)) return SCL_OK;
+    const size_t images = sc_screen_prep_bytes(db_view(e), e->SR);
+    if (!images) return SCL_OK;
+    for (int &o : e->prep_owner) o = -1;
+    dev_free(e->d_prep); e->prep_bytes = 0; e->prep_km_cap = 0;
+    const size_t bytes = images + (size_t)e->cap * 64;
+    int rc;
+    if ((rc = dev_alloc(e, &e->d_prep, bytes * scl_engine::kPrepSlots))) return rc;
+    SCL_HIP(e, hipMemsetAsync(e->d_prep, 0, bytes * scl_engine::kPrepSlots, e->stream));
+    SCL_HIP(e, hipStreamSynchronize(e->stream));
+    e->prep_bytes = bytes; e->prep_km_cap = e->cap;
+    return SCL_OK;
+}
+
 int ensure_sets(scl_engine *e, size_t n)
 {
+    if (int prc = ensure_prep(e)) return prc;
     if (n <= e->set_stride && e->pair_cap >= e->set_stride * scl_engine::kScreenSets) return SCL_OK;
     const size_t stride = n + n / 4 + 64;
     int rc = ensure_pairs(e, stride * scl_engine::kScreenSets);
@@ -537,6 +554,7 @@
     hipDeviceProp_t prop;
     if (hipGetDeviceProperties(&prop, e->device) == hipSuccess && prop.multiProcessorCount > 0)
         e->num_cu = prop.multiProcessorCount;
+    { const char *v = getenv("SCL_SCREEN_PREP"); e->prep_on = !(v && atoi(v) == 0); }
     if (hipStreamCreateWithFlags(&e->stream, hipStreamNonBlocking) != hipSuccess) return bail(SCL_ERR_HIP);
     {
         int lo_p = 0, hi_p = 0;
@@ -633,7 +651,7 @@
     for (hipStream_t cs : e->stream_copy_x) if (cs) { (void)hipStreamSynchronize(cs); (void)hipStreamDestroy(cs); }
     for (void *hp : e->host_allocs) (void)hipHostFree(hp);
     dev_free(e->d_dist); dev_free(e->d_shift); dev_free(e->d_cand); dev_free(e->d_ring_d2);
-    dev_free(e->d_approx); dev_free(e->d_starts); dev_free(e->d_surv); dev_free(e->d_nsurv); dev_free(e->d_tmin); dev_free(e->d_part);
+    dev_free(e->d_approx); dev_free(e->d_starts); dev_free(e->d_surv); dev_free(e->d_nsurv); dev_free(e->d_tmin); dev_free(e->d_part); dev_free(e->d_prep);
     dev_free(e->d_align_fallbacks);
     dev_free(e->d_smask);
     if (e->d_mat_dist) (void)hipFree(e->d_mat_dist);
@@ -1316,6 +1334,11 @@
         sb.survivors = nullptr; sb.n_surv = nullptr; sb.t_min = e->d_tmin;
         sb.smask = (g.masks || sc_screen_is_wide(db_view(e), e->SR)) ? e->d_smask : nullptr;
         sb.part = e->d_part + (g.part_half ? e->part_cap / 2 : 0);
+        if (e->d_prep) {
+            const int ps = stream == e->stream ? 0 : 1;
+            sb.prep = e->d_prep + (size_t)ps * e->prep_bytes; sb.prep_owner = &e->prep_owner[ps]; sb.prep_id = g.set0;
+            sb.prep_km_cap = e->prep_km_cap; sb.prep_launches = &e->prep_launches;
+        }
         sb.no_ring_metric = g.keys_later;
         sb.k = e->cfg.num_candidates; sb.exclude_eps = e->cfg.knn_exclude_eps; sb.topk_idx = e->d_topk_idx; sb.topk_d2 = e->d_topk_d2;
     };
@@ -2499,6 +2522,8 @@
     }
     sb.approx = e->d_approx; sb.starts = e->d_starts; sb.align_fallbacks = e->d_align_fallbacks; sb.ring_d2 = e->d_ring_d2; sb.survivors = e->d_surv; sb.n_surv = e->d_nsurv; sb.t_min = e->d_tmin;
     sb.k = e->cfg.num_candidates; sb.exclude_eps = e->cfg.knn_exclude_eps; sb.topk_idx = e->d_topk_idx; sb.topk_d2 = e->d_topk_d2;
+    if ((rc = ensure_prep(e))) return rc;
+    if (e->d_prep) { sb.prep = e->d_prep; sb.prep_owner = &e->prep_owner[0]; sb.prep_id = 0; sb.prep_km_cap = e->prep_km_cap; sb.prep_launches = &e->prep_launches; }
     SCL_HIP(e, launch_sc_screen_batch(db_view(e), sb, e->SR, sc_align_filter_enabled(), e->num_cu, e->stream));
     SCL_HIP(e, hipMemsetAsync(e->d_tmin, 0xff, sizeof(unsigned int) * (size_t)n_queries, e->stream));
     SCL_HIP(e, hipMemsetAsync(e->d_tmin + kTminEpsOffset, 0, sizeof(unsigned int) * (size_t)n_queries, e->stream));
@@ -3933,6 +3958,16 @@
     return SCL_OK;
 }
 
+int scl_screen_prepared_launches(scl_engine *e, uint64_t *launches, int reset)
+{
+    if (!e || !launches) return SCL_ERR_INVALID_ARG;
+    if (e->front) return fail(e, SCL_ERR_UNSUPPORTED, "screen_prepared_launches: call it on a one-GPU engine");
+    std::lock_guard<std::mutex> lk(e->mu);
+    *launches = (uint64_t)e->prep_launches;
+    if (reset) e->prep_launches = 0;
+    return SCL_OK;
+}
+
 int scl_survivor_stats(scl_engine *e, uint64_t *queries, uint64_t *survivors, uint64_t *max_survivors, int reset)
 {
     if (!e) return SCL_ERR_INVALID_ARG;
diff --git a/scl_slam_amd/csrc/engine_internal.hpp b/scl_slam_amd/csrc/engine_internal.hpp
--- a/scl_slam_amd/csrc/engine_internal.hpp
+++ b/scl_slam_amd/csrc/engine_internal.hpp
@@ -72,6 +72,9 @@
     static constexpr int kScreenSets = SCL_SCREEN_SETS;
     float *d_approx = nullptr; int *d_starts = nullptr; int *d_surv = nullptr;
     unsigned int *d_smask = nullptr; size_t smask_cap = 0;
+    static constexpr int kPrepSlots = 2;
+    unsigned char *d_prep = nullptr; size_t prep_bytes = 0; int prep_km_cap = 0; int prep_owner[kPrepSlots] = {-1, -1}; bool prep_on = true;
+    unsigned long long prep_launches = 0;
     float *d_part = nullptr; size_t part_cap = 0;
     int *d_nsurv = nullptr; unsigned int *d_tmin = nullptr;
     unsigned long long *d_align_fallbacks = nullptr; uint64_t align_pairs = 0;
diff --git a/scl_slam_amd/csrc/kernels.hpp b/scl_slam_amd/csrc/kernels.hpp
--- a/scl_slam_amd/csrc/kernels.hpp
+++ b/scl_slam_amd/csrc/kernels.hpp
@@ -144,12 +144,17 @@
     unsigned int *smask;
     int k; float exclude_eps; int *topk_idx; float *topk_d2;
     float *part;
+    unsigned char *prep;
+    int prep_km_cap;
+    unsigned long long *prep_launches;
+    int *prep_owner; int prep_id;
     bool no_ring_metric;
 };
 bool sc_screen_supported(const struct DbView &db, int SR);
 bool sc_screen_is_wide(const struct DbView &db, int SR);
 float sc_screen_eps();
 int sc_screen_max_batch(const struct DbView &db, int SR);
+size_t sc_screen_prep_bytes(const struct DbView &db, int SR);
 size_t sc_screen_scratch_floats(const struct DbView &db, int SR);
 constexpr int kScreenAlign = 1, kScreenProducts = 2;
 hipError_t launch_sc_screen_batch(const struct DbView &db, const ScreenBatch &sb, int SR, int align_filter, int num_cu, hipStream_t stream,
diff --git a/scl_slam_amd/csrc/sc_screen.hip b/scl_slam_amd/csrc/sc_screen.hip
--- a/scl_slam_amd/csrc/sc_screen.hip
+++ b/scl_slam_amd/csrc/sc_screen.hip
@@ -336,7 +336,7 @@
 
 template <int S, int W>
 __device__ __forceinline__ void sc_align2_role(const ScreenBatchArgs &ab, const unsigned char *halign, int u_lo, int u_n,
-                                               const int wave_global, const int waves_total, unsigned char *smem_wave)
+                                               const int wave_global, const int waves_total, unsigned char *smem_wave, int *km = nullptr)
 {
     using C = Align2Cfg<S>;
     constexpr int P = C::P, CP = C::CP, KS = C::KS, NTAU = C::NTAU, NT = C::NT, ND = C::ND, IMG = C::IMG, SK = C::SK, NLD = C::NLD;
@@ -396,11 +396,15 @@
         wave_fence();
         const unsigned char *g_cur = image_of(idx);
         {
+            const int left = u_n - idx - waves_total;
+            const int nx_lanes = (left < 1 ? left : 1) * kWave;
             const unsigned char *g = image_of(idx + waves_total);
-            pre0 = *reinterpret_cast<const uint4 *>(g + 16 + loff0);
-            if (NLD > 1) pre1 = *reinterpret_cast<const uint4 *>(g + 16 + (ld1 ? loff1 : 0u));
-            knorm_pre = *reinterpret_cast<const float *>(g);
-            kerr_pre = *reinterpret_cast<const float *>(g + 4);
+            if (lane < nx_lanes) {
+                pre0 = *reinterpret_cast<const uint4 *>(g + 16 + loff0);
+                if (NLD > 1) pre1 = *reinterpret_cast<const uint4 *>(g + 16 + (ld1 ? loff1 : 0u));
+                knorm_pre = *reinterpret_cast<const float *>(g);
+                kerr_pre = *reinterpret_cast<const float *>(g + 4);
+            }
         }
         float hi[2] = {kNegInf, kNegInf}, lo[2] = {kNegInf, kNegInf};
         h8 af[2][KS];
@@ -488,6 +492,8 @@
         }
         if (mine && j4 == 0 && uniq) starts_q[ci] = wrapS(a1 - SR, S);
         if (SCL_A2_PROBE == 1 && mine && j4 == 0 && !uniq) starts_q[ci] = kAlignUndecided;
+        if (km && j4 == 0 && !(mine && !uniq)) km[(size_t)idx * 16 + c16] = (mine && uniq) ? wrapS(a1 - SR, S) : 0;
+        if (SCL_A2_PROBE == 1 && km && mine && j4 == 0 && !uniq) km[(size_t)idx * 16 + c16] = kAlignUndecided;
         open_pairs += (unsigned long long)__popcll(amb);
         while (SCL_A2_PROBE != 1 && amb) {
             const int qn = __ffsll((long long)amb) - 1;
@@ -511,19 +517,12 @@
                 al = align_keyframe_wide<S>(vk, lane, vk2, vq);
             }
             if (lane == 0) (ab.starts + (size_t)oq.buf * (size_t)ab.pair_stride)[u_lo + idx - oq.base] = wrapS(al - SR, S);
+            if (lane == 0 && km) km[(size_t)idx * 16 + qn] = wrapS(al - SR, S);
         }
     }
     if (lane == 0 && open_pairs && ab.fallbacks) atomicAdd(ab.fallbacks, open_pairs);
 }
 
-template <int RG, int S, int W>
-__global__ __launch_bounds__(kScreenWaves * kWave, Align2Cfg<S>::OCC) void sc_align2_kernel(ScreenBatchArgs ab, const unsigned char *halign, int u_lo, int u_n)
-{
-    extern __shared__ __attribute__((aligned(16))) unsigned char smem_align2[];
-    const int wave = __builtin_amdgcn_readfirstlane((int)(threadIdx.x >> 6));
-    sc_align2_role<S, W>(ab, halign, u_lo, u_n, (int)blockIdx.x * kScreenWaves + wave, (int)gridDim.x * kScreenWaves,
-                         smem_align2 + (size_t)wave * Align2Cfg<S>::LDS_WAVE);
-}
 
 
 template <int S>
@@ -984,9 +983,44 @@
     float *part;
     int u_lo, u_n;
     int nwg;
+    const unsigned char *prep;
 };
-
+template <int RG, int S, int W> constexpr size_t s2_prep_part_bytes() { return (s2_lds<RG, S, W>() + 127) / 128 * 128; }
+template <int RG, int S, int W> __host__ __device__ constexpr size_t s2_prep_images_bytes() { return S2Cfg<RG, S, W>::NP * s2_prep_part_bytes<RG, S, W>(); }
+template <int RG, int S, int W> __device__ __forceinline__ int *s2_prep_km(unsigned char *prep) { return prep ? reinterpret_cast<int *>(prep + s2_prep_images_bytes<RG, S, W>()) : nullptr; }
+constexpr int kPrepBlocks = 32;
 template <int RG, int S, int W>
+__device__ __forceinline__ void sc_screen2_prep_role(const ScreenBatchArgs &ab, unsigned char *prep, const int block, const int nblocks)
+{
+    using C = S2Cfg<RG, S, W>;
+    constexpr int NP = C::NP, NQ = C::NQ, SPK = C::SPK, SECT = C::STEPS * SPK, ROWS = S + SECT - 1;
+    constexpr int QUAD = s2_quad(S, SECT, SPK), SPR = 4 * SPK, SCB = 64 / SPK, PPS = 4 / SPK;
+    constexpr int SB = hdesc_rgh(RG) * 8, HS = hdesc_stride(RG, S);
+    constexpr int PER_SCAN = ROWS * PPS, TOTAL = NP * NQ * PER_SCAN;
+    static_assert((size_t)(NQ / SPR - 1) * QUAD + (size_t)(ROWS - 1) * 256 + (size_t)(SPR - 1) * SCB + (size_t)PPS * 16 <= s2_lds<RG, S, W>(), "the image's last piece");
+    const unsigned char *hd = reinterpret_cast<const unsigned char *>(ab.hdesc);
+    auto piece = [&](const int i, const unsigned char *&src, unsigned char *&dst) {
+        const int pq = i / PER_SCAN, r = i - pq * PER_SCAN;
+        const int part = pq / NQ, q = pq - part * NQ;
+        const int sx = r / PPS, ch = r - sx * PPS;
+        const int sct = sx < S ? sx : sx - S;
+        src = hd + (size_t)ab.q[q].slot * (size_t)(HS * 8) + (unsigned int)(sct * SB + part * SCB + ch * 16);
+        dst = prep + (size_t)part * s2_prep_part_bytes<RG, S, W>() + (unsigned int)((q / SPR) * QUAD + sx * 256 + (q % SPR) * SCB + ch * 16);
+    };
+    const int stride = nblocks * (int)blockDim.x;
+    for (int i = block * (int)blockDim.x + (int)threadIdx.x; i < TOTAL; i += 2 * stride) {
+        const bool two = i + stride < TOTAL;
+        const unsigned char *s0, *s1;
+        unsigned char *d0, *d1;
+        piece(i, s0, d0);
+        piece(two ? i + stride : i, s1, d1);
+        const uint4 v0 = *reinterpret_cast<const uint4 *>(s0), v1 = *reinterpret_cast<const uint4 *>(s1);
+        *reinterpret_cast<uint4 *>(d0) = v0;
+        if (two) *reinterpret_cast<uint4 *>(d1) = v1;
+    }
+}
+
+template <int RG, int S, int W, bool PREP = false>
 __global__ __launch_bounds__((S2Cfg<RG, S, W>::WV * kWave), 1) void sc_screen2_kernel(Screen2Args fa)
 {
     using C = S2Cfg<RG, S, W>;
@@ -1025,7 +1059,6 @@
     const int c16 = lane & 15, j4 = lane >> 4;
     const int cq = c16 < NQ ? c16 : c16 - 12;
     const ScreenQuery sq = ab.q[cq];
-    const int *starts_q = ab.starts + (size_t)sq.buf * (size_t)ab.pair_stride;
     const bool q_live = c16 < ab.nq && c16 < NQ;
     const int lsec = c16 + (SPK == 2 ? (j4 >> 1) : 0);
     const unsigned int a_lane = (unsigned int)(hdesc2_offset(RG, S) * 8 + (((SPK == 2 ? part * 2 + (j4 & 1) : part * 4 + j4)) * (S + 16) + lsec) * 16);
@@ -1036,12 +1069,29 @@
         idx = idx < 0 ? 0 : idx;
         return hd + (size_t)(fa.u_lo + idx) * (size_t)(HS * 8);
     };
+    constexpr int kRsrcWord3 = 0x00020000;
+    auto has_kf = [&](int k) -> bool { return gw + k * waves_part < fa.u_n; };
+    auto kf_rsrc = [&](int k) {
+        return __builtin_amdgcn_make_buffer_rsrc(const_cast<unsigned char *>(kf_base(k)), 0, has_kf(k) ? HS * 8 : 0, kRsrcWord3);
+    };
+    auto starts_rsrc = [&](int k) {
+        return __builtin_amdgcn_make_buffer_rsrc(const_cast<int *>(ab.starts), 0, __builtin_amdgcn_readfirstlane(has_kf(k) ? -1 : 0), kRsrcWord3);
+    };
+    const unsigned int starts_lane = (unsigned int)sq.buf * (unsigned int)ab.pair_stride;
+    auto km_rsrc = [&](int k) {
+        return __builtin_amdgcn_make_buffer_rsrc(const_cast<unsigned char *>(fa.prep + s2_prep_images_bytes<RG, S, W>()), 0,
+                                                 __builtin_amdgcn_readfirstlane(has_kf(k) ? fa.u_n * 64 : 0), kRsrcWord3);
+    };
     auto first_shift = [&](int k) -> int {
         int idx = gw + k * waves_part;
         idx = idx < fa.u_n ? idx : fa.u_n - 1;
-        const int ci = fa.u_lo + idx - sq.base;
-        const bool ok = ci >= 0 && ci < sq.n;
-        return starts_q[ok ? ci : 0];
+        idx = idx < 0 ? 0 : idx;
+        if constexpr (PREP) return (int)__builtin_amdgcn_raw_buffer_load_b32(km_rsrc(k), idx * 64 + cq * 4, 0, 0);
+        else {
+            const int ci = fa.u_lo + idx - sq.base;
+            const bool ok = ci >= 0 && ci < sq.n;
+            return (int)__builtin_amdgcn_raw_buffer_load_b32(starts_rsrc(k), (int)((starts_lane + (unsigned int)(ok ? ci : 0)) * 4u), 0, 0);
+        }
     };
     const int nk = gw < fa.u_n ? (fa.u_n - gw + waves_part - 1) / waves_part : 0;
     const unsigned int q_lds = (unsigned int)((cq / SPR) * QUAD + (cq % SPR) * SCB + (SPK == 2 ? (j4 & 1) * 16 + (j4 >> 1) * 256 : j4 * 16));
@@ -1052,7 +1102,8 @@
     static_assert(NL % NBUF == 0 && NBUF >= 3, "fragment buffers");
     auto load_off = [&](int g) -> unsigned int { const int sct = 16 * g + lsec; return a_lane + (unsigned int)((sct < S ? sct : (sct - S < S ? sct - S : 0)) - lsec) * 16u; };
     u32x4 F[NBUF];
-    const unsigned char *base_cur = kf_base(0), *base_nxt = kf_base(1);
+    auto rs_cur = kf_rsrc(0), rs_nxt = kf_rsrc(1);
+    auto frag_load = [&](decltype(rs_cur) rs, int g) -> u32x4 { return __builtin_amdgcn_raw_buffer_load_b128(rs, (int)load_off(g), 0, 0); };
     int b_cur = 0, b_nxt = 0;
     {
         constexpr int PPS = 4 / SPK;
@@ -1075,32 +1126,50 @@
                                S2_STAGE_RQ(BASE, 4, pc4, ds4) S2_STAGE_RQ(BASE, 5, pc5, ds5) S2_STAGE_RQ(BASE, 6, pc6, ds6) S2_STAGE_RQ(BASE, 7, pc7, ds7)
 #define S2_STAGE_STORE(BASE) S2_STAGE_ST(BASE, 0, pc0, ds0) S2_STAGE_ST(BASE, 1, pc1, ds1) S2_STAGE_ST(BASE, 2, pc2, ds2) S2_STAGE_ST(BASE, 3, pc3, ds3) \
                              S2_STAGE_ST(BASE, 4, pc4, ds4) S2_STAGE_ST(BASE, 5, pc5, ds5) S2_STAGE_ST(BASE, 6, pc6, ds6) S2_STAGE_ST(BASE, 7, pc7, ds7)
-        if (wave + NWV < NQ) {
-            const int q2 = wave + NWV;
-            const unsigned char *sbase = reinterpret_cast<const unsigned char *>(ab.hdesc + (size_t)ab.q[q2].slot * HS) + part * SCB;
-            const unsigned int dbase = (unsigned int)((q2 / SPR) * QUAD + (q2 % SPR) * SCB);
+        constexpr int NLIN = (int)(s2_lds<RG, S, W>() / 16), NTH = WVP * kWave;
+        static_assert(!PREP || (s2_lds<RG, S, W>() % 16 == 0 && NLIN <= 8 * NTH), "linear staging");
+#define S2_LIN_RQ(r, PC, DS)                                                                                                                    \
+        if constexpr ((r) * NTH < NLIN) {                                                                                                       \
+            const int i0 = (r) * NTH + (int)threadIdx.x;                                                                                        \
+            DS = (unsigned int)(i0 < NLIN ? i0 : NLIN - 1) * 16u;                                                                               \
+            PC = *reinterpret_cast<const uint4 *>(img + DS);                                                                                    \
+        }
+#define S2_LIN_ST(r, PC, DS) if constexpr ((r) * NTH < NLIN) { if ((r) * NTH + (int)threadIdx.x < NLIN) *reinterpret_cast<uint4 *>(smem2 + DS) = PC; }
+        if constexpr (PREP) {
+            const unsigned char *img = fa.prep + (size_t)part * s2_prep_part_bytes<RG, S, W>();
+            S2_LIN_RQ(0, pc0, ds0) S2_LIN_RQ(1, pc1, ds1) S2_LIN_RQ(2, pc2, ds2) S2_LIN_RQ(3, pc3, ds3)
+            S2_LIN_RQ(4, pc4, ds4) S2_LIN_RQ(5, pc5, ds5) S2_LIN_RQ(6, pc6, ds6) S2_LIN_RQ(7, pc7, ds7)
+        } else {
+            if (wave + NWV < NQ) {
+                const int q2 = wave + NWV;
+                const unsigned char *sbase = reinterpret_cast<const unsigned char *>(ab.hdesc + (size_t)ab.q[q2].slot * HS) + part * SCB;
+                const unsigned int dbase = (unsigned int)((q2 / SPR) * QUAD + (q2 % SPR) * SCB);
+                if constexpr (NBATCH == 2) { S2_STAGE_REQUEST(0) S2_STAGE_STORE(0) }
+                S2_STAGE_REQUEST((NBATCH - 1) * BATCH * kWave)
+                S2_STAGE_STORE((NBATCH - 1) * BATCH * kWave)
+            }
+            const int q1 = wave < NQ ? wave : NQ - 1;
+            const unsigned char *sbase = reinterpret_cast<const unsigned char *>(ab.hdesc + (size_t)ab.q[q1].slot * HS) + part * SCB;
+            const unsigned int dbase = (unsigned int)((q1 / SPR) * QUAD + (q1 % SPR) * SCB);
             if constexpr (NBATCH == 2) { S2_STAGE_REQUEST(0) S2_STAGE_STORE(0) }
             S2_STAGE_REQUEST((NBATCH - 1) * BATCH * kWave)
-            S2_STAGE_STORE((NBATCH - 1) * BATCH * kWave)
-        }
-        const int q1 = wave < NQ ? wave : NQ - 1;
-        const unsigned char *sbase = reinterpret_cast<const unsigned char *>(ab.hdesc + (size_t)ab.q[q1].slot * HS) + part * SCB;
-        const unsigned int dbase = (unsigned int)((q1 / SPR) * QUAD + (q1 % SPR) * SCB);
-        if constexpr (NBATCH == 2) { S2_STAGE_REQUEST(0) S2_STAGE_STORE(0) }
-        S2_STAGE_REQUEST((NBATCH - 1) * BATCH * kWave)
+        }
         S2_STAMP_AT(61);
         __builtin_amdgcn_sched_barrier(0);
         constexpr int NPRE = NBUF - 1 < 4 ? NBUF - 1 : 4;
 #pragma unroll
-        for (int j = 0; j < NPRE; ++j) F[j] = *reinterpret_cast<const u32x4 *>(base_cur + load_off(j));
+        for (int j = 0; j < NPRE; ++j) F[j] = frag_load(rs_cur, j);
         b_cur = first_shift(0); b_nxt = first_shift(1);
         __builtin_amdgcn_sched_barrier(0);
         S2_STAMP_AT(62);
-        if (wave < NQ) { S2_STAGE_STORE((NBATCH - 1) * BATCH * kWave) }
+        if constexpr (PREP) {
+            S2_LIN_ST(0, pc0, ds0) S2_LIN_ST(1, pc1, ds1) S2_LIN_ST(2, pc2, ds2) S2_LIN_ST(3, pc3, ds3)
+            S2_LIN_ST(4, pc4, ds4) S2_LIN_ST(5, pc5, ds5) S2_LIN_ST(6, pc6, ds6) S2_LIN_ST(7, pc7, ds7)
+        } else if (wave < NQ) { S2_STAGE_STORE((NBATCH - 1) * BATCH * kWave) }
         S2_STAMP_AT(63);
         __builtin_amdgcn_sched_barrier(0);
 #pragma unroll
-        for (int j = NPRE; j < NBUF - 1; ++j) F[j] = *reinterpret_cast<const u32x4 *>(base_cur + load_off(j));
+        for (int j = NPRE; j < NBUF - 1; ++j) F[j] = frag_load(rs_cur, j);
     }
     __syncthreads();
     S2_STAMP_AT(33);
@@ -1165,9 +1234,9 @@
             if (o == 0) {
                 const int j = g + NBUF - 1;
                 constexpr int kLastLanes = SPK == 2 ? 16 : 4 * (NIT - 1) + 16 - 16 * (NL - 1);
-                if (j == NL - 1 && kLastLanes < 16) { if (c16 < kLastLanes) F[j % NBUF] = *reinterpret_cast<const u32x4 *>(base_cur + load_off(j)); }
-                else if (j < NL) F[j % NBUF] = *reinterpret_cast<const u32x4 *>(base_cur + load_off(j));
-                else if (j - NL < NBUF - 1) F[j % NBUF] = *reinterpret_cast<const u32x4 *>(base_nxt + load_off(j - NL));
+                if (j == NL - 1 && kLastLanes < 16) { if (c16 < kLastLanes) F[j % NBUF] = frag_load(rs_cur, j); }
+                else if (j < NL) F[j % NBUF] = frag_load(rs_cur, j);
+                else if (j - NL < NBUF - 1) F[j % NBUF] = frag_load(rs_nxt, j - NL);
             }
             if (it + 1 < NIT) readB(bfr[(it + 1) & 1], it + 1);
 #ifndef S2_NO_READ_PIN
@@ -1228,7 +1297,7 @@
         if (k < 6) S2_STAMP_AT(35 + 3 * k);
 #pragma unroll
         for (int j = NGR + NBUF - 1 - NL; j < NBUF - 1; ++j)
-            if (j >= 0) F[j % NBUF] = *reinterpret_cast<const u32x4 *>(base_nxt + load_off(j));
+            if (j >= 0) F[j % NBUF] = frag_load(rs_nxt, j);
         static_assert(NIT >= 2, "");
         scan_bases(b_nxt);
         if constexpr (((NIT - 1) & 1) == 0) __builtin_amdgcn_sched_barrier(0);
@@ -1255,7 +1324,7 @@
                     *reinterpret_cast<f4v *>(fa.part + (((size_t)c16 * (size_t)ab.pair_stride + (size_t)ci) * NP + part) * (s2_part_f4<RG, S, W>() * 4) + (s2_pass_off<RG, S, W>(p) + j4) * 4) = sum;
             }
         }
-        base_cur = base_nxt; base_nxt = kf_base(k + 2);
+        rs_cur = rs_nxt; rs_nxt = kf_rsrc(k + 2);
         b_cur = b_nxt; b_nxt = first_shift(k + 2);
         if (k < 6) S2_STAMP_AT(36 + 3 * k);
     }
@@ -1481,23 +1550,38 @@
 
 template <int RG, int S, int W, bool MASKS = true, bool D2 = true>
 __global__ __launch_bounds__(kScreenWaves * kWave, Align2Cfg<S>::OCC) void sc_screen2_tail2_kernel(Screen2Args fa, ScreenBatchArgs nb, const unsigned char *halign, int u_lo, int u_n,
-                                                                                     int align_blocks, int chunks)
+                                                                                     int align_blocks, int chunks, unsigned char *prep, int prep_blocks)
 {
     extern __shared__ __attribute__((aligned(16))) unsigned char smem_tail2[];
+    const int front = align_blocks + prep_blocks;
 #ifdef SCL_TAIL_FINISH_FIRST
-    const int fblocks = (int)gridDim.x - align_blocks;
-    const int b = (int)blockIdx.x < fblocks ? (int)blockIdx.x + align_blocks : (int)blockIdx.x - fblocks;
+    const int fblocks = (int)gridDim.x - front;
+    const int b = (int)blockIdx.x < fblocks ? (int)blockIdx.x + front : (int)blockIdx.x - fblocks;
 #else
     const int b = (int)blockIdx.x;
 #endif
     if (b < align_blocks) {
         const int wave = __builtin_amdgcn_readfirstlane((int)(threadIdx.x >> 6));
-        sc_align2_role<S, W>(nb, halign, u_lo, u_n, b * kScreenWaves + wave, align_blocks * kScreenWaves, smem_tail2 + (size_t)wave * Align2Cfg<S>::LDS_WAVE);
+        sc_align2_role<S, W>(nb, halign, u_lo, u_n, b * kScreenWaves + wave, align_blocks * kScreenWaves, smem_tail2 + (size_t)wave * Align2Cfg<S>::LDS_WAVE,
+                             s2_prep_km<RG, S, W>(prep));
         return;
     }
+    if (b < front) { sc_screen2_prep_role<RG, S, W>(nb, prep, b - align_blocks, prep_blocks); return; }
     int qi, chunk;
-    if (!finish_block_of(b - align_blocks, fa.prod.nq, chunks, qi, chunk)) return;
+    if (!finish_block_of(b - front, fa.prod.nq, chunks, qi, chunk)) return;
     sc_screen2_finish_body<RG, S, W, MASKS, D2>(fa, qi, chunk);
+}
+
+template <int RG, int S, int W>
+__global__ __launch_bounds__(kScreenWaves * kWave, Align2Cfg<S>::OCC) void sc_align2_kernel(ScreenBatchArgs ab, const unsigned char *halign, int u_lo, int u_n,
+                                                                                     unsigned char *prep, int prep_blocks)
+{
+    extern __shared__ __attribute__((aligned(16))) unsigned char smem_align2[];
+    const int align_blocks = (int)gridDim.x - prep_blocks;
+    if ((int)blockIdx.x >= align_blocks) { sc_screen2_prep_role<RG, S, W>(ab, prep, (int)blockIdx.x - align_blocks, prep_blocks); return; }
+    const int wave = __builtin_amdgcn_readfirstlane((int)(threadIdx.x >> 6));
+    sc_align2_role<S, W>(ab, halign, u_lo, u_n, (int)blockIdx.x * kScreenWaves + wave, align_blocks * kScreenWaves,
+                         smem_align2 + (size_t)wave * Align2Cfg<S>::LDS_WAVE, s2_prep_km<RG, S, W>(prep));
 }
 
 static bool screen_second_form()
@@ -1513,6 +1597,10 @@
 int sc_screen_max_batch(const DbView &db, int SR)
 {
     return (sc_screen_is_wide(db, SR) && screen_second_form()) ? S2Cfg<20, 180, 19>::NQ : kMaxScreenBatch;
+}
+size_t sc_screen_prep_bytes(const DbView &db, int SR)
+{
+    return sc_screen_is_wide(db, SR) ? s2_prep_images_bytes<20, 180, 19>() : s2_prep_images_bytes<16, 120, 13>();
 }
 size_t sc_screen_scratch_floats(const DbView &db, int SR)
 {
@@ -1585,6 +1673,8 @@
     };
     const int v2_min = screen_v2_min_env() > 0 ? screen_v2_min_env() : (S <= 128 ? 4 : 2);
     auto second_form_for = [&](const ScreenBatch &b) {
+        for (int i = 0; i < b.nq; ++i)
+            if ((unsigned long long)(b.buf[i] + 1) * (unsigned long long)b.pair_stride * sizeof(int) > 0xffffffffull) return false;
         return screen_second_form() && b.part && probe == 0 && variant == 0 && b.nq >= v2_min && b.nq <= S2Cfg<RG, S, W>::NQ;
     };
     const bool use_v2 = second_form_for(sb);
@@ -1596,6 +1686,14 @@
         for (int i = 1; i < b.nq; ++i) { lo = b.base[i] < lo ? b.base[i] : lo; hi = b.base[i] + b.n[i] > hi ? b.base[i] + b.n[i] : hi; }
         *lo_out = lo; *n_out = hi - lo;
     };
+    auto prep_of = [&](const ScreenBatch &b) -> unsigned char * {
+        int lo, n;
+        union_of(b, &lo, &n);
+        return (b.prep && b.prep_owner && n <= b.prep_km_cap) ? b.prep : nullptr;
+    };
+    bool sb_prepared = !(phases & kScreenAlign) && prep_of(sb) && *sb.prep_owner == sb.prep_id;
+    if ((phases & kScreenAlign) && sb.prep_owner) *sb.prep_owner = -1;
+    if (next && next->prep_owner) *next->prep_owner = -1;
     auto align2_blocks = [&](int u_n) {
         static const int env = scl_lab_int("SCL_ALIGN2_WGS", 0);
         int b = (u_n + kScreenWaves * 3 - 1) / (kScreenWaves * 3);
@@ -1608,7 +1706,10 @@
         if (use_v2) {
             int ulo, un;
             union_of(sb, &ulo, &un);
-            hipLaunchKernelGGL((sc_align2_kernel<RG, S, W>), dim3(align2_blocks(un)), dim3(kScreenWaves * kWave), lds_a2, stream, ab, db.halign, ulo, un);
+            unsigned char *prep = prep_of(sb);
+            const int pblocks = prep ? kPrepBlocks : 0;
+            hipLaunchKernelGGL((sc_align2_kernel<RG, S, W>), dim3(align2_blocks(un) + pblocks), dim3(kScreenWaves * kWave), lds_a2, stream, ab, db.halign, ulo, un, prep, pblocks);
+            if (prep) { *sb.prep_owner = sb.prep_id; sb_prepared = true; }
         } else {
             ab.nb = align_blocks(ngroups, sb.nq, false);
             hipLaunchKernelGGL((sc_align_kernel<RG, S, W>), dim3(ab.nb * sb.nq), dim3(kScreenWaves * kWave), lds0, stream, ab);
@@ -1622,6 +1723,7 @@
         std::atomic<bool> &attr2 = attr2_dev[dev_ & 63];
         if (!attr2.load(std::memory_order_acquire)) {
             hipError_t e = hipFuncSetAttribute((const void *)sc_screen2_kernel<RG, S, W>, hipFuncAttributeMaxDynamicSharedMemorySize, (int)(s2_lds<RG, S, W>()));
+            if (e == hipSuccess) e = hipFuncSetAttribute((const void *)sc_screen2_kernel<RG, S, W, true>, hipFuncAttributeMaxDynamicSharedMemorySize, (int)(s2_lds<RG, S, W>()));
             if (e != hipSuccess) return e;
             attr2.store(true, std::memory_order_release);
         }
@@ -1633,7 +1735,10 @@
         if (nwg < WGU) nwg = WGU;
         f2.nwg = nwg;
         hipError_t e = hipSuccess;
-        hipLaunchKernelGGL((sc_screen2_kernel<RG, S, W>), dim3(nwg), dim3(S2Cfg<RG, S, W>::WV * kWave), (s2_lds<RG, S, W>()), stream, f2);
+        f2.prep = sb_prepared ? sb.prep : nullptr;
+        if (f2.prep && sb.prep_launches) ++*sb.prep_launches;
+        if (f2.prep) hipLaunchKernelGGL((sc_screen2_kernel<RG, S, W, true>), dim3(nwg), dim3(S2Cfg<RG, S, W>::WV * kWave), (s2_lds<RG, S, W>()), stream, f2);
+        else hipLaunchKernelGGL((sc_screen2_kernel<RG, S, W>), dim3(nwg), dim3(S2Cfg<RG, S, W>::WV * kWave), (s2_lds<RG, S, W>()), stream, f2);
         if ((e = hipGetLastError()) != hipSuccess) return e;
         const int chunks = (nmax + 255) / 256;
         const dim3 fgrid(finish_blocks(chunks, sb.nq)), ablock(kScreenWaves * kWave);
@@ -1658,20 +1763,23 @@
             nb.nb = nb.nb > per_q ? per_q : nb.nb;
             ablocks = nb.nb * next->nq;
         }
+        unsigned char *nprep = next_v2 ? prep_of(*next) : nullptr;
+        const int pblocks = nprep ? kPrepBlocks : 0;
+        if (nprep) *next->prep_owner = next->prep_id;
         static const int tail_env = scl_lab_int("SCL_SCREEN_TAIL", 1);
         if (tail_env) {
-            const dim3 tgrid(ablocks + finish_blocks(chunks, sb.nq));
+            const dim3 tgrid(ablocks + pblocks + finish_blocks(chunks, sb.nq));
             const bool d2 = !sb.no_ring_metric;
             if (!next_v2) hipLaunchKernelGGL((sc_screen2_tail_kernel<RG, S, W>), tgrid, ablock, lds0, stream, f2, nb, ablocks, chunks);
-            else if (sb.smask && d2) hipLaunchKernelGGL((sc_screen2_tail2_kernel<RG, S, W, true, true>), tgrid, ablock, lds_a2, stream, f2, nb, db.halign, ulo, un, ablocks, chunks);
-            else if (sb.smask) hipLaunchKernelGGL((sc_screen2_tail2_kernel<RG, S, W, true, false>), tgrid, ablock, lds_a2, stream, f2, nb, db.halign, ulo, un, ablocks, chunks);
-            else if (d2) hipLaunchKernelGGL((sc_screen2_tail2_kernel<RG, S, W, false, true>), tgrid, ablock, lds_a2, stream, f2, nb, db.halign, ulo, un, ablocks, chunks);
-            else hipLaunchKernelGGL((sc_screen2_tail2_kernel<RG, S, W, false, false>), tgrid, ablock, lds_a2, stream, f2, nb, db.halign, ulo, un, ablocks, chunks);
+            else if (sb.smask && d2) hipLaunchKernelGGL((sc_screen2_tail2_kernel<RG, S, W, true, true>), tgrid, ablock, lds_a2, stream, f2, nb, db.halign, ulo, un, ablocks, chunks, nprep, pblocks);
+            else if (sb.smask) hipLaunchKernelGGL((sc_screen2_tail2_kernel<RG, S, W, true, false>), tgrid, ablock, lds_a2, stream, f2, nb, db.halign, ulo, un, ablocks, chunks, nprep, pblocks);
+            else if (d2) hipLaunchKernelGGL((sc_screen2_tail2_kernel<RG, S, W, false, true>), tgrid, ablock, lds_a2, stream, f2, nb, db.halign, ulo, un, ablocks, chunks, nprep, pblocks);
+            else hipLaunchKernelGGL((sc_screen2_tail2_kernel<RG, S, W, false, false>), tgrid, ablock, lds_a2, stream, f2, nb, db.halign, ulo, un, ablocks, chunks, nprep, pblocks);
             return hipGetLastError();
         }
         hipLaunchKernelGGL((sc_screen2_finish_kernel<RG, S, W>), fgrid, dim3(256), 0, stream, f2, chunks);
         if ((e = hipGetLastError()) != hipSuccess) return e;
-        if (next_v2) hipLaunchKernelGGL((sc_align2_kernel<RG, S, W>), dim3(ablocks), ablock, lds_a2, stream, nb, db.halign, ulo, un);
+        if (next_v2) hipLaunchKernelGGL((sc_align2_kernel<RG, S, W>), dim3(ablocks + pblocks), ablock, lds_a2, stream, nb, db.halign, ulo, un, nprep, pblocks);
         else hipLaunchKernelGGL((sc_align_kernel<RG, S, W>), dim3(ablocks), ablock, lds0, stream, nb);
         return hipGetLastError();
     }
diff --git a/scl_slam_amd/engine.py b/scl_slam_amd/engine.py
--- a/scl_slam_amd/engine.py
+++ b/scl_slam_amd/engine.py
@@ -1068,6 +1068,13 @@
         self._check(self._lib.scl_alignment_stats(self._h, byref(a), byref(b), int(bool(reset))), "scl_alignment_stats")
         return int(a.value), int(b.value)
 
+    def screen_prepared_launches(self, reset=False):
+        fn = self._lib.scl_screen_prepared_launches
+        fn.restype, fn.argtypes = c_int, [c_void_p, POINTER(c_uint64), c_int]
+        a = c_uint64(0)
+        self._check(fn(self._h, byref(a), int(bool(reset))), "scl_screen_prepared_launches")
+        return int(a.value)
+
     def survivor_stats(self, reset=False):
         q, s, m = c_uint64(0), c_uint64(0), c_uint64(0)
         self._check(self._lib.scl_survivor_stats(self._h, byref(q), byref(s), byref(m), int(bool(reset))), "scl_survivor_stats")
```

Result: faster. 2.635 billion, median of 6 (+3.4%).
